# Florescence/UNet-Medical-Image-Contour-Segmentation

Hardware: AMD Instinct MI355X
Metric: images/sec (train step) UNet 1x512x512->1 (higher is better)
Workload: dtype bf16; 1 GPU; UNet(1,1,bilinear=True) train step (BCE+Dice+boundary, clip 1.0, RMSprop), 8 x 1x512x512 per GPU, global batch 8; parallelism=dp1, global_batch=8, per_gpu_batch=8, bn=per-rank batch statistics, dice=global-batch sums (all-reduced), streams=backward-weights on a side stream

## Files before the change

### include/unet_hip.h

```cpp
#ifndef UNET_HIP_H
#define UNET_HIP_H

#include <stddef.h>
#include <stdint.h>

#ifdef __cplusplus
extern "C" {
#endif

typedef void* uh_stream;

enum { UH_F32 = 0, UH_BF16 = 1,
       UH_F32X3 = 2,
       UH_WFRAG = 0x100, UH_WFRAG_D = 0x200 };
enum { UH_OK = 0, UH_EINVAL = -1, UH_ELAUNCH = -2, UH_EWORKSPACE = -3 };

const char* uh_last_error(void);
int uh_version(void);

int uh_pack_w3x3(const float* w, int64_t sO, int64_t sI, int64_t sH, int64_t sW, int Cout, int Cin,
                 void* w_fwd, void* w_dgrad, int dt, uh_stream stream);
int uh_pack_w3x3_batched(const int64_t* table, int nlayers, int64_t ntiles, void* w_fwd_flat,
                         void* w_dgrad_flat, int dt, uh_stream stream);
int uh_unpack_dw3x3(const float* dw_krsc, float* dw, int64_t sO, int64_t sI, int64_t sH, int64_t sW,
                    int Cout, int Cin, uh_stream stream);

int uh_conv3x3_stat_slabs(int B, int H, int W, int Cin, int Cout, int dt);
int uh_conv3x3_wfrag_ok(int B, int H, int W, int C0, int C1, int Cout, int ld0, int ld1, int ldy, int dt);
int uh_conv3x3_fwd_kernel(int B, int H, int W, int C0, int C1, int Cout, int dt);
int uh_conv3x3_wgrad_plan(int B, int H, int W, int C0, int C1, int Cout, int dt, int narrow, int64_t* out);
int uh_conv3x3_fwd_kernel_plan(int B, int plan_B, int H, int W, int C0, int C1, int Cout, int dt);
int uh_conv3x3_wfrag_ok_plan(int B, int plan_B, int H, int W, int C0, int C1, int Cout, int ld0, int ld1, int ldy, int dt);
int uh_conv3x3_fwd_sum_class(int kernel);
int uh_conv3x3_fwd(const void* x0, int C0, int ld0, const void* x1, int C1, int ld1,
                   const void* w, void* y, int ldy, int Cout, float* stat_partials,
                   int B, int H, int W, int dt, uh_stream stream);
int uh_conv3x3_dgrad_bnsum_rows(int B, int H, int W, int Cdy, int Cdx, int lddy, int lddx, int ldq, int dt);
int uh_conv3x3_dgrad_bnsum(const void* dy, int Cdy, int lddy, const void* w_dgrad, void* dx, int lddx, int Cdx,
                           const void* q, int ldq, const float* coef, float* partials,
                           int B, int H, int W, int dt, uh_stream stream);
int uh_stem_ok(int Cin, int Cout, int dt);
int uh_stem_nblk(int B, int H, int W);
int uh_stem_stats(const void* x, int Cin, int ldx, const void* w, float* stat_partials, int B, int H, int W, int dt,
                  uh_stream stream);
int uh_stem_bn_relu_fwd(const void* x, int Cin, int ldx, const void* w, const float* scale, const float* shift, void* z, int ldz,
                        int B, int H, int W, int dt, uh_stream stream);
int uh_stem_bn_relu_bwd_reduce(const void* dz, int lddz, const void* x, int Cin, int ldx, const void* w, const float* scale,
                               const float* shift, const float* mean, const float* rstd, float* partials, int B, int H, int W,
                               int dt, uh_stream stream);
size_t uh_stem_bwd_wgrad_ws_bytes(int B, int H, int W, int Cin);
int uh_stem_bn_relu_bwd_wgrad(const void* dz, int lddz, const void* x, int Cin, int ldx, const void* w, const float* scale,
                              const float* shift, const float* mean, const float* rstd, const float* dgamma, const float* dbeta,
                              int64_t n_total, float* dw_krsc, void* ws, size_t ws_bytes, int B, int H, int W, int dt,
                              uh_stream stream);
int uh_conv3x3_fwd_affine_relu(const void* x0, int C0, int ld0, const void* x1, int C1, int ld1,
                               const void* w, void* z, int ldz, int Cout, const float* scale,
                               const float* shift, int B, int H, int W, int dt, uh_stream stream);
int uh_conv3x3_fwd_affine_relu_plan(const void* x0, int C0, int ld0, const void* x1, int C1, int ld1,
                                    const void* w, void* z, int ldz, int Cout, const float* scale,
                                    const float* shift, int B, int plan_B, int H, int W, int dt, uh_stream stream);
size_t uh_conv3x3_wgrad_ws_bytes(int B, int H, int W, int Cin, int Cout, int dt);
int uh_conv3x3_wgrad(const void* dy, int lddy, const void* x0, int C0, int ld0,
                     const void* x1, int C1, int ld1, float* dw_krsc, int Cout,
                     void* ws, size_t ws_bytes, int B, int H, int W, int dt, uh_stream stream);
int uh_conv3x3_wgrad_partials(const void* dy, int lddy, const void* x0, int C0, int ld0, const void* x1, int C1, int ld1,
                              float* dw_krsc, int Cout, void* ws, size_t ws_bytes, int B, int H, int W, int dt,
// ... 249 lines not shown
```

### unet-medical-image-contour-segmentation_amd/_lib.py

```python
from __future__ import annotations

import ctypes
import os
import re
from typing import Dict, List, Tuple

PKG_DIR = os.path.dirname(os.path.abspath(__file__))
ROOT = os.path.dirname(PKG_DIR)
HEADER = os.path.join(ROOT, "include", "unet_hip.h")
LIB_PATH = os.environ.get("UH_LIB_PATH") or os.path.join(PKG_DIR, "libunet_hip.so")

UH_F32, UH_BF16, UH_F32X3 = 0, 1, 2
UH_WFRAG, UH_WFRAG_D = 0x100, 0x200

_CTYPES = {
    "int": ctypes.c_int, "int64_t": ctypes.c_int64, "float": ctypes.c_float, "double": ctypes.c_double,
    "size_t": ctypes.c_size_t, "uh_stream": ctypes.c_void_p,
}
_RET = {"int": ctypes.c_int, "size_t": ctypes.c_size_t, "const char*": ctypes.c_char_p}


def parse_header(path: str = HEADER) -> Dict[str, Tuple[str, List[str]]]:
    text = open(path).read()
    text = re.sub(r"/\*.*?\*/", " ", text, flags=re.S)
    protos = {}
    for m in re.finditer(r"(const char\*|int|size_t)\s+(uh_\w+)\s*\(([^;{]*?)\)\s*;", text, flags=re.S):
        ret, name, args = m.group(1), m.group(2), " ".join(m.group(3).split())
        types = []
        if args and args != "void":
            for a in args.split(","):
                a = a.strip()
                if "*" in a:
                    types.append("ptr")
                else:
                    types.append(a.rsplit(" ", 1)[0].strip())
        protos[name] = (ret, types)
    return protos


class _Lib:
    def __init__(self):
        self._dll = None
        self.protos = parse_header()

    def load(self):
        if self._dll is not None:
# ... 26 lines not shown
```

### unet-medical-image-contour-segmentation_amd/csrc/conv3x3.hip

```cpp
#include "uh_vec.h"

__host__ __device__ __forceinline__ int uh_wfrag_mode(int es, int rows) { return es == 2 ? ((rows % 128 == 0) ? 2 : 1) : 0; }
template <int ES>
__device__ __forceinline__ int64_t uh_wfrag_index(int o, int tap, int k, int K, int mode) {
    constexpr int CK = 64 / ES, VEC = 16 / ES;
    int g, m;
    if (mode == 2) {
        const int c32 = o & 31;
        g = ((o >> 5) << 1) | ((c32 >> 2) & 1);
        m = ((c32 >> 3) << 2) | (c32 & 3);
    } else if (mode == 1) {
        const int c16 = o & 15, q = c16 >> 2;
        g = o >> 4;
        m = ((((q & 1) << 1) | (q >> 1)) << 2) | (c16 & 3);
    } else {
        g = o >> 4;
        m = o & 15;
    }
    const int chunk = k / CK, e = k - chunk * CK, kp = e / VEC, v = e - kp * VEC;
    return ((((int64_t)g * 9 + tap) * (K / CK) + chunk) * 64 + (kp * 16 + m)) * VEC + v;
}

template <typename T>
__global__ void pack_w3x3_kernel(const float* __restrict__ w, int64_t sO, int64_t sI, int64_t sH, int64_t sW,
// ... 433 lines not shown
            stats[((int64_t)blockIdx.x * 2 + 0) * Cout + co_blk + tid] = red[2 * BN + tid];
            stats[((int64_t)blockIdx.x * 2 + 1) * Cout + co_blk + tid] = red[tid] + red[BN + tid];
        }
        if (blockIdx.y == 0 && tid == 0) stats[(int64_t)gridDim.x * 2 * Cout + blockIdx.x] = (float)(vy * vx);
    }
}

constexpr int HALO2_BYTES = HALO_PIX * 64;
constexpr int HALO2_STRIDE = 6 * 4096;
constexpr unsigned OOB_OFFSET = 0xF0000000u;

__device__ __forceinline__ void uh_dma16(u32x4 desc, unsigned lds_addr, unsigned voff, int soff) {
    asm volatile("s_mov_b32 m0, %0\n\ts_nop 0\n\tbuffer_load_dwordx4 %1, %2, %3 offen lds"
                 :: "s"(lds_addr), "v"(voff), "s"(desc), "s"(soff) : "memory", "m0");
}
__device__ __forceinline__ void uh_ld16_async(u32x4& dst, u32x4 desc, unsigned voff, int soff) {
    asm volatile("buffer_load_dwordx4 %0, %1, %2, %3 offen" : "+v"(dst) : "v"(voff), "s"(desc), "s"(soff) : "memory");
}
__device__ __forceinline__ void uh_ld8_async(u32x2& dst, u32x4 desc, unsigned voff, int soff) {
    asm volatile("buffer_load_dwordx2 %0, %1, %2, %3 offen" : "+v"(dst) : "v"(voff), "s"(desc), "s"(soff) : "memory");
}
__device__ __forceinline__ u32x4 uh_desc_words(const void* p, unsigned bytes) {
    const uint64_t a = (uint64_t)p;
    return u32x4{(unsigned)a, (unsigned)(a >> 32) & 0xffffu, bytes, 0x00020000u};
}
#define UH_WAIT_VM(n) do { asm volatile("s_waitcnt vmcnt(%0)" :: "n"(n) : "memory"); __builtin_amdgcn_sched_barrier(0); } while (0)

__device__ __forceinline__ int halo_swz(int hx) { return ((hx >> 2) & 1) << 1; }

#ifndef UH_BUILD_PRE
#define UH_BUILD_PRE 0
#endif
constexpr int PRE_MAX_C = 512;
template <typename T, int NBW, bool SPLIT = false, bool WRES = false, bool PRE = false, bool BSUM = false, int KS = 1>
__global__ __launch_bounds__(256 * KS, ((NBW == 1 && !WRES && !BSUM && KS == 1) ? 3 : 2)) void conv3x3_fwd_mfma_v2(
    const T* __restrict__ x0, int C0, int ld0, const T* __restrict__ x1, int C1, int ld1,
    const T* __restrict__ w, T* __restrict__ y, int ldy, int Cout, float* __restrict__ stats,
    int B, int H, int W, int tilesX, int tilesY, unsigned x0_bytes, unsigned x1_bytes, unsigned y_bytes,
    const float* __restrict__ ep_scale, const float* __restrict__ ep_shift, int C0v, int C1v, int Coutv, int wfrag,
    const float* __restrict__ pre_scale = nullptr, const float* __restrict__ pre_shift = nullptr,
    const T* __restrict__ bs_y = nullptr, int bs_ld = 0, unsigned bs_bytes = 0, const float* __restrict__ bs_coef = nullptr) {
    static_assert(!PRE || (sizeof(T) == 2 && !SPLIT), "PRE is the bf16 training path");
    static_assert(!BSUM || (sizeof(T) == 2 && !SPLIT && !PRE), "BSUM is the bf16 backward-data path");
    static_assert(KS == 1 || (KS == 2 && sizeof(T) == 2 && NBW == 1 && !SPLIT && !WRES && !PRE), "KS = 2 is a bf16 NBW = 1 form");
    if constexpr (BSUM) {
        x1 = nullptr; C1 = 0; ld1 = 0; x1_bytes = 0;
        C0v = C0; C1v = 0; Coutv = Cout;
        ep_scale = nullptr; ep_shift = nullptr;
        bs_ld = ldy; bs_bytes = y_bytes;
    }
    constexpr int ES = sizeof(T);
    constexpr int CK = 64 / ES;
    constexpr int VEC = 16 / ES;
    constexpr int BN = NBW * 64;
    constexpr int NPIECE = HALO_PIX * 4;
    constexpr int NLOAD = 6;
    constexpr int PF = WRES ? 1 : 2;

    constexpr bool TRI = WRES && !PRE;
    __shared__ __attribute__((aligned(16))) unsigned char lds_all[(TRI ? 3 : KS * 2) * HALO2_STRIDE];
    __shared__ float wg_sum[3][BN];
    __shared__ __attribute__((aligned(16))) float pre_tab[PRE ? 2 * PRE_MAX_C : 4];
    __shared__ __attribute__((aligned(16))) float bs_tab[BSUM ? 4 * BN : 4];
    float n_run = 0.f;

    const int tid = threadIdx.x & 255;
    const int lane = tid & 63;
    const int wave_all = __builtin_amdgcn_readfirstlane((int)(threadIdx.x >> 6));
    const int wave = wave_all & 3;
    const int grp = KS == 2 ? (wave_all >> 2) : 0;
    unsigned char* const lds = lds_all + grp * (2 * HALO2_STRIDE);
    const int lx = lane & 15, kg = lane >> 4;
    const int nslab = Cout / BN;
    const int nlanes = gridDim.x / nslab;
    int tile_lane, slab;
    if ((nlanes & 7) == 0) {
        const int xcd = blockIdx.x & 7, jj = blockIdx.x >> 3;
        slab = jj % nslab;
        tile_lane = (jj / nslab) * 8 + xcd;
    } else {
        slab = blockIdx.x / nlanes;
        tile_lane = blockIdx.x - slab * nlanes;
    }
    const int co_blk = slab * BN;
    const int Cin = C0 + C1;
    const int nch0 = (C0v + CK - 1) / CK, nch1 = (C1v + CK - 1) / CK;
    const int nchunk = nch0 + nch1;
    const int skip1 = C0 / CK - nch0;
    auto chunk_of = [&](int v) -> int { return v < nch0 ? v : v + skip1; };
    const int ntile = B * tilesX * tilesY;

    const u32x4 rs0 = uh_desc_words(x0, x0_bytes);
    const u32x4 rs1 = uh_desc_words(x1 ? x1 : x0, x1 ? x1_bytes : x0_bytes);
    __amdgpu_buffer_rsrc_t rsy = __builtin_amdgcn_make_buffer_rsrc((void*)y, 0, (int)y_bytes, 0x00020000);
    const unsigned lds_base = (unsigned)(uintptr_t)(__attribute__((address_space(3))) unsigned char*)lds;
    constexpr bool REL_LIVE = !(BSUM && NBW == 2);
    auto rel_of = [&](int t, int k) -> int {
        const int p = t + k * 256, q = p >> 2;
        const int hy = (q * 3641) >> 16, hx = q - hy * HALO_W;
        return (hy * W + hx) * ld0 * ES + (((p & 3) ^ halo_swz(hx)) << 4);
    };
    int rel0[NLOAD];
#pragma unroll
    for (int k = 0; k < NLOAD; ++k) rel0[k] = REL_LIVE ? rel_of(tid, k) : 0;
    int d_b = 0, d_y0 = 0, d_x0 = 0;
    bool d_in = false;
    auto dma_tile = [&](int tile) {
        int t = tile;
        const int txt = t % tilesX; t /= tilesX;
        const int tyt = t % tilesY;
        d_b = t / tilesY;
        d_y0 = tyt * TILE; d_x0 = txt * TILE;
        d_in = d_y0 >= 1 && d_y0 + TILE + 1 <= H && d_x0 >= 1 && d_x0 + TILE + 1 <= W;
    };
    auto dma_chunk = [&](int c, int bufi, bool live) {
// ... 107 lines not shown
                    const f32x4 t0 = t[0], t1 = t[1], t2 = t[2], t3 = t[3];
                    float r[8];
#pragma unroll
                    for (int e = 0; e < 4; ++e) {
                        r[2 * e] = __uint_as_float(v[e] << 16);
                        r[2 * e + 1] = __uint_as_float(v[e] & 0xffff0000u);
                    }
                    r[0] = uh_relu(fmaf(r[0], t0[0], t0[1])); r[1] = uh_relu(fmaf(r[1], t0[2], t0[3]));
                    r[2] = uh_relu(fmaf(r[2], t1[0], t1[1])); r[3] = uh_relu(fmaf(r[3], t1[2], t1[3]));
                    r[4] = uh_relu(fmaf(r[4], t2[0], t2[1])); r[5] = uh_relu(fmaf(r[5], t2[2], t2[3]));
                    r[6] = uh_relu(fmaf(r[6], t3[0], t3[1])); r[7] = uh_relu(fmaf(r[7], t3[2], t3[3]));
                    const bf16x8 o = {(bf16_t)r[0], (bf16_t)r[1], (bf16_t)r[2], (bf16_t)r[3],
                                      (bf16_t)r[4], (bf16_t)r[5], (bf16_t)r[6], (bf16_t)r[7]};
                    *slot = __builtin_bit_cast(u32x4, o);
                }
            }
        }
    };
    auto chunk_fence = [&](int c_next, int bufi_next, bool live_next) {
        if constexpr (TRI) {
            asm volatile("s_waitcnt vmcnt(%0) lgkmcnt(0)\n\ts_barrier" :: "n"(NLOAD) : "memory");
        } else if constexpr (PRE) {
            asm volatile("s_waitcnt vmcnt(0)" ::: "memory");
            __builtin_amdgcn_sched_barrier(0);
            if (live_next) pre_transform(c_next, bufi_next);
            asm volatile("s_waitcnt lgkmcnt(0)\n\ts_barrier" ::: "memory");
        } else {
            asm volatile("s_waitcnt vmcnt(0) lgkmcnt(0)\n\ts_barrier" ::: "memory");
        }
        __builtin_amdgcn_sched_barrier(0);
    };

    int tile = tile_lane;
    if (tile >= ntile) return;
    WFrag wA[3][NBW], wB[3][NBW], wC[3][NBW];
#pragma unroll
    for (int r = 0; r < 3; ++r)
#pragma unroll
        for (int n = 0; n < NBW; ++n) {
            wA[r][n].v = wB[r][n].v = wC[r][n].v = u32x4{0u, 0u, 0u, 0u};
            wA[r][n].hi = wB[r][n].hi = wC[r][n].hi = wA[r][n].lo = wB[r][n].lo = wC[r][n].lo = u32x2{0u, 0u};
        }
    auto load_w = [&](WFrag (&dst)[3][NBW], int chunk, int sft) {
        const int64_t wsrc = (int64_t)chunk * CK + (int64_t)sft * Cin;
#pragma unroll
        for (int r = 0; r < 3; ++r)
#pragma unroll
            for (int n = 0; n < NBW; ++n) wfrag_async(dst[r][n], wsrc + wn_off(n) + (int64_t)(r * 3) * Cin, n, r * 3 + sft, chunk);
    };
    int bufi = 0;
    f32x4 acc[16][NBW];
    auto mma_shift = [&](const unsigned char* buf, int sft, auto&& wget) {
        u32x4 xf[18];
        int lq = lane;
        if constexpr (!REL_LIVE) asm volatile("" : "+v"(lq));
        const unsigned char* xcol = buf + ((lq & 15) + sft) * 64 + (((lq >> 4) ^ halo_swz((lq & 15) + sft)) << 4);
        auto rd = [&](int k) { return *reinterpret_cast<const u32x4*>(xcol + k * (HALO_W * 64)); };
#pragma unroll
        for (int k = 0; k < 2 + PF; ++k) xf[k] = rd(k);
#pragma unroll
        for (int k = 2; k < 18; ++k) {
            if (k + PF < 18) xf[k + PF] = rd(k + PF);
            __builtin_amdgcn_sched_barrier(0);
            if constexpr (SPLIT) {
                if (k == 2) { split4(xf[0]); split4(xf[1]); }
                split4(xf[k]);
            }
// ... 97 lines not shown
            const int cur_c = chunk_of(v);
            const int next_c = chunk_of((v + 1 < v_end) ? v + 1 : v_first);
            const unsigned char* buf = lds + bufi * HALO2_STRIDE;
            load_w(wB, cur_c, 1);
            __builtin_amdgcn_sched_barrier(0);
            mma_shift(buf, 0, wsel(wA));
            load_w(wC, cur_c, 2);
            bool live_next = true;
            if (v + 1 < v_end) {
                dma_chunk(chunk_of(v + 1), bufi ^ 1, true);
            } else {
                live_next = next_tile < ntile;
                if (live_next) dma_tile(next_tile);
                dma_chunk(chunk_of(v_first), bufi ^ 1, live_next);
            }
            UH_WAIT_VM(NWLOAD + NLOAD);
            mma_shift(buf, 1, wsel(wB));
            load_w(wA, next_c, 0);
            UH_WAIT_VM(NLOAD + NWLOAD);
            mma_shift(buf, 2, wsel(wC));
            chunk_fence(next_c, bufi ^ 1, live_next);
        }
        }

        if constexpr (KS == 2) {
            f32x4* scratch = reinterpret_cast<f32x4*>(lds_all);
            if (grp == 1) {
#pragma unroll
                for (int i = 0; i < 16; ++i)
#pragma unroll
                    for (int n = 0; n < NBW; ++n) scratch[(i * NBW + n) * 256 + tid] = acc[i][n];
            }
            __syncthreads();
            if (grp == 1) return;
#pragma unroll
            for (int i = 0; i < 16; ++i)
#pragma unroll
                for (int n = 0; n < NBW; ++n) acc[i][n] += scratch[(i * NBW + n) * 256 + tid];
        }
        int t = tile;
        const int txt = t % tilesX; t /= tilesX;
        const int tyt = t % tilesY;
        const int b = t / tilesY;
        const int y0 = tyt * TILE, x0p = txt * TILE;
        const int gx = x0p + lx;
        const int vy = min(TILE, H - y0), vx = min(TILE, W - x0p);
        const bool full = (vy == TILE) && (vx == TILE);
        constexpr int BQB = 2 * NBW;
        u32x2 bqA[BSUM ? 8 : 1], bqB[BSUM ? 8 : 1];
        int lane_o = lane;
        if constexpr (BSUM) asm volatile("" : "+v"(lane_o));
        const int lx_o = lane_o & 15, kg_o = lane_o >> 4;
        auto bq_load = [&](u32x2 (&dst)[BSUM ? 8 : 1], int bi) {
            if constexpr (BSUM) {
                __amdgpu_buffer_rsrc_t rsq = __builtin_amdgcn_make_buffer_rsrc((void*)bs_y, 0, (int)bs_bytes, 0x00020000);
                const int n = bi >> 1, i0 = (bi & 1) * 8;
                const int gxc = min(x0p + (lane_o & 15), W - 1);
                const unsigned voff = (unsigned)((gxc * bs_ld + co_blk + ch(lane_o >> 4, n, 0)) * ES);
#pragma unroll
                for (int i = 0; i < 8; ++i) {
                    const int r = min(i0 + i, vy - 1);
                    dst[i] = __builtin_amdgcn_raw_buffer_load_b64(rsq, voff, ((b * H + y0 + r) * W) * bs_ld * ES, 0);
                }
            }
        };
        if (ep_scale) {
#pragma unroll
// ... 233 lines not shown
                for (int n = 0; n < NBW; ++n) {
                    const f32x4 q = *reinterpret_cast<const f32x4*>(&PV[ch(kg, n, 0)]);
#pragma unroll
                    for (int j = 0; j < 4; ++j) {
                        const float pv = q[j];
                        float s1 = 0.f, s2 = 0.f;
                        if (full) {
#pragma unroll
                            for (int i = 0; i < 16; ++i) {
                                const float d = acc[i][n][j] - pv;
                                s1 += d;
                                s2 = fmaf(d, d, s2);
                            }
                        } else {
#pragma unroll
                            for (int i = 0; i < 16; ++i) {
                                const float d = ((i < vy) && (gx < W)) ? acc[i][n][j] - pv : 0.f;
                                s1 += d;
                                s2 = fmaf(d, d, s2);
                            }
                        }
                        const float a1 = uh_row16_sum(s1), a2 = uh_row16_sum(s2);
                        if (lx == 0) {
                            const int cl = ch(kg, n, j);
                            S1[cl] += a1;
                            S2[cl] += a2;
                        }
                    }
                }
            }
            n_run += (float)(vy * vx);
        }
    }
    if constexpr (BSUM) {
        if (lx == 0) {
#pragma unroll
            for (int n = 0; n < NBW; ++n)
#pragma unroll
                for (int j = 0; j < 4; ++j) {
                    const int cl = ch(kg, n, j);
                    stats[((int64_t)tile_lane * 2 + 0) * Cout + co_blk + cl] = wg_sum[0][cl];
                    stats[((int64_t)tile_lane * 2 + 1) * Cout + co_blk + cl] = wg_sum[1][cl] * bs_tab[3 * BN + cl];
                }
        }
        return;
    }
    if (stats) {
        if (lx == 0) {
            const float inv_n = 1.f / n_run;
#pragma unroll
            for (int n = 0; n < NBW; ++n)
#pragma unroll
                for (int j = 0; j < 4; ++j) {
                    const int cl = ch(kg, n, j);
                    const float a1 = wg_sum[0][cl], a2 = wg_sum[1][cl];
                    stats[((int64_t)tile_lane * 2 + 0) * Cout + co_blk + cl] = wg_sum[2][cl] + a1 * inv_n;
                    stats[((int64_t)tile_lane * 2 + 1) * Cout + co_blk + cl] = fmaxf(a2 - a1 * a1 * inv_n, 0.f);
                }
        }
        float* counts = stats + (int64_t)ntile * 2 * Cout;
        if (slab == 0) {
            if (tid == 0) counts[tile_lane] = n_run;
            if (tile_lane == 0)
                for (int r = nlanes + tid; r < ntile; r += 256) counts[r] = 0.f;
        }
    }
}

template <typename T>
__global__ __launch_bounds__(256) void conv3x3_fwd_stem(const T* __restrict__ x, int Cin, int ldx,
                                                        const T* __restrict__ w, T* __restrict__ y, int ldy, int Cout,
                                                        float* __restrict__ stats, int B, int H, int W, int tilesX,
                                                        int tilesY) {
    __shared__ float xs[HALO_PIX * 4];
    __shared__ float red[4 * 64];
    const int tid = threadIdx.x, lane = tid & 63, wave = tid >> 6;
    int t = blockIdx.x;
    const int txt = t % tilesX; t /= tilesX;
    const int tyt = t % tilesY;
    const int b = t / tilesY;
    const int y0 = tyt * TILE, x0p = txt * TILE;
    for (int idx = tid; idx < HALO_PIX * 4; idx += 256) {
        int q = idx >> 2, ci = idx & 3;
        int hy = q / HALO_W, hx = q - hy * HALO_W;
        int gy = y0 - 1 + hy, gx = x0p - 1 + hx;
        float v = 0.f;
        if (ci < Cin && gy >= 0 && gy < H && gx >= 0 && gx < W)
            v = uh_to_f32(x[(int64_t)((b * H + gy) * W + gx) * ldx + ci]);
        xs[idx] = v;
    }
    __syncthreads();
    for (int cg = 0; cg < Cout; cg += 64) {
        const int co = cg + lane;
        const bool cok = co < Cout;
        float wr[36];
#pragma unroll
        for (int tap = 0; tap < 9; ++tap)
#pragma unroll
// ... 352 lines not shown
    if (threadIdx.x == 0) stats[(int64_t)gridDim.x * 2 * C + blockIdx.x] = (float)(vy * vx);
}

extern "C" int uh_conv3x3_stat_slabs(int B, int H, int W, int Cin, int Cout, int dt) {
    (void)Cin; (void)Cout; (void)dt;
    return B * ((H + TILE - 1) / TILE) * ((W + TILE - 1) / TILE);
}

static bool fwd_ksplit_ok(int64_t ntile, int Cin, int Cout) {
    static const bool off = getenv("UH_NO_KSPLIT") != nullptr && getenv("UH_NO_KSPLIT")[0] == '1';
    const int nchunk = Cin / 32;
    return !off && Cin % 32 == 0 && Cout % 64 == 0 && ntile * (Cout / 64) <= 256 && nchunk >= 8 && nchunk % 2 == 0;
}

enum FwdKernel {
    FWD_SIMT = 0,
    FWD_SLAB128 = 1,
    FWD_WRES = 2,
    FWD_KSPLIT = 3,
    FWD_STREAM = 4,
    FWD_LARGE = 5,
};

static int fwd_sum_class(int kernel) {
    return (kernel == FWD_SLAB128 || kernel == FWD_WRES || kernel == FWD_STREAM) ? FWD_SLAB128 : kernel;
}

struct FwdPlan {
    FwdKernel kernel;
    int stem;
    int slabs, lanes;
    int threads;
    bool split, pre, bsum;
};

static FwdPlan fwd_plan(int es, int B, int H, int W, int C0, int C1, int Cout, int ld0, int ld1, int ldy, bool ptrs16, bool y16,
                        bool split, bool narrow, bool pre, bool bsum, int plan_B = 0) {
    const int tiles1 = ((H + TILE - 1) / TILE) * ((W + TILE - 1) / TILE);
    const int ntile = B * tiles1;
    const int ck = 64 / es, Cin = C0 + C1;
    FwdPlan p = {FWD_SIMT, 0, 1, ntile, 256, split, pre, bsum};
    const bool mfma = C0 % ck == 0 && C1 % ck == 0 && Cout % 64 == 0 && ptrs16 && (ld0 * es) % 16 == 0 &&
                      (C1 == 0 || (ld1 * es) % 16 == 0) && (ldy * es) % 16 == 0;
    if (!mfma) {
        const bool y_ok = y16 && (ldy * es) % 16 == 0;
        if (Cin > 4 || C1 != 0) p.stem = 0;
        else if (es == 2 && Cout == 64 && y_ok) { p.stem = 3; p.lanes = ntile < 1024 ? ntile : 1024; }
        else p.stem = (Cout % (16 / es) == 0 && y_ok) ? 2 : 1;
        return p;
    }
    const int64_t px = (int64_t)B * H * W, lim = (1ll << 31) - 4096;
    if (px * ld0 * es >= lim || (C1 && px * ld1 * es >= lim) || px * ldy * es >= lim ||
        (int64_t)Cout * 9 * Cin * (split ? 4 : es) >= lim) {
        p.kernel = FWD_LARGE;
        p.slabs = Cout % 128 == 0 ? Cout / 128 : Cout / 64;
        return p;
    }
    auto lanes_for = [&](int per_cu, int slabs) {
        int gx = (per_cu * 256 + slabs - 1) / slabs;
        gx = (gx + 7) & ~7;
        return gx < ntile ? gx : ntile;
    };
    const bool bf16 = es == 2 && !split && !narrow;
    auto form = [&](int64_t nt) {
        if (Cout % 128 == 0 && nt * (Cout / 128) >= 512) return FWD_SLAB128;
        if (bf16 && Cin == 64) return FWD_WRES;
        if (bf16 && !pre && fwd_ksplit_ok(nt, Cin, Cout)) return FWD_KSPLIT;
        return FWD_STREAM;
    };
    p.kernel = form(ntile);
    if (plan_B > 0 && plan_B != B) {
        const FwdKernel pinned = form((int64_t)plan_B * tiles1);
        if (fwd_sum_class(pinned) != fwd_sum_class(p.kernel)) p.kernel = pinned;
    }
    switch (p.kernel) {
    case FWD_SLAB128: p.slabs = Cout / 128; p.lanes = lanes_for(2, p.slabs); break;
    case FWD_WRES: p.slabs = Cout / 64; p.lanes = lanes_for(2, p.slabs); break;
    case FWD_KSPLIT: p.slabs = Cout / 64; p.lanes = ntile; p.threads = 512; break;
    default: p.slabs = Cout / 64; p.lanes = lanes_for(bsum ? 2 : 3, p.slabs); break;
    }
    return p;
}

template <typename T, bool SPLIT, bool PRE, bool BSUM, typename... Args>
static void fwd_v2_form(const FwdPlan& p, hipStream_t st, Args... args) {
    constexpr bool BF16 = sizeof(T) == 2 && !SPLIT;
    const dim3 grid(p.lanes * p.slabs), block(p.threads);
    switch (p.kernel) {
    case FWD_SLAB128: hipLaunchKernelGGL((conv3x3_fwd_mfma_v2<T, 2, SPLIT, false, PRE, BSUM>), grid, block, 0, st, args...); break;
    case FWD_WRES:
        if constexpr (BF16) hipLaunchKernelGGL((conv3x3_fwd_mfma_v2<T, 1, false, true, PRE, BSUM>), grid, block, 0, st, args...);
        break;
    case FWD_KSPLIT:
        if constexpr (BF16 && !PRE) hipLaunchKernelGGL((conv3x3_fwd_mfma_v2<T, 1, false, false, false, BSUM, 2>), grid, block, 0, st, args...);
        break;
    case FWD_STREAM: hipLaunchKernelGGL((conv3x3_fwd_mfma_v2<T, 1, SPLIT, false, PRE, BSUM>), grid, block, 0, st, args...); break;
    default: break;
    }
}

template <typename T, typename... Args>
static void fwd_v2_launch(const FwdPlan& p, hipStream_t st, Args... args) {
    constexpr bool BF16 = sizeof(T) == 2;
    if (p.split) {
        if constexpr (!BF16) fwd_v2_form<T, true, false, false>(p, st, args...);
    } else if (p.bsum) {
        if constexpr (BF16) fwd_v2_form<T, false, false, true>(p, st, args...);
    } else if (p.pre) {
        if constexpr (BF16 && UH_BUILD_PRE) fwd_v2_form<T, false, true, false>(p, st, args...);
    } else {
        fwd_v2_form<T, false, false, false>(p, st, args...);
    }
}

struct ConvCall {
    const void *x0 = nullptr, *x1 = nullptr;
    int C0 = 0, ld0 = 0, C1 = 0, ld1 = 0, Cout = 0, B = 0, H = 0, W = 0;
    int dt = UH_F32;
    bool wfrag = false;
    int C0v = -1, C1v = -1, Coutv = -1;
    const float *pre_scale = nullptr, *pre_shift = nullptr;
    hipStream_t st = nullptr;
};
struct FwdCall : ConvCall {
    const void* w = nullptr;
    void* y = nullptr; int ldy = 0, plan_B = 0;
    float* stats = nullptr;
    const float *ep_scale = nullptr, *ep_shift = nullptr;
    bool ep_done = false;
    const void* bs_y = nullptr;
    int bs_ld = 0; const float* bs_coef = nullptr;
};

enum { CK_BF16_ONLY = 1, CK_NARROW = 2, CK_WFRAG = 4 };
static int conv_check(const char* fn, ConvCall& c, bool ptrs, int ldo, int dt, int flags = 0) {
    const bool narrow = (flags & CK_NARROW) != 0;
    UH_REQUIRE(c.x0 && ptrs, "%s: null pointer", fn);
    UH_REQUIRE(c.B > 0 && c.H > 0 && c.W > 0 && c.C0 > 0 && c.C1 >= 0 && c.Cout > 0, "%s: bad shape", fn);
    UH_REQUIRE(!narrow || (c.C0v > 0 && c.C0v <= c.C0 && c.C1v >= 0 && c.C1v <= c.C1 && c.Coutv > 0 && c.Coutv <= c.Cout),
               "%s: bad valid counts", fn);
    UH_REQUIRE(c.ld0 >= (narrow ? c.C0v : c.C0) && ldo >= (narrow ? c.Coutv : c.Cout) &&
               (c.C1 == 0 || (c.x1 && c.ld1 >= (narrow ? c.C1v : c.C1))), "%s: bad strides", fn);
    UH_REQUIRE((int64_t)c.B * c.H * c.W < (1ll << 31), "%s: pixel count overflows int32", fn);
    c.wfrag = (flags & CK_WFRAG) && (dt & UH_WFRAG);
    if (flags & CK_WFRAG) dt &= ~UH_WFRAG;
    UH_REQUIRE(!(flags & CK_BF16_ONLY) || dt == UH_BF16, "%s: bf16 only (dtype %d)", fn, dt);
    UH_REQUIRE(dt == UH_F32 || dt == UH_BF16 || dt == UH_F32X3, "%s: bad dtype %d", fn, dt);
    const int vec = dt == UH_BF16 ? 8 : 4;
    UH_REQUIRE(!narrow || (c.C0v % vec == 0 && c.C1v % vec == 0 && c.Coutv % vec == 0),
               "%s: valid counts must be multiples of a 16-byte piece", fn);
    c.dt = dt;
    return UH_OK;
}

template <typename T>
static int conv3x3_fwd_dispatch(FwdCall& c) {
    const T *x0 = (const T*)c.x0, *x1 = (const T*)c.x1, *w = (const T*)c.w, *bs_y = (const T*)c.bs_y;
    T* y = (T*)c.y;
    const float *ep_scale = c.ep_scale, *ep_shift = c.ep_shift;
    const bool split = c.dt == UH_F32X3, narrow = c.C0v >= 0, pre = c.pre_scale != nullptr, bsum = bs_y != nullptr;
    const int C0v = narrow ? c.C0v : c.C0, C1v = narrow ? c.C1v : c.C1, Coutv = narrow ? c.Coutv : c.Cout;
    c.ep_done = false;
    constexpr int ES = sizeof(T);
    const int tilesX = (c.W + TILE - 1) / TILE, tilesY = (c.H + TILE - 1) / TILE;
    const int Cin = c.C0 + c.C1;
    const bool ptrs16 = uh_aligned16(x0) && (c.C1 == 0 || uh_aligned16(x1)) && uh_aligned16(w) && uh_aligned16(y);
    const FwdPlan p = fwd_plan(ES, c.B, c.H, c.W, c.C0, c.C1, c.Cout, c.ld0, c.ld1, c.ldy, ptrs16, uh_aligned16(y), split, narrow, pre, bsum, c.plan_B);
    if (p.kernel != FWD_SIMT && p.kernel != FWD_LARGE) {
        if (ep_scale && !(uh_aligned16(ep_scale) && uh_aligned16(ep_shift))) ep_scale = ep_shift = nullptr;
        UH_REQUIRE(!split || ES == 4, "conv3x3_fwd: bf16x3 needs fp32 tensors");
        UH_REQUIRE(!(split && c.wfrag), "conv3x3_fwd: bf16x3 filters are KRSC packs");
        UH_REQUIRE(!(narrow && c.wfrag), "conv3x3_fwd: narrow-tensor calls take KRSC packs");
        if (pre) {
            UH_REQUIRE(UH_BUILD_PRE, "conv3x3_fwd: the consumer-side BatchNorm+ReLU instantiations are not in this build (UH_BUILD_PRE=1); uh_conv3x3_pre_ok says so");
            UH_REQUIRE(ES == 2, "conv3x3_fwd: the fused BatchNorm+ReLU input is a bf16 path; ask uh_conv3x3_pre_ok first");
            UH_REQUIRE(!(split || narrow || c.C0 > PRE_MAX_C), "conv3x3_fwd: the fused BatchNorm+ReLU input needs a plain bf16 call with at most %d channels in source 0; ask uh_conv3x3_pre_ok first", PRE_MAX_C);
        }
        const int64_t px = (int64_t)c.B * c.H * c.W, bq = bsum ? px * c.bs_ld * ES : 0;
        if (bsum) {
            UH_REQUIRE(ES == 2, "uh_conv3x3_dgrad_bnsum: bf16 only; ask uh_conv3x3_dgrad_bnsum_rows first");
            UH_REQUIRE(!(split || narrow || c.C1 != 0 || !c.stats || !c.bs_coef || c.bs_ld != c.ldy || !uh_aligned16(bs_y) || bq >= (1ll << 31) - 4096),
                       "uh_conv3x3_dgrad_bnsum: needs a plain single-source bf16 call and a 16-byte aligned BatchNorm input below 2 GiB; ask uh_conv3x3_dgrad_bnsum_rows first");
        }
        fwd_v2_launch<T>(p, c.st, x0, c.C0, c.ld0, x1, c.C1, c.ld1, w, y, c.ldy, c.Cout, c.stats, c.B, c.H, c.W, tilesX, tilesY, (unsigned)(px * c.ld0 * ES),
                         (unsigned)(c.C1 ? px * c.ld1 * ES : 0), (unsigned)(px * c.ldy * ES), ep_scale, ep_shift, C0v, C1v, Coutv,
                         c.wfrag ? 1 : 0, c.pre_scale, c.pre_shift, bs_y, c.bs_ld, (unsigned)bq, c.bs_coef);
        UH_CHECK_LAUNCH(pre ? "conv3x3_fwd_mfma_v2 (BatchNorm+ReLU input)"
                            : bsum ? "conv3x3_fwd_mfma_v2 (backward-data + BatchNorm sums)" : "conv3x3_fwd_mfma_v2");
        c.ep_done = ep_scale != nullptr;
        return UH_OK;
    }
    if (p.kernel == FWD_LARGE) {
        UH_REQUIRE(!pre, "conv3x3_fwd: the fused BatchNorm+ReLU input needs the LDS-DMA MFMA kernel (tensors below 2 GiB); ask uh_conv3x3_pre_ok first");
        UH_REQUIRE(!bsum, "uh_conv3x3_dgrad_bnsum: needs the LDS-DMA MFMA kernel (tensors below 2 GiB); ask uh_conv3x3_dgrad_bnsum_rows first");
        UH_REQUIRE(!c.wfrag, "conv3x3_fwd: the filter is packed fragment-major (UH_WFRAG) but this call cannot take the LDS-DMA MFMA kernel (a tensor of 2 GiB or more); ask uh_conv3x3_wfrag_ok first");
        UH_REQUIRE(!split, "conv3x3_fwd: bf16x3 is implemented for tensors below 2 GiB only");
        UH_REQUIRE(!narrow, "conv3x3_fwd: narrow tensors are implemented for tensors below 2 GiB only");
        if (c.Cout % 128 == 0)
            hipLaunchKernelGGL((conv3x3_fwd_mfma<T, 4>), dim3(p.lanes, p.slabs), dim3(p.threads), 0, c.st, x0, c.C0, c.ld0, x1, c.C1,
                               c.ld1, w, y, c.ldy, c.Cout, c.stats, c.B, c.H, c.W, tilesX, tilesY);
        else
            hipLaunchKernelGGL((conv3x3_fwd_mfma<T, 2>), dim3(p.lanes, p.slabs), dim3(p.threads), 0, c.st, x0, c.C0, c.ld0, x1, c.C1,
                               c.ld1, w, y, c.ldy, c.Cout, c.stats, c.B, c.H, c.W, tilesX, tilesY);
        UH_CHECK_LAUNCH("conv3x3_fwd_mfma");
        return UH_OK;
    }
    UH_REQUIRE(!pre, "conv3x3_fwd: the fused BatchNorm+ReLU input needs an MFMA-aligned shape; ask uh_conv3x3_pre_ok first");
    UH_REQUIRE(!bsum, "uh_conv3x3_dgrad_bnsum: needs an MFMA-aligned shape; ask uh_conv3x3_dgrad_bnsum_rows first");
    UH_REQUIRE(!c.wfrag, "conv3x3_fwd: the filter is packed fragment-major (UH_WFRAG) but the shape / alignment is outside the MFMA path; ask uh_conv3x3_wfrag_ok first");
    UH_REQUIRE(!split, "conv3x3_fwd: bf16x3 needs an MFMA-aligned shape (Cin %% 16 == 0, Cout %% 64 == 0, 16-byte strides)");
    UH_REQUIRE(!narrow, "conv3x3_fwd: narrow tensors need padded counts that are MFMA-aligned and 16-byte strides");
    if (p.stem == 3) {
        if constexpr (ES == 2) {
            switch (Cin) {
                case 1: hipLaunchKernelGGL((conv3x3_fwd_stem_v3<T, 1>), dim3(p.lanes), dim3(256), 0, c.st, x0, c.ld0, w, y, c.ldy, c.stats, c.B, c.H, c.W, tilesX, tilesY, ep_scale, ep_shift); break;
                case 2: hipLaunchKernelGGL((conv3x3_fwd_stem_v3<T, 2>), dim3(p.lanes), dim3(256), 0, c.st, x0, c.ld0, w, y, c.ldy, c.stats, c.B, c.H, c.W, tilesX, tilesY, ep_scale, ep_shift); break;
                case 3: hipLaunchKernelGGL((conv3x3_fwd_stem_v3<T, 3>), dim3(p.lanes), dim3(256), 0, c.st, x0, c.ld0, w, y, c.ldy, c.stats, c.B, c.H, c.W, tilesX, tilesY, ep_scale, ep_shift); break;
                default: hipLaunchKernelGGL((conv3x3_fwd_stem_v3<T, 4>), dim3(p.lanes), dim3(256), 0, c.st, x0, c.ld0, w, y, c.ldy, c.stats, c.B, c.H, c.W, tilesX, tilesY, ep_scale, ep_shift); break;
            }
// ... 38 lines not shown
                              int ldy, int Cout, float* stat_partials, int B, int H, int W, int dt, uh_stream stream) {
    FwdCall c;
    c.x0 = x0; c.C0 = C0; c.ld0 = ld0; c.x1 = x1; c.C1 = C1; c.ld1 = ld1; c.w = w; c.y = y; c.ldy = ldy; c.Cout = Cout;
    c.stats = stat_partials; c.B = B; c.H = H; c.W = W; c.st = (hipStream_t)stream;
    return conv3x3_fwd_call("uh_conv3x3_fwd", c, dt);
}

extern "C" int uh_conv3x3_wfrag_ok_plan(int B, int plan_B, int H, int W, int C0, int C1, int Cout, int ld0, int ld1, int ldy,
                                        int dt) {
    if (dt != UH_F32 && dt != UH_BF16) return 0;
    if (B <= 0 || plan_B < 0 || H <= 0 || W <= 0 || C0 <= 0 || C1 < 0 || Cout <= 0) return 0;
    const FwdKernel k = fwd_plan(dt == UH_BF16 ? 2 : 4, B, H, W, C0, C1, Cout, ld0, ld1, ldy, true, true, false, false, false,
                                 false, plan_B).kernel;
    return k != FWD_SIMT && k != FWD_LARGE;
}
extern "C" int uh_conv3x3_wfrag_ok(int B, int H, int W, int C0, int C1, int Cout, int ld0, int ld1, int ldy, int dt) {
    return uh_conv3x3_wfrag_ok_plan(B, 0, H, W, C0, C1, Cout, ld0, ld1, ldy, dt);
}

extern "C" int uh_conv3x3_fwd_kernel(int B, int H, int W, int C0, int C1, int Cout, int dt) {
    UH_REQUIRE(B > 0 && H > 0 && W > 0 && C0 > 0 && C1 >= 0 && Cout > 0, "uh_conv3x3_fwd_kernel: bad shape");
    UH_REQUIRE(dt == UH_F32 || dt == UH_BF16 || dt == UH_F32X3, "uh_conv3x3_fwd_kernel: bad dtype %d", dt);
    return fwd_plan(dt == UH_BF16 ? 2 : 4, B, H, W, C0, C1, Cout, C0, C1, Cout, true, true, dt == UH_F32X3, false, false,
                    false).kernel;
}

extern "C" int uh_conv3x3_fwd_kernel_plan(int B, int plan_B, int H, int W, int C0, int C1, int Cout, int dt) {
    UH_REQUIRE(B > 0 && plan_B >= 0 && H > 0 && W > 0 && C0 > 0 && C1 >= 0 && Cout > 0, "uh_conv3x3_fwd_kernel_plan: bad shape");
    UH_REQUIRE(dt == UH_F32 || dt == UH_BF16 || dt == UH_F32X3, "uh_conv3x3_fwd_kernel_plan: bad dtype %d", dt);
    return fwd_plan(dt == UH_BF16 ? 2 : 4, B, H, W, C0, C1, Cout, C0, C1, Cout, true, true, dt == UH_F32X3, false, false,
                    false, plan_B).kernel;
}

extern "C" int uh_conv3x3_fwd_sum_class(int kernel) {
    UH_REQUIRE(kernel >= FWD_SIMT && kernel <= FWD_LARGE, "uh_conv3x3_fwd_sum_class: bad kernel code %d", kernel);
    return fwd_sum_class(kernel);
}

extern "C" int uh_conv3x3_pre_ok(int B, int H, int W, int C0, int Cout, int ld0, int ldy, int dt) {
#if !UH_BUILD_PRE
    return 0;
#endif
    if (dt != UH_BF16 || C0 > PRE_MAX_C) return 0;
    if (C0 % 64 || Cout % 64) return 0;
    return uh_conv3x3_wfrag_ok(B, H, W, C0, 0, Cout, ld0, 0, ldy, dt);
}

extern "C" int uh_conv3x3_fwd_pre(const void* x0, int C0, int ld0, const float* pre_scale, const float* pre_shift, const void* w,
                                  void* y, int ldy, int Cout, float* stat_partials, int B, int H, int W, int dt,
                                  uh_stream stream) {
    UH_REQUIRE(pre_scale && pre_shift, "uh_conv3x3_fwd_pre: null pointer");
    FwdCall c;
    c.x0 = x0; c.C0 = C0; c.ld0 = ld0; c.w = w; c.y = y; c.ldy = ldy; c.Cout = Cout; c.stats = stat_partials;
    c.B = B; c.H = H; c.W = W; c.st = (hipStream_t)stream; c.pre_scale = pre_scale; c.pre_shift = pre_shift;
    if (const int rc = conv_check("uh_conv3x3_fwd_pre", c, c.w && c.y, c.ldy, dt, CK_BF16_ONLY | CK_WFRAG)) return rc;
    UH_REQUIRE(UH_BUILD_PRE, "uh_conv3x3_fwd_pre: the consumer-side BatchNorm+ReLU instantiations are not in this build (UH_BUILD_PRE=1); uh_conv3x3_pre_ok says so");
    UH_REQUIRE(uh_conv3x3_pre_ok(B, H, W, C0, Cout, ld0, ldy, c.dt), "uh_conv3x3_fwd_pre: shape outside the fused path (uh_conv3x3_pre_ok)");
    return conv3x3_fwd_dispatch<bf16_t>(c);
}

extern "C" int uh_conv3x3_dgrad_bnsum_rows(int B, int H, int W, int Cdy, int Cdx, int lddy, int lddx, int ldq, int dt) {
    if (dt != UH_BF16) return 0;
    if (!uh_conv3x3_wfrag_ok(B, H, W, Cdy, 0, Cdx, lddy, 0, lddx, dt)) return 0;
    if (ldq != lddx) return 0;
    return fwd_plan(2, B, H, W, Cdy, 0, Cdx, lddy, 0, lddx, true, true, false, false, false, true).lanes;
}
// ... 15 lines not shown
}

extern "C" int uh_conv3x3_fwd_affine_relu_plan(const void* x0, int C0, int ld0, const void* x1, int C1, int ld1, const void* w,
                                               void* z, int ldz, int Cout, const float* scale, const float* shift, int B,
                                               int plan_B, int H, int W, int dt, uh_stream stream) {
    UH_REQUIRE(plan_B >= 0, "uh_conv3x3_fwd_affine_relu: bad plan length %d", plan_B);
    UH_REQUIRE(scale && shift, "uh_conv3x3_fwd_affine_relu: null pointer");
    FwdCall c;
    c.x0 = x0; c.C0 = C0; c.ld0 = ld0; c.x1 = x1; c.C1 = C1; c.ld1 = ld1; c.w = w; c.y = z; c.ldy = ldz; c.Cout = Cout;
    c.B = B; c.H = H; c.W = W; c.st = (hipStream_t)stream; c.ep_scale = scale; c.ep_shift = shift; c.plan_B = plan_B;
    const int rc = conv3x3_fwd_call("uh_conv3x3_fwd_affine_relu", c, dt);
    if (rc != UH_OK || c.ep_done) return rc;
    return uh_bn_relu_apply(z, ldz, scale, shift, z, ldz, (int64_t)B * H * W, Cout, c.dt == UH_BF16 ? UH_BF16 : UH_F32, stream);
}

extern "C" int uh_conv3x3_fwd_affine_relu(const void* x0, int C0, int ld0, const void* x1, int C1, int ld1, const void* w,
                                          void* z, int ldz, int Cout, const float* scale, const float* shift, int B,
                                          int H, int W, int dt, uh_stream stream) {
    return uh_conv3x3_fwd_affine_relu_plan(x0, C0, ld0, x1, C1, ld1, w, z, ldz, Cout, scale, shift, B, 0, H, W, dt, stream);
}

extern "C" int uh_conv3x3_fwd_narrow_plan(const void* x0, int C0, int C0v, int ld0, const void* x1, int C1, int C1v, int ld1,
                                          const void* w, void* y, int ldy, int Cout, int Coutv, float* stat_partials,
                                          const float* scale, const float* shift, int B, int plan_B, int H, int W, int dt,
                                          uh_stream stream) {
    UH_REQUIRE(plan_B >= 0, "uh_conv3x3_fwd_narrow: bad plan length %d", plan_B);
    UH_REQUIRE((scale == nullptr) == (shift == nullptr), "uh_conv3x3_fwd_narrow: scale and shift come together");
    FwdCall c;
    c.x0 = x0; c.C0 = C0; c.ld0 = ld0; c.x1 = x1; c.C1 = C1; c.ld1 = ld1; c.w = w; c.y = y; c.ldy = ldy; c.Cout = Cout;
    c.stats = stat_partials; c.B = B; c.H = H; c.W = W; c.st = (hipStream_t)stream; c.ep_scale = scale; c.ep_shift = shift;
    c.C0v = C0v; c.C1v = C1v; c.Coutv = Coutv; c.plan_B = plan_B;
    const int rc = conv3x3_fwd_call("uh_conv3x3_fwd_narrow", c, dt, CK_NARROW);
    if (rc != UH_OK || !scale || c.ep_done) return rc;
    return uh_bn_relu_apply(y, ldy, scale, shift, y, ldy, (int64_t)B * H * W, Coutv, dt == UH_BF16 ? UH_BF16 : UH_F32, stream);
}

extern "C" int uh_conv3x3_fwd_narrow(const void* x0, int C0, int C0v, int ld0, const void* x1, int C1, int C1v, int ld1,
                                     const void* w, void* y, int ldy, int Cout, int Coutv, float* stat_partials,
                                     const float* scale, const float* shift, int B, int H, int W, int dt, uh_stream stream) {
    return uh_conv3x3_fwd_narrow_plan(x0, C0, C0v, ld0, x1, C1, C1v, ld1, w, y, ldy, Cout, Coutv, stat_partials, scale, shift, B, 0,
                                      H, W, dt, stream);
}

template <typename T> struct WgradCfg;
template <> struct WgradCfg<bf16_t> { static constexpr int TH = 8; };
template <> struct WgradCfg<float> { static constexpr int TH = 8; };

typedef __attribute__((ext_vector_type(16))) float f32x16;
typedef __attribute__((ext_vector_type(4))) short s16x4;

template <typename T, bool SPLIT = false>
__global__ __launch_bounds__(256, 2) void conv3x3_wgrad_mfma(
    const T* __restrict__ dy, int lddy, const T* __restrict__ x0, int C0, int ld0, const T* __restrict__ x1, int C1,
    int ld1, float* __restrict__ slabs, int Cout, int B, int H, int W, int tilesX, int tilesY, int nsplit,
    int C0v, int C1v, int Coutv) {
    constexpr int ES = sizeof(T);
    constexpr int TH = WgradCfg<T>::TH;
    constexpr int PB = 64 * ES;
    constexpr int XPIX = (TH + 2) * HALO_W;
    constexpr int DPIX = TH * TILE;
    constexpr int VEC = 16 / ES;
    constexpr int PPP = PB / 16;
    __shared__ __attribute__((aligned(16))) unsigned char lds[(XPIX + DPIX) * PB];
    unsigned char* xs = lds;
    unsigned char* ds = lds + XPIX * PB;

    const int tid = threadIdx.x, lane = tid & 63, wave = tid >> 6;
    const int wr = wave >> 1, wc = wave & 1;
    const int Cin = C0 + C1;
    const int nci = Cin / 64;
    const int cot = blockIdx.y / nci, cit = blockIdx.y - cot * nci;
    const int co0 = cot * 64, ci0 = cit * 64;
    const T* xsrc; int ldx;
    int xleft;
    if (ci0 < C0) { xsrc = x0 + ci0; ldx = ld0; xleft = C0v - ci0; } else { xsrc = x1 + (ci0 - C0); ldx = ld1; xleft = C1v - (ci0 - C0); }
    const T* dsrc = dy + co0;
    const int dleft = Coutv - co0;

    const int ntile = B * tilesX * tilesY;
    const int split = blockIdx.x;
    const int t_begin = (int)(((int64_t)ntile * split) / nsplit);
    const int t_end = (int)(((int64_t)ntile * (split + 1)) / nsplit);

    f32x16 acc[9];
#pragma unroll
    for (int k = 0; k < 9; ++k)
#pragma unroll
        for (int j = 0; j < 16; ++j) acc[k][j] = 0.f;

    auto lds_addr = [&](int q, int byte) -> int {
        if constexpr (ES == 2) return q * PB + (byte ^ (((q >> 1) & 1) << 6));
        else return q * PB + byte;
    };

    for (int tile = t_begin; tile < t_end; ++tile) {
        int t = tile;
        const int txt = t % tilesX; t /= tilesX;
        const int tyt = t % tilesY;
        const int b = t / tilesY;
        const int y0 = tyt * TH, x0p = txt * TILE;
        __syncthreads();
        constexpr int SB = 4;
        for (int base = 0; base < XPIX * PPP; base += SB * 256) {
            u32x4 v[SB];
            bool ok[SB];
#pragma unroll
            for (int k = 0; k < SB; ++k) {
                const int idx = min(base + tid + k * 256, XPIX * PPP - 1);
                const int q = idx / PPP, part = idx - q * PPP;
                const int hy = q / HALO_W, hx = q - hy * HALO_W;
                const int gy = y0 - 1 + hy, gx = x0p - 1 + hx;
                ok[k] = gy >= 0 && gy < H && gx >= 0 && gx < W && part * VEC < xleft;
                const int gyc = min(max(gy, 0), H - 1), gxc = min(max(gx, 0), W - 1), pc = part * VEC < xleft ? part : 0;
// ... 123 lines not shown
            }
        } else {
            const int l32 = lane & 31, kh = lane >> 5;
#pragma unroll 1
            for (int hy = 0; hy < TH + 2; ++hy) {
#pragma unroll
                for (int s = 0; s < 3; ++s) {
#pragma unroll
                    for (int r = 0; r < 3; ++r) {
                        const int ty = hy - r;
                        if (ty < 0 || ty >= TH) continue;
#pragma unroll
                        for (int kk = 0; kk < 8; ++kk) {
                            const int px = kk * 2 + kh;
                            float a = *reinterpret_cast<const float*>(ds + (ty * TILE + px) * PB + (wr * 32 + l32) * 4);
                            float bb = *reinterpret_cast<const float*>(xs + (hy * HALO_W + px + s) * PB + (wc * 32 + l32) * 4);
                            acc[r * 3 + s] = __builtin_amdgcn_mfma_f32_32x32x2f32(a, bb, acc[r * 3 + s], 0, 0, 0);
                        }
                    }
                }
            }
        }
    }

    float* slab = slabs + (int64_t)split * Cout * 9 * Cin;
    const int ci = ci0 + wc * 32 + (lane & 31);
#pragma unroll
    for (int tap = 0; tap < 9; ++tap)
#pragma unroll
        for (int reg = 0; reg < 16; ++reg) {
            int co = co0 + wr * 32 + (reg & 3) + 8 * (reg >> 2) + 4 * (lane >> 5);
            slab[((int64_t)co * 9 + tap) * Cin + ci] = acc[tap][reg];
        }
}

__device__ __forceinline__ void slab_reduce_block_f32(const float* __restrict__ slabs, float* __restrict__ out, int64_t n,
                                                      int nsplit, int64_t blk, f32x4 (*red)[64]) {
    const int cl = threadIdx.x & 63, sl = threadIdx.x >> 6;
    const int64_t i4 = blk * 64 + cl;
    const int64_t n4 = n >> 2;
    f32x4 a0 = {0.f, 0.f, 0.f, 0.f}, a1 = a0, a2 = a0, a3 = a0;
    if (i4 < n4) {
        const f32x4* base = reinterpret_cast<const f32x4*>(slabs) + i4;
        int k = sl;
        for (; k + 12 < nsplit; k += 16) {
            a0 += base[(int64_t)k * n4];
            a1 += base[(int64_t)(k + 4) * n4];
            a2 += base[(int64_t)(k + 8) * n4];
            a3 += base[(int64_t)(k + 12) * n4];
        }
        for (; k < nsplit; k += 4) a0 += base[(int64_t)k * n4];
    }
    red[sl][cl] = (a0 + a1) + (a2 + a3);
    __syncthreads();
    if (sl == 0 && i4 < n4) reinterpret_cast<f32x4*>(out)[i4] = (red[0][cl] + red[1][cl]) + (red[2][cl] + red[3][cl]);
}

__global__ __launch_bounds__(256) void slab_reduce_kernel(const float* __restrict__ slabs, float* __restrict__ out, int64_t n,
                                                          int nsplit) {
    __shared__ f32x4 red[8][64];
    slab_reduce_block_f32(slabs, out, n, nsplit, blockIdx.x, red);
}

__global__ __launch_bounds__(256) void slab_reduce_tall_kernel(const float* __restrict__ slabs, float* __restrict__ out, int64_t n,
                                                               int nsplit) {
    __shared__ f32x4 red[4][4];
// ... 103 lines not shown
        default: f(std::integral_constant<int, 4>{}); break;
    }
}

__global__ __launch_bounds__(256) void slab_reduce_f16pair_kernel(const unsigned* __restrict__ slabs, float* __restrict__ out,
                                                                  int64_t npair, int row, int nsplit, int coblk) {
    __shared__ f32x4 red[512];
    __shared__ float sc_tab[512];
    slab16_dispatch(nsplit, [&](auto sl) {
        slab_reduce_block_f16pair<decltype(sl)::value>(slabs, out, npair, row, nsplit, coblk, blockIdx.x, red, sc_tab);
    });
}

constexpr int SLAB_TAB = 8;
__global__ __launch_bounds__(256) void slab_reduce_batched_kernel(const int64_t* __restrict__ table, int nrows) {
    __shared__ f32x4 red[512];
    __shared__ float sc_tab[512];
    const int64_t b = blockIdx.x;
    int r = 0;
    for (int k = 1; k < nrows; ++k)
        if (table[k * SLAB_TAB + 6] <= b) r = k;
    const int64_t* t = table + r * SLAB_TAB;
    const int64_t blk = b - t[6];
    if (t[4] == 0)
        slab_reduce_block_f32(reinterpret_cast<const float*>(t[0]), reinterpret_cast<float*>(t[1]), t[2], (int)t[3], blk,
                              reinterpret_cast<f32x4(*)[64]>(red));
    else
        slab16_dispatch((int)t[3], [&](auto sl) {
            slab_reduce_block_f16pair<decltype(sl)::value>(reinterpret_cast<const unsigned*>(t[0]), reinterpret_cast<float*>(t[1]),
                                                           t[2] / 2, (int)t[5], (int)t[3], (int)t[7], blk, red, sc_tab);
        });
}

template <typename T, int NWR, bool PRE = false, bool SLAB16 = false>
__global__ __launch_bounds__(128 * NWR, 2) void conv3x3_wgrad_mfma_v2(
    const T* __restrict__ dy, int lddy, const T* __restrict__ x0, int C0, int ld0, const T* __restrict__ x1, int C1,
    int ld1, float* __restrict__ slabs, int Cout, int B, int H, int W, int tilesX, int tilesY, int nsplit,
    unsigned dy_bytes, unsigned x_bytes, int C0v, int C1v, int Coutv, const float* __restrict__ pre_scale = nullptr,
    const float* __restrict__ pre_shift = nullptr) {
    static_assert(sizeof(T) == 2, "v2 is the bf16 kernel");
    constexpr int TH = 8;
    constexpr int NT = 128 * NWR;
    constexpr int PB = 128;
    constexpr int DPB = 64 * NWR;
    constexpr int DU = DPB / 16;
    constexpr int XPIX = (TH + 2) * HALO_W;
    constexpr int DPIX = TH * TILE;
    constexpr int XUNITS = XPIX * 8;
    constexpr int XR = (XUNITS + NT - 1) / NT;
    constexpr int DR = DPIX * DU / NT;
    constexpr int RB = NT * 16;
    constexpr int XBYTES = XR * RB, STAGE = XBYTES + DR * RB;
    __shared__ __attribute__((aligned(16))) unsigned char lds[2 * STAGE];

    const int tid = threadIdx.x, lane = tid & 63;
    const int wave = __builtin_amdgcn_readfirstlane(tid >> 6);
    const int wr = wave >> 1, wc = wave & 1;
    const int Cin = C0 + C1;
    const int nci = Cin / 64;
    const int cot = blockIdx.y / nci, cit = blockIdx.y - cot * nci;
    const int co0 = cot * (32 * NWR), ci0 = cit * 64;
    const T* xsrc; int ldx;
    int xleft;
    if (ci0 < C0) { xsrc = x0 + ci0; ldx = ld0; xleft = C0v - ci0; } else { xsrc = x1 + (ci0 - C0); ldx = ld1; xleft = C1v - (ci0 - C0); }
    const int dleft = Coutv - co0;
    const u32x4 rsx = uh_desc_words(xsrc, x_bytes);
    const u32x4 rsd = uh_desc_words(dy + co0, dy_bytes);
    const unsigned lds_base = (unsigned)(uintptr_t)(__attribute__((address_space(3))) unsigned char*)lds;

    const int ntile = B * tilesX * tilesY;
    const int split = blockIdx.x;
    const int t_begin = (int)(((int64_t)ntile * split) / nsplit);
    const int t_end = (int)(((int64_t)ntile * (split + 1)) / nsplit);

    int xg[XR], xo[XR];
#pragma unroll
    for (int k = 0; k < XR; ++k) {
        const int p = tid + k * NT;
        const int q = p >> 3;
        const int hy = q / HALO_W, hx = q - hy * HALO_W;
        const int u = (p & 7) ^ (((hx >> 1) & 1) << 2);
        xg[k] = (p < XUNITS && u * 8 < xleft) ? ((hy << 8) | hx) : -1;
        xo[k] = (hy * W + hx) * ldx * 2 + u * 16;
    }
    auto dswz = [&](int col) -> int { return NWR == 2 ? (((col >> 1) & 1) << 2) : ((col & 3) << 2); };
    static_assert(NT / DU == 2 * TILE, "dy DMA rounds are two tile rows apart");
    int dg0, dof0;
    {
        const int q = tid / DU, u = (tid % DU) ^ dswz(q & 15);
        dg0 = (u * 8 < dleft) ? (((q >> 4) << 8) | (q & 15)) : -1;
        dof0 = ((q >> 4) * W + (q & 15)) * lddy * 2 + u * 16;
    }
    const int dof_round = 2 * W * lddy * 2;
    auto issue = [&](int tile, int bufi) {
        int t = tile;
        const int txt = t % tilesX; t /= tilesX;
        const int tyt = t % tilesY;
        const int b = t / tilesY;
        const int y0 = tyt * TH, x0p = txt * TILE;
        const int xbase = ((b * H + y0 - 1) * W + x0p - 1) * ldx * 2;
        const int dbase = ((b * H + y0) * W + x0p) * lddy * 2;
        const unsigned xb = lds_base + bufi * STAGE + wave * 1024;
        const unsigned db = xb + XBYTES;
        const bool inside = y0 >= 1 && y0 + TH + 1 <= H && x0p >= 1 && x0p + TILE + 1 <= W;
// ... 205 lines not shown
                            for (int hh = 0; hh < 2; ++hh)
                                acc[r * 3 + sft][h][hh] = __builtin_amdgcn_mfma_f32_16x16x32_bf16(dfr[pr][h], xfr[a][sft][hh],
                                                                                                 acc[r * 3 + sft][h][hh], 0, 0, 0);
                }
            }
        }
        tile_fence(tile + 1, bufi ^ 1, tile + 1 < t_end);
    }
    }

    if constexpr (SLAB16) {
        float m = 0.f;
#pragma unroll
        for (int tap = 0; tap < 9; ++tap)
#pragma unroll
            for (int h = 0; h < 2; ++h)
#pragma unroll
                for (int hh = 0; hh < 2; ++hh)
#pragma unroll
                    for (int j = 0; j < 4; ++j) m = fmaxf(m, fabsf(acc[tap][h][hh][j]));
#pragma unroll
        for (int o = 32; o > 0; o >>= 1) m = fmaxf(m, __shfl_xor(m, o, 64));
        float* wmax = reinterpret_cast<float*>(lds);
        if (lane == 0) wmax[wave] = m;
        __syncthreads();
#pragma unroll
        for (int k = 0; k < 2 * NWR; ++k) m = fmaxf(m, wmax[k]);
        unsigned eb = (__float_as_uint(m) >> 23) & 0xffu;
        eb = eb < 15u ? 15u : (eb > 254u ? 254u : eb);
        const float sc = __uint_as_float((268u - eb) << 23);
        unsigned* slab16 = reinterpret_cast<unsigned*>(slabs) + (int64_t)split * (Cout / 2) * 9 * Cin;
        if (tid == 0) {
            float* inv = reinterpret_cast<float*>(reinterpret_cast<unsigned*>(slabs) + (int64_t)nsplit * (Cout / 2) * 9 * Cin);
            inv[(int64_t)split * gridDim.y + blockIdx.y] = __uint_as_float((eb - 14u) << 23);
        }
#pragma unroll
        for (int tap = 0; tap < 9; ++tap)
#pragma unroll
            for (int h = 0; h < 2; ++h)
#pragma unroll
                for (int hh = 0; hh < 2; ++hh)
#pragma unroll
                    for (int jp = 0; jp < 4; jp += 2) {
                        const int co = co0 + wr * 32 + h * 16 + (lane >> 4) * 4 + jp;
                        const int ci = ci0 + wc * 32 + hh * 16 + (lane & 15);
                        const f16x2 pr = {(_Float16)(acc[tap][h][hh][jp] * sc), (_Float16)(acc[tap][h][hh][jp + 1] * sc)};
                        slab16[((int64_t)(co >> 1) * 9 + tap) * Cin + ci] = __builtin_bit_cast(unsigned, pr);
                    }
        return;
    }
    float* slab = slabs + (int64_t)split * Cout * 9 * Cin;
#pragma unroll
    for (int tap = 0; tap < 9; ++tap)
#pragma unroll
        for (int h = 0; h < 2; ++h)
#pragma unroll
            for (int hh = 0; hh < 2; ++hh)
#pragma unroll
                for (int j = 0; j < 4; ++j) {
                    const int co = co0 + wr * 32 + h * 16 + (lane >> 4) * 4 + j;
                    const int ci = ci0 + wc * 32 + hh * 16 + (lane & 15);
                    slab[((int64_t)co * 9 + tap) * Cin + ci] = acc[tap][h][hh][j];
                }
}

__global__ void slab_reduce_scalar_kernel(const float* __restrict__ slabs, float* __restrict__ out, int64_t n, int nsplit) {
    int64_t i = (int64_t)blockIdx.x * blockDim.x + threadIdx.x;
    if (i >= n) return;
    float s = 0.f;
    for (int k = 0; k < nsplit; ++k) s += slabs[(int64_t)k * n + i];
    out[i] = s;
}

template <typename T>
__global__ __launch_bounds__(256) void conv3x3_wgrad_stem(const T* __restrict__ dy, int lddy, const T* __restrict__ x,
                                                          int Cin, int ldx, float* __restrict__ slabs, int Cout, int B,
                                                          int H, int W, int tilesX, int tilesY, int nsplit) {
    __shared__ float xs[HALO_PIX * 4];
    __shared__ float red[4 * 64];
    const int tid = threadIdx.x, lane = tid & 63, wave = tid >> 6;
    const int ntile = B * tilesX * tilesY;
    const int split = blockIdx.x;
    const int t_begin = (int)(((int64_t)ntile * split) / nsplit);
    const int t_end = (int)(((int64_t)ntile * (split + 1)) / nsplit);
    const int cg = blockIdx.y * 64;
    const int co = cg + lane;
    const bool cok = co < Cout;
    float acc[36];
#pragma unroll
    for (int k = 0; k < 36; ++k) acc[k] = 0.f;
    for (int tile = t_begin; tile < t_end; ++tile) {
        int t = tile;
        const int txt = t % tilesX; t /= tilesX;
        const int tyt = t % tilesY;
        const int b = t / tilesY;
        const int y0 = tyt * TILE, x0p = txt * TILE;
// ... 240 lines not shown
};

enum SlabReduceKernel { SR_NONE = 0, SR_SCALAR = 1, SR_VEC = 2, SR_TALL = 3, SR_F16PAIR = 4 };
struct SlabReduce {
    SlabReduceKernel kernel;
    int64_t n, blocks;
    int nsplit, row, coblk;
};

static SlabReduce slab_reduce_plan(int64_t n, int nsplit, int row, int coblk, bool f16pair, bool vec16, bool tall) {
    SlabReduce r = {SR_SCALAR, n, (n + 255) / 256, nsplit, row, coblk};
    if (f16pair) { r.kernel = SR_F16PAIR; r.blocks = uh_slab16_blocks(n / 2, nsplit); }
    else if (n % 4 == 0 && vec16 && tall && n <= 4096 && nsplit >= 256) { r.kernel = SR_TALL; r.blocks = (n / 4 + 3) / 4; }
    else if (n % 4 == 0 && vec16) { r.kernel = SR_VEC; r.blocks = (n / 4 + 63) / 64; }
    return r;
}

static int slab_reduce_launch(const SlabReduce& r, const void* slabs, float* dw, hipStream_t st) {
    const dim3 grid((unsigned)r.blocks), block(256);
    if (r.kernel == SR_F16PAIR)
        hipLaunchKernelGGL(slab_reduce_f16pair_kernel, grid, block, 0, st, (const unsigned*)slabs, dw, r.n / 2, r.row, r.nsplit, r.coblk);
    else if (r.kernel != SR_NONE)
        hipLaunchKernelGGL(r.kernel == SR_SCALAR ? slab_reduce_scalar_kernel : r.kernel == SR_TALL ? slab_reduce_tall_kernel : slab_reduce_kernel,
                           grid, block, 0, st, (const float*)slabs, dw, r.n, r.nsplit);
    UH_CHECK_LAUNCH(r.kernel == SR_F16PAIR ? "slab_reduce_f16pair_kernel" : "slab_reduce_kernel");
    return UH_OK;
}

struct WgradPlan {
    WgradKernel kernel;
    int tilesX, tilesY;
    int nsplit;
    dim3 grid;
    int threads;
    bool slab16, pre;
    SlabReduce reduce;
};
struct WgradAlign { bool ptrs, dy, dw, ws; };
static const WgradAlign WG_ALIGNED = {true, true, true, true};
static size_t wgrad_slab_bytes(const WgradPlan& p) { return (size_t)p.nsplit * p.reduce.n * sizeof(float); }

static WgradPlan wgrad_plan(int es, int B, int H, int W, int C0, int C1, int Cout, int ld0, int ld1, int lddy, WgradAlign a16,
                            bool narrow, bool pre) {
    static const bool slab_f32 = getenv("UH_WGRAD_SLAB_F32") != nullptr && getenv("UH_WGRAD_SLAB_F32")[0] == '1';
    static_assert(WgradCfg<bf16_t>::TH == WgradCfg<float>::TH, "one pixel-tile height for both element types");
    const int Cin = C0 + C1;
    const int64_t n = (int64_t)Cout * 9 * Cin;
    WgradPlan p = {WG_GENERIC, 0, 0, 0, dim3(Cout * 9), 256, false, pre, {SR_NONE, n, 0, 0, 9 * Cin, 0}};
    const bool dy_ok = a16.dy && (lddy * es) % 16 == 0;
    int nwr = 2;
    if (a16.ptrs && dy_ok && (ld0 * es) % 16 == 0 && (C1 == 0 || (ld1 * es) % 16 == 0) && C0 % 64 == 0 && Cin % 64 == 0 && Cout % 64 == 0) {
        p.tilesX = (W + TILE - 1) / TILE; p.tilesY = (H + WgradCfg<float>::TH - 1) / WgradCfg<float>::TH;
        const int ntile = B * p.tilesX * p.tilesY;
        const int64_t px = (int64_t)B * H * W, lim = (1ll << 31) - 4096;
        const bool dma = es == 2 && px * (ld0 > ld1 ? ld0 : ld1) * 2 < lim && px * lddy * 2 < lim;
        if (dma && !narrow && Cout % 128 == 0) nwr = 4;
        p.kernel = !dma ? WG_MFMA : nwr == 4 ? WG_DMA128 : WG_DMA64;
        const int ctiles = (Cin / 64) * (Cout / (32 * nwr));
        const int want = ((nwr == 4 ? 256 : 512) + ctiles - 1) / ctiles;
        p.nsplit = want < 1 ? 1 : (want > ntile ? ntile : want);
        p.grid = dim3(p.nsplit, ctiles); p.threads = 128 * nwr;
        p.slab16 = dma && a16.dw && !slab_f32;
    } else if (Cin <= 4 && C1 == 0) {
        p.tilesX = (W + TILE - 1) / TILE; p.tilesY = (H + TILE - 1) / TILE;
        const int ntile = B * p.tilesX * p.tilesY;
        p.nsplit = 1024 > ntile ? ntile : 1024;
        if (es == 2 && Cout == 64 && dy_ok) { p.kernel = WG_STEM_V3; p.grid = dim3(p.nsplit, Cin); }
        else if (Cout % (16 / es) == 0 && dy_ok) { p.kernel = WG_STEM_V2; p.grid = dim3(p.nsplit, 1, Cin); }
        else { p.kernel = WG_STEM; p.grid = dim3(p.nsplit, (Cout + 63) / 64); }
    } else
        return p;
    p.reduce = slab_reduce_plan(n, p.nsplit, 9 * Cin, 32 * nwr, p.slab16, a16.dw && a16.ws, false);
    return p;
}

extern "C" size_t uh_conv3x3_wgrad_ws_bytes(int B, int H, int W, int Cin, int Cout, int dt) {
    const int es = dt == UH_BF16 ? 2 : 4;
    const size_t wide = wgrad_slab_bytes(wgrad_plan(es, B, H, W, Cin, 0, Cout, Cin, 0, Cout, WG_ALIGNED, false, false));
    const size_t narrow = wgrad_slab_bytes(wgrad_plan(es, B, H, W, Cin, 0, Cout, Cin, 0, Cout, WG_ALIGNED, true, false));
    return (wide > narrow ? wide : narrow) + 16;
}

extern "C" int uh_conv3x3_wgrad_plan(int B, int H, int W, int C0, int C1, int Cout, int dt, int narrow, int64_t* out) {
    UH_REQUIRE(out && B > 0 && H > 0 && W > 0 && C0 > 0 && C1 >= 0 && Cout > 0, "uh_conv3x3_wgrad_plan: null pointer or bad shape");
    UH_REQUIRE(dt == UH_F32 || dt == UH_BF16 || dt == UH_F32X3, "uh_conv3x3_wgrad_plan: bad dtype %d", dt);
    const WgradPlan p = wgrad_plan(dt == UH_BF16 ? 2 : 4, B, H, W, C0, C1, Cout, C0, C1, Cout, WG_ALIGNED, narrow != 0, false);
    out[0] = p.kernel; out[1] = p.nsplit; out[2] = p.grid.x; out[3] = p.grid.y; out[4] = p.threads; out[5] = p.slab16 ? 1 : 0;
    out[6] = p.reduce.kernel; out[7] = p.reduce.blocks;
    return UH_OK;
}

template <typename T, typename... Args>
static void wgrad_v2_launch(const WgradPlan& p, hipStream_t st, Args... args) {
    auto form = [&](auto pre) {
        constexpr bool PRE = decltype(pre)::value;
        const dim3 block(p.threads);
        switch ((p.kernel == WG_DMA128 ? 2 : 0) + (p.slab16 ? 1 : 0)) {
        case 3: hipLaunchKernelGGL((conv3x3_wgrad_mfma_v2<T, 4, PRE, true>), p.grid, block, 0, st, args...); break;
        case 2: hipLaunchKernelGGL((conv3x3_wgrad_mfma_v2<T, 4, PRE, false>), p.grid, block, 0, st, args...); break;
        case 1: hipLaunchKernelGGL((conv3x3_wgrad_mfma_v2<T, 2, PRE, true>), p.grid, block, 0, st, args...); break;
        default: hipLaunchKernelGGL((conv3x3_wgrad_mfma_v2<T, 2, PRE, false>), p.grid, block, 0, st, args...); break;
        }
    };
    if (p.pre) {
        if constexpr (UH_BUILD_PRE) form(std::true_type{});
    } else
        form(std::false_type{});
}

struct WgradCall : ConvCall {
    const void* dy = nullptr; int lddy = 0;
    float* dw = nullptr;
    void* ws = nullptr; size_t ws_bytes = 0;
    int64_t* defer = nullptr;
};

template <typename T>
static int conv3x3_wgrad_dispatch(const WgradCall& c) {
    const T *dy = (const T*)c.dy, *x0 = (const T*)c.x0, *x1 = (const T*)c.x1;
    float* slabs = (float*)c.ws;
    constexpr int ES = sizeof(T);
    const int Cin = c.C0 + c.C1;
    const bool split = c.dt == UH_F32X3, narrow = c.C0v >= 0, pre = c.pre_scale != nullptr;
    const int C0v = narrow ? c.C0v : c.C0, C1v = narrow ? c.C1v : c.C1, Coutv = narrow ? c.Coutv : c.Cout;
    const WgradAlign a16 = {uh_aligned16(dy) && uh_aligned16(x0) && (c.C1 == 0 || uh_aligned16(x1)), uh_aligned16(dy), uh_aligned16(c.dw),
                            uh_aligned16(slabs)};
    const WgradPlan p = wgrad_plan(ES, c.B, c.H, c.W, c.C0, c.C1, c.Cout, c.ld0, c.ld1, c.lddy, a16, narrow, pre);
    const bool mfma = p.kernel >= WG_MFMA, dma = p.kernel >= WG_DMA64;
    UH_REQUIRE(!narrow || mfma, "uh_conv3x3_wgrad_narrow: needs the MFMA path (padded channel counts multiples of 64, 16-byte strides)");
    UH_REQUIRE(!split || mfma, "uh_conv3x3_wgrad: bf16x3 needs an MFMA-aligned shape (channel counts multiples of 64, 16-byte strides)");
    UH_REQUIRE(!pre || UH_BUILD_PRE, "uh_conv3x3_wgrad_pre: the consumer-side BatchNorm+ReLU instantiations are not in this build (UH_BUILD_PRE=1); uh_conv3x3_pre_ok says so");
    UH_REQUIRE(!pre || (dma && !narrow && !split), "uh_conv3x3_wgrad_pre: needs the bf16 LDS-DMA kernel (64-aligned channels, tensors below 2 GiB); ask uh_conv3x3_pre_ok first");
    for (int k = 0; c.defer && k < 8; ++k) c.defer[k] = 0;
    if (p.kernel != WG_GENERIC && (c.ws_bytes < wgrad_slab_bytes(p) || !c.ws)) {
        uh_set_error("uh_conv3x3_wgrad: workspace %zu < %zu bytes", c.ws_bytes, wgrad_slab_bytes(p));
        return UH_EWORKSPACE;
    }
    const dim3 block(p.threads);
    const int64_t px = (int64_t)c.B * c.H * c.W;
    switch (p.kernel) {
    case WG_GENERIC:
        hipLaunchKernelGGL(conv3x3_wgrad_generic<T>, p.grid, block, 0, c.st, dy, c.lddy, x0, c.C0, c.ld0, x1, c.C1, c.ld1, c.dw, c.Cout, c.B, c.H, c.W);
        UH_CHECK_LAUNCH("conv3x3_wgrad_generic");
        return UH_OK;
    case WG_DMA64: case WG_DMA128:
        if constexpr (ES == 2)
            wgrad_v2_launch<T>(p, c.st, dy, c.lddy, x0, c.C0, c.ld0, x1, c.C1, c.ld1, slabs, c.Cout, c.B, c.H, c.W, p.tilesX, p.tilesY, p.nsplit,
                               (unsigned)(px * c.lddy * 2), (unsigned)(px * (c.ld0 > c.ld1 ? c.ld0 : c.ld1) * 2), C0v, C1v, Coutv, c.pre_scale,
                               c.pre_shift);
        UH_CHECK_LAUNCH("conv3x3_wgrad_mfma_v2");
        break;
    case WG_MFMA:
        if (split) {
            if constexpr (ES == 4)
                hipLaunchKernelGGL((conv3x3_wgrad_mfma<T, true>), p.grid, block, 0, c.st, dy, c.lddy, x0, c.C0, c.ld0, x1, c.C1, c.ld1, slabs, c.Cout,
                                   c.B, c.H, c.W, p.tilesX, p.tilesY, p.nsplit, C0v, C1v, Coutv);
        } else
            hipLaunchKernelGGL(conv3x3_wgrad_mfma<T>, p.grid, block, 0, c.st, dy, c.lddy, x0, c.C0, c.ld0, x1, c.C1, c.ld1, slabs, c.Cout, c.B, c.H, c.W,
                               p.tilesX, p.tilesY, p.nsplit, C0v, C1v, Coutv);
        UH_CHECK_LAUNCH("conv3x3_wgrad_mfma");
        break;
    case WG_STEM_V3:
        if constexpr (ES == 2)
            hipLaunchKernelGGL((conv3x3_wgrad_stem_v3<T, 1>), p.grid, block, 0, c.st, dy, c.lddy, x0, c.ld0, slabs, c.B, c.H, c.W, p.tilesX,
                               p.tilesY, Cin);
        UH_CHECK_LAUNCH("conv3x3_wgrad_stem_v3");
        break;
    case WG_STEM_V2:
        hipLaunchKernelGGL(conv3x3_wgrad_stem_v2<T>, p.grid, block, 0, c.st, dy, c.lddy, x0, Cin, c.ld0, slabs, c.Cout, c.B, c.H, c.W, p.nsplit);
        UH_CHECK_LAUNCH("conv3x3_wgrad_stem_v2");
        break;
    case WG_STEM:
        hipLaunchKernelGGL(conv3x3_wgrad_stem<T>, p.grid, block, 0, c.st, dy, c.lddy, x0, Cin, c.ld0, slabs, c.Cout, c.B, c.H, c.W, p.tilesX,
                           p.tilesY, p.nsplit);
        UH_CHECK_LAUNCH("conv3x3_wgrad_stem");
        break;
    }
    const SlabReduce& r = p.reduce;
    if (c.defer && (r.kernel == SR_VEC || r.kernel == SR_F16PAIR) && a16.ws) {
        const int64_t row[8] = {(int64_t)(uintptr_t)slabs, (int64_t)(uintptr_t)c.dw, r.n, r.nsplit, r.kernel == SR_F16PAIR, r.row, r.blocks, r.coblk};
        for (int k = 0; k < 8; ++k) c.defer[k] = row[k];
        return UH_OK;
    }
    return slab_reduce_launch(r, slabs, c.dw, c.st);
}

static int conv3x3_wgrad_call(const char* fn, WgradCall& c, int dt, int flags = 0) {
    if (const int rc = conv_check(fn, c, c.dy && c.dw, c.lddy, dt, flags)) return rc;
    return c.dt == UH_BF16 ? conv3x3_wgrad_dispatch<bf16_t>(c) : conv3x3_wgrad_dispatch<float>(c);
}

extern "C" int uh_conv3x3_wgrad(const void* dy, int lddy, const void* x0, int C0, int ld0, const void* x1, int C1, int ld1,
// ... 21 lines not shown
    UH_CHECK_LAUNCH("slab_reduce_batched_kernel");
    return UH_OK;
}

extern "C" int uh_conv3x3_wgrad_pre(const void* dy, int lddy, const void* x0, int C0, int ld0, const float* pre_scale,
                                    const float* pre_shift, float* dw_krsc, int Cout, void* ws, size_t ws_bytes, int B, int H,
                                    int W, int dt, uh_stream stream) {
    UH_REQUIRE(pre_scale && pre_shift, "uh_conv3x3_wgrad_pre: null pointer");
    WgradCall c;
    c.dy = dy; c.lddy = lddy; c.x0 = x0; c.C0 = C0; c.ld0 = ld0; c.dw = dw_krsc; c.Cout = Cout; c.ws = ws; c.ws_bytes = ws_bytes;
    c.B = B; c.H = H; c.W = W; c.st = (hipStream_t)stream; c.pre_scale = pre_scale; c.pre_shift = pre_shift;
    if (const int rc = conv_check("uh_conv3x3_wgrad_pre", c, c.dy && c.dw, c.lddy, dt, CK_BF16_ONLY)) return rc;
    UH_REQUIRE(C0 % 64 == 0 && Cout % 64 == 0, "uh_conv3x3_wgrad_pre: channel counts must be multiples of 64");
    return conv3x3_wgrad_dispatch<bf16_t>(c);
}

extern "C" int uh_stem_ok(int Cin, int Cout, int dt) { return (dt == UH_BF16 && Cin == 1 && Cout == 64) ? 1 : 0; }
extern "C" int uh_stem_nblk(int B, int H, int W) {
    const int64_t ntile = (int64_t)B * ((H + TILE - 1) / TILE) * ((W + TILE - 1) / TILE);
    return (int)(ntile < 1024 ? ntile : 1024);
}

#define UH_STEM_COMMON(fn)                                                                                                    \
    UH_REQUIRE(x && w, fn ": null pointer");                                                                                  \
    UH_REQUIRE(B > 0 && H > 0 && W > 0 && ldx >= Cin, fn ": bad shape");                                                      \
    UH_REQUIRE(uh_stem_ok(Cin, 64, dt), fn ": bf16, one input channel, 64 output channels (uh_stem_ok)");                   \
    UH_REQUIRE((int64_t)B * H * W < (1ll << 31), fn ": pixel count overflows int32")

extern "C" int uh_stem_stats(const void* x, int Cin, int ldx, const void* w, float* stat_partials, int B, int H, int W, int dt,
                             uh_stream stream) {
    UH_STEM_COMMON("uh_stem_stats");
    UH_REQUIRE(stat_partials, "uh_stem_stats: null statistics buffer");
    return uh_stem_mfma_launch(0, x, ldx, w, nullptr, nullptr, nullptr, nullptr, nullptr, nullptr, 0.f, nullptr, 0, nullptr, 0,
                               stat_partials, B, H, W, uh_stem_nblk(B, H, W), stream);
}

extern "C" int uh_stem_bn_relu_fwd(const void* x, int Cin, int ldx, const void* w, const float* scale, const float* shift, void* z,
                                   int ldz, int B, int H, int W, int dt, uh_stream stream) {
    UH_STEM_COMMON("uh_stem_bn_relu_fwd");
    UH_REQUIRE(scale && shift && z && ldz >= 64, "uh_stem_bn_relu_fwd: null pointer / bad stride");
    UH_REQUIRE(uh_aligned16(z) && (ldz * 2) % 16 == 0, "uh_stem_bn_relu_fwd: z must be 16-byte aligned with a 16-byte pixel pitch");
    return uh_stem_mfma_launch(1, x, ldx, w, scale, shift, nullptr, nullptr, nullptr, nullptr, 0.f, nullptr, 0, z, ldz, nullptr, B, H, W,
                               uh_stem_nblk(B, H, W), stream);
}

extern "C" int uh_stem_bn_relu_bwd_reduce(const void* dz, int lddz, const void* x, int Cin, int ldx, const void* w,
                                          const float* scale, const float* shift, const float* mean, const float* rstd,
                                          float* partials, int B, int H, int W, int dt, uh_stream stream) {
    UH_STEM_COMMON("uh_stem_bn_relu_bwd_reduce");
    UH_REQUIRE(dz && scale && shift && mean && rstd && partials && lddz >= 64, "uh_stem_bn_relu_bwd_reduce: null pointer / bad stride");
    UH_REQUIRE(uh_aligned16(dz) && (lddz * 2) % 16 == 0, "uh_stem_bn_relu_bwd_reduce: dz must be 16-byte aligned with a 16-byte pixel pitch");
    return uh_stem_mfma_launch(2, x, ldx, w, scale, shift, mean, rstd, nullptr, nullptr, 0.f, dz, lddz, nullptr, 0, partials, B, H, W,
                               uh_stem_nblk(B, H, W), stream);
}

extern "C" size_t uh_stem_bwd_wgrad_ws_bytes(int B, int H, int W, int Cin) {
    return (size_t)uh_stem_nblk(B, H, W) * 64 * 9 * (Cin > 0 ? Cin : 1) * sizeof(float) + 16;
}

extern "C" int uh_stem_bn_relu_bwd_wgrad(const void* dz, int lddz, const void* x, int Cin, int ldx, const void* w,
                                         const float* scale, const float* shift, const float* mean, const float* rstd,
                                         const float* dgamma, const float* dbeta, int64_t n_total, float* dw_krsc, void* ws,
                                         size_t ws_bytes, int B, int H, int W, int dt, uh_stream stream) {
    UH_STEM_COMMON("uh_stem_bn_relu_bwd_wgrad");
    UH_REQUIRE(dz && scale && shift && mean && rstd && dgamma && dbeta && dw_krsc && ws && lddz >= 64,
               "uh_stem_bn_relu_bwd_wgrad: null pointer / bad stride");
    UH_REQUIRE(uh_aligned16(dz) && (lddz * 2) % 16 == 0, "uh_stem_bn_relu_bwd_wgrad: dz must be 16-byte aligned with a 16-byte pixel pitch");
    UH_REQUIRE(ws_bytes >= uh_stem_bwd_wgrad_ws_bytes(B, H, W, Cin), "uh_stem_bn_relu_bwd_wgrad: workspace too small");
    const float inv_n = (float)(1.0 / (double)(n_total > 0 ? n_total : (int64_t)B * H * W));
    float* slabs = (float*)ws;
    const int rc = uh_stem_mfma_launch(3, x, ldx, w, scale, shift, mean, rstd, dgamma, dbeta, inv_n, dz, lddz, nullptr, 0, slabs, B, H, W,
                                       uh_stem_nblk(B, H, W), stream);
    if (rc != UH_OK) return rc;
    return slab_reduce_launch(slab_reduce_plan((int64_t)64 * 9 * Cin, uh_stem_nblk(B, H, W), 9 * Cin, 64, false,
                                               uh_aligned16(dw_krsc) && uh_aligned16(slabs), true), slabs, dw_krsc, (hipStream_t)stream);
}

extern "C" int uh_conv3x3_wgrad_narrow(const void* dy, int lddy, int Cout, int Coutv, const void* x0, int C0, int C0v, int ld0,
                                       const void* x1, int C1, int C1v, int ld1, float* dw_krsc, void* ws, size_t ws_bytes,
                                       int B, int H, int W, int dt, uh_stream stream) {
    WgradCall c;
    c.dy = dy; c.lddy = lddy; c.x0 = x0; c.C0 = C0; c.ld0 = ld0; c.x1 = x1; c.C1 = C1; c.ld1 = ld1; c.dw = dw_krsc; c.Cout = Cout;
    c.ws = ws; c.ws_bytes = ws_bytes; c.B = B; c.H = H; c.W = W; c.st = (hipStream_t)stream;
    c.C0v = C0v; c.C1v = C1v; c.Coutv = Coutv;
    return conv3x3_wgrad_call("uh_conv3x3_wgrad_narrow", c, dt, CK_NARROW);
}
```

### unet-medical-image-contour-segmentation_amd/csrc/stem_mfma.hip

```cpp
#include "uh_common.h"
#include <type_traits>

namespace {

constexpr int ST_TILE = 16, ST_HALO = 18, ST_PITCH = 20;
constexpr int ST_C = 64;

struct StemArgs {
    const bf16_t* x; int ldx;
    const bf16_t* w;
    const float* scale; const float* shift; const float* mean; const float* rstd;
    const float* dgamma; const float* dbeta; float inv_n;
    const bf16_t* dz; int lddz;
    bf16_t* z; int ldz;
    float* out;
    int B, H, W, tilesX, tilesY;
};

template <int MODE>
__global__ __launch_bounds__(256, 2) void stem_mfma_kernel(StemArgs a) {
    __shared__ unsigned short xs[ST_HALO * ST_PITCH + 4];
    __shared__ float red[4][MODE == 3 ? 9 : 2][ST_C];
    __shared__ float pivot[ST_C];
    __shared__ __attribute__((aligned(16))) float cf[4][ST_C];
    constexpr int DP = 68;
    __shared__ __attribute__((aligned(16))) unsigned short dyt[MODE == 3 ? 4 * 16 * DP : 4];
    const int tid = threadIdx.x, lane = tid & 63, wave = tid >> 6;
    const int lx = lane & 15, kg = lane >> 4;
    const int ntile = a.B * a.tilesX * a.tilesY;
    const int H = a.H, W = a.W;

    s16x4 wA[4];
#pragma unroll
    for (int n = 0; n < 4; ++n) {
        const int c = 16 * (lx >> 2) + 4 * n + (lx & 3);
        short v[4];
#pragma unroll
        for (int e = 0; e < 4; ++e) {
            const int k = 4 * kg + e;
            v[e] = k < 9 ? __builtin_bit_cast(short, a.w[c * 9 + k]) : (short)0;
        }
        wA[n] = s16x4{v[0], v[1], v[2], v[3]};
    }
    int toff[4];
#pragma unroll
    for (int e = 0; e < 4; ++e) {
        const int k = 4 * kg + e;
        toff[e] = k < 9 ? (k / 3) * ST_PITCH + (k % 3) : -1;
    }
    const int c0 = 16 * kg;
    const int woff = lx < 9 ? (lx / 3) * ST_PITCH + (lx % 3) + 4 * kg : -1;

    float r_a[16], r_s[16], r_b[16], r_k[16];
#pragma unroll
    for (int i = 0; i < 16; ++i) { r_a[i] = r_s[i] = r_b[i] = r_k[i] = 0.f; }
    if constexpr (MODE == 1 || MODE == 2) {
#pragma unroll
        for (int i = 0; i < 16; ++i) {
            r_a[i] = a.scale[c0 + i]; r_s[i] = a.shift[c0 + i];
            if (MODE == 2) { r_b[i] = a.mean[c0 + i]; r_k[i] = a.rstd[c0 + i]; }
        }
    }
    if constexpr (MODE == 3) {
        if (tid < ST_C) {
            const float sc = a.scale[tid];
            const float b_ = -sc * a.rstd[tid] * a.dgamma[tid] * a.inv_n;
            cf[0][tid] = sc;
            cf[1][tid] = a.shift[tid];
            cf[2][tid] = b_;
            cf[3][tid] = -sc * a.dbeta[tid] * a.inv_n - b_ * a.mean[tid];
        }
    }

    constexpr int NACC = MODE == 3 ? 1 : (MODE == 1 ? 1 : 2);
    float acc[NACC][16];
#pragma unroll
    for (int k = 0; k < NACC; ++k)
#pragma unroll
        for (int i = 0; i < 16; ++i) acc[k][i] = 0.f;
    float pv[16];
#pragma unroll
    for (int i = 0; i < 16; ++i) pv[i] = 0.f;
    bool have_pivot = false;
    float cnt = 0.f;

    unsigned short xr[2];
    auto fetch_halo = [&](int tile_) {
        int t = tile_;
        const int txt = t % a.tilesX; t /= a.tilesX;
        const int tyt = t % a.tilesY;
        const int b = t / a.tilesY;
        const int y0 = tyt * ST_TILE, x0p = txt * ST_TILE;
#pragma unroll
        for (int k = 0; k < 2; ++k) {
            const int q = tid + k * 256;
            const int hy = q / ST_HALO, hx = q - hy * ST_HALO;
            const int gy = y0 - 1 + hy, gx = x0p - 1 + hx;
            const bool in = q < ST_HALO * ST_HALO && gy >= 0 && gy < H && gx >= 0 && gx < W;
            const int gyc = min(max(gy, 0), H - 1), gxc = min(max(gx, 0), W - 1);
            const unsigned short v = __builtin_bit_cast(unsigned short, a.x[(int64_t)((b * H + gyc) * W + gxc) * a.ldx]);
            xr[k] = in ? v : (unsigned short)0;
        }
    };
    if ((int)blockIdx.x < ntile) fetch_halo(blockIdx.x);

    for (int tile = blockIdx.x; tile < ntile; tile += gridDim.x) {
        int t = tile;
        const int txt = t % a.tilesX; t /= a.tilesX;
        const int tyt = t % a.tilesY;
        const int b = t / a.tilesY;
        const int y0 = tyt * ST_TILE, x0p = txt * ST_TILE;
        const int vy = min(ST_TILE, H - y0), vx = min(ST_TILE, W - x0p);
        u32x4 draw[4][2];
        if constexpr (MODE >= 2) {
#pragma unroll
            for (int rr = 0; rr < 4; ++rr) {
                const int gp = (b * H + y0 + min(4 * wave + rr, vy - 1)) * W + x0p + min(lx, vx - 1);
                const bf16_t* dp = a.dz + (int64_t)gp * a.lddz + c0;
                draw[rr][0] = *reinterpret_cast<const u32x4*>(dp);
                draw[rr][1] = *reinterpret_cast<const u32x4*>(dp + 8);
            }
        }
        __syncthreads();
#pragma unroll
        for (int k = 0; k < 2; ++k) {
            const int q = tid + k * 256;
            if (q < ST_HALO * ST_HALO) xs[(q / ST_HALO) * ST_PITCH + (q % ST_HALO)] = xr[k];
        }
        __syncthreads();
        if (tile + (int)gridDim.x < ntile) fetch_halo(tile + gridDim.x);

        auto do_row = [&](auto rr_c) {
            constexpr int rr = decltype(rr_c)::value;
            const int ty = 4 * wave + rr;
            const bool in = ty < vy && lx < vx;
            const int gpix = (b * H + y0 + min(ty, vy - 1)) * W + x0p + min(lx, vx - 1);
            const int base = ty * ST_PITCH + lx;
            short bv[4];
#pragma unroll
            for (int e = 0; e < 4; ++e) bv[e] = toff[e] >= 0 ? (short)xs[base + toff[e]] : (short)0;
            const s16x4 bB = {bv[0], bv[1], bv[2], bv[3]};
            float y[16];
#pragma unroll
            for (int n = 0; n < 4; ++n) {
                const f32x4 d = __builtin_amdgcn_mfma_f32_16x16x16bf16_1k(wA[n], bB, f32x4{0.f, 0.f, 0.f, 0.f}, 0, 0, 0);
#pragma unroll
                for (int j = 0; j < 4; ++j) y[4 * n + j] = uh_round_as<bf16_t>(d[j]);
            }
            if constexpr (MODE == 0) {
                if (!have_pivot) {
                    const bool mid = vy > 8 && vx > 8;
                    const int prow = mid ? 8 : 0, pcol = mid ? 8 : 0;
                    if (ty == prow && lx == pcol) {
#pragma unroll
                        for (int i = 0; i < 16; ++i) pivot[c0 + i] = y[i];
                    }
                }
                if (have_pivot && in) {
#pragma unroll
                    for (int i = 0; i < 16; ++i) { const float d = y[i] - pv[i]; acc[0][i] += d; acc[1][i] = fmaf(d, d, acc[1][i]); }
                }
                if (!have_pivot) {
#pragma unroll
// ... 77 lines not shown
            }
        };
        do_row(std::integral_constant<int, 0>{});
        if constexpr (MODE >= 2) __builtin_amdgcn_sched_barrier(0);
        do_row(std::integral_constant<int, 1>{});
        if constexpr (MODE >= 2) __builtin_amdgcn_sched_barrier(0);
        do_row(std::integral_constant<int, 2>{});
        if constexpr (MODE >= 2) __builtin_amdgcn_sched_barrier(0);
        do_row(std::integral_constant<int, 3>{});
        if constexpr (MODE == 0) {
            if (!have_pivot) {
                __syncthreads();
#pragma unroll
                for (int i = 0; i < 16; ++i) pv[i] = pivot[c0 + i];
                have_pivot = true;
#pragma unroll
                for (int rr = 0; rr < 4; ++rr) {
                    const int ty = 4 * wave + rr;
                    if (ty < vy && lx < vx) {
#pragma unroll
                        for (int i = 0; i < 16; ++i) {
                            const float v = rr == 0 ? r_a[i] : (rr == 1 ? r_s[i] : (rr == 2 ? r_b[i] : r_k[i]));
                            const float d = v - pv[i];
                            acc[0][i] += d;
                            acc[1][i] = fmaf(d, d, acc[1][i]);
                        }
                    }
                }
            }
            cnt += (float)(vy * vx);
        }
    }

    if constexpr (MODE == 1) return;
    if constexpr (MODE == 3) {
        __syncthreads();
        if (lx < 9) {
#pragma unroll
            for (int gq = 0; gq < 4; ++gq)
#pragma unroll
                for (int j = 0; j < 4; ++j) red[wave][lx][16 * gq + 4 * kg + j] = acc[0][4 * gq + j];
        }
        __syncthreads();
        float* slab = a.out + (int64_t)blockIdx.x * ST_C * 9;
        for (int idx = tid; idx < 9 * ST_C; idx += 256) {
            const int k = idx / ST_C, c = idx - k * ST_C;
            slab[c * 9 + k] = (red[0][k][c] + red[1][k][c]) + (red[2][k][c] + red[3][k][c]);
        }
        return;
    }
    constexpr int NK = 2;
#pragma unroll
    for (int k = 0; k < NK; ++k)
#pragma unroll
        for (int i = 0; i < 16; ++i) acc[k][i] = uh_row16_sum(acc[k][i]);
    __syncthreads();
    if (lx == 0) {
#pragma unroll
        for (int k = 0; k < NK; ++k)
#pragma unroll
            for (int i = 0; i < 16; ++i) red[wave][k][c0 + i] = acc[k][i];
    }
    __syncthreads();
    if constexpr (MODE == 0) {
        if (tid < ST_C) {
            const float s1 = (red[0][0][tid] + red[1][0][tid]) + (red[2][0][tid] + red[3][0][tid]);
            const float s2 = (red[0][1][tid] + red[1][1][tid]) + (red[2][1][tid] + red[3][1][tid]);
            const float n = cnt > 0.f ? cnt : 1.f;
            const float kk = have_pivot ? pivot[tid] : 0.f;
            a.out[((int64_t)blockIdx.x * 2 + 0) * ST_C + tid] = kk + s1 / n;
            a.out[((int64_t)blockIdx.x * 2 + 1) * ST_C + tid] = fmaxf(s2 - s1 * s1 / n, 0.f);
        }
        float* counts = a.out + (int64_t)ntile * 2 * ST_C;
        if (tid == 0) counts[blockIdx.x] = cnt;
        for (int r = gridDim.x + blockIdx.x * 256 + tid; r < ntile; r += gridDim.x * 256) counts[r] = 0.f;
    } else if constexpr (MODE == 2) {
        for (int idx = tid; idx < 2 * ST_C; idx += 256) {
            const int k = idx / ST_C, c = idx - k * ST_C;
            a.out[((int64_t)blockIdx.x * 2 + k) * ST_C + c] = (red[0][k][c] + red[1][k][c]) + (red[2][k][c] + red[3][k][c]);
        }
    }
}

}

int uh_stem_mfma_launch(int mode, const void* x, int ldx, const void* w, const float* scale, const float* shift,
                                   const float* mean, const float* rstd, const float* dgamma, const float* dbeta, float inv_n,
                                   const void* dz, int lddz, void* z, int ldz, float* out, int B, int H, int W, int grid,
                                   uh_stream stream) {
    StemArgs a;
    a.x = (const bf16_t*)x; a.ldx = ldx; a.w = (const bf16_t*)w;
    a.scale = scale; a.shift = shift; a.mean = mean; a.rstd = rstd; a.dgamma = dgamma; a.dbeta = dbeta; a.inv_n = inv_n;
    a.dz = (const bf16_t*)dz; a.lddz = lddz; a.z = (bf16_t*)z; a.ldz = ldz; a.out = out;
    a.B = B; a.H = H; a.W = W; a.tilesX = (W + ST_TILE - 1) / ST_TILE; a.tilesY = (H + ST_TILE - 1) / ST_TILE;
    hipStream_t st = (hipStream_t)stream;
    switch (mode) {
        case 0: hipLaunchKernelGGL(stem_mfma_kernel<0>, dim3(grid), dim3(256), 0, st, a); break;
        case 1: hipLaunchKernelGGL(stem_mfma_kernel<1>, dim3(grid), dim3(256), 0, st, a); break;
        case 2: hipLaunchKernelGGL(stem_mfma_kernel<2>, dim3(grid), dim3(256), 0, st, a); break;
        case 3: hipLaunchKernelGGL(stem_mfma_kernel<3>, dim3(grid), dim3(256), 0, st, a); break;
        default: uh_set_error("uh_stem_mfma_launch: bad mode %d", mode); return UH_EINVAL;
    }
    UH_CHECK_LAUNCH("stem_mfma_kernel");
    return UH_OK;
}
```

### unet-medical-image-contour-segmentation_amd/csrc/uh_common.h

```cpp
#pragma once
#include <hip/hip_runtime.h>
#include <stdint.h>
#include <stdio.h>
#include <stdarg.h>
#include "unet_hip.h"

typedef __bf16 bf16_t;
typedef __attribute__((ext_vector_type(8))) __bf16 bf16x8;
typedef __attribute__((ext_vector_type(4))) __bf16 bf16x4;
typedef __attribute__((ext_vector_type(4))) float f32x4;
typedef __attribute__((ext_vector_type(4))) unsigned int u32x4;
typedef __attribute__((ext_vector_type(2))) unsigned int u32x2;
typedef __attribute__((ext_vector_type(4))) short s16x4;

#define UH_WAVE 64

void uh_set_error(const char* fmt, ...);
#define UH_REQUIRE(cond, ...)                                   \
    do {                                                        \
        if (!(cond)) {                                          \
            uh_set_error(__VA_ARGS__);                          \
            return UH_EINVAL;                                   \
        }                                                       \
    } while (0)
#define UH_CHECK_LAUNCH(name)                                                         \
    do {                                                                              \
        hipError_t e__ = hipGetLastError();                                           \
        if (e__ != hipSuccess) {                                                      \
            uh_set_error("%s: launch failed: %s", name, hipGetErrorString(e__));      \
            return UH_ELAUNCH;                                                        \
        }                                                                             \
    } while (0)

static inline bool uh_aligned16(const void* p) { return (((uintptr_t)p) & 15) == 0; }

int uh_stem_mfma_launch(int mode, const void* x, int ldx, const void* w, const float* scale, const float* shift, const float* mean,
                        const float* rstd, const float* dgamma, const float* dbeta, float inv_n, const void* dz, int lddz, void* z,
                        int ldz, float* out, int B, int H, int W, int grid, uh_stream stream);

template <typename T> struct uh_traits;
template <> struct uh_traits<float> {
    static constexpr int VEC = 4;
};
template <> struct uh_traits<bf16_t> {
    static constexpr int VEC = 8;
};

__device__ __forceinline__ float uh_bf16_bits_to_f32(unsigned short b) {
    return __uint_as_float(((unsigned int)b) << 16);
}
__device__ __forceinline__ float uh_to_f32(float v) { return v; }
__device__ __forceinline__ float uh_to_f32(bf16_t v) { return (float)v; }
template <typename T> __device__ __forceinline__ T uh_from_f32(float v);
template <> __device__ __forceinline__ float uh_from_f32<float>(float v) { return v; }
template <> __device__ __forceinline__ bf16_t uh_from_f32<bf16_t>(float v) { return (bf16_t)v; }
template <typename T> __device__ __forceinline__ float uh_round_as(float v) { return uh_to_f32(uh_from_f32<T>(v)); }

template <typename T> struct uh_vec16;
template <> struct uh_vec16<float> {
    f32x4 v;
    static constexpr int N = 4;
    __device__ __forceinline__ float get(int i) const { return v[i]; }
    __device__ __forceinline__ void set(int i, float f) { v[i] = f; }
};
template <> struct uh_vec16<bf16_t> {
    bf16x8 v;
    static constexpr int N = 8;
    __device__ __forceinline__ float get(int i) const { return (float)v[i]; }
    __device__ __forceinline__ void set(int i, float f) { v[i] = (bf16_t)f; }
};

// ... 25 lines not shown
```

### unet-medical-image-contour-segmentation_amd/ops.py

```python
from __future__ import annotations

import contextlib
import ctypes
import os
from typing import NamedTuple, Optional, Tuple

import torch
from torch.autograd import Function

from ._lib import LIB, UH_BF16, UH_F32, UH_F32X3, UH_WFRAG, UH_WFRAG_D

BN_EPS_DEFAULT = 1e-5

PROFILE_ON = False
PROFILE = []


def _variant(Cin_split, Cout, esize):
    ck = 64 // esize
    ok = all(c % ck == 0 for c in Cin_split if c) and Cout % 64 == 0
    if ok:
        return "mfma"
    return "stem" if sum(Cin_split) <= 4 else "generic"


class _Timed:
    def __init__(self, name, flops, tag=None):
        self.name, self.flops, self.tag = name, flops, tag

    def __enter__(self):
        if PROFILE_ON:
            self.e0 = torch.cuda.Event(enable_timing=True)
            self.e1 = torch.cuda.Event(enable_timing=True)
            self.e0.record()
        return self

    def __exit__(self, *a):
        if PROFILE_ON:
            self.e1.record()
            PROFILE.append((self.name, self.flops, self.e0, self.e1, self.tag))


def _require_gpu(t: torch.Tensor, what: str = "tensor"):
# ... 49 lines not shown
        return False
    if H > 1 and t.stride(1) != W * ld:
        return False
    if B > 1 and t.stride(0) != H * W * ld:
        return False
    return True


def dense_nhwc(t: torch.Tensor) -> torch.Tensor:
    return t if is_pixel_dense(t) else t.contiguous()


def grad_like(dz: torch.Tensor, ref: torch.Tensor) -> torch.Tensor:
    return dense_nhwc(dz if dz.dtype == ref.dtype else dz.to(ref.dtype))


def to_nhwc(x: torch.Tensor, dtype: Optional[torch.dtype] = None) -> torch.Tensor:
    _require_gpu(x, "input")
    v = x.permute(0, 2, 3, 1)
    if dtype is not None and v.dtype != dtype:
        v = v.to(dtype)
    return dense_nhwc(v)


def to_nchw(x: torch.Tensor) -> torch.Tensor:
    return x.permute(0, 3, 1, 2)


def _empty_like_param(p: torch.Tensor) -> torch.Tensor:
    return torch.empty_strided(p.shape, p.stride(), dtype=torch.float32, device=p.device)


WGRAD_STREAM = None


GRAD_DST = {}


def _grad_buffer(p: torch.Tensor, wanted: bool = True):
    ent = GRAD_DST.get(p.data_ptr()) if wanted else None
    if ent is not None and ent[0].shape == p.shape and ent[0].stride() == p.stride():
        return ent
    return _empty_like_param(p), None


def _is_krsc_dense(w: torch.Tensor) -> bool:
    O, I, kh, kw = w.shape
    return w.stride() == (kh * kw * I, 1, kw * I, I)


FP32_MODE = "exact"


def conv_dt(x: torch.Tensor, C0: int, C1: int, Cout: int, need_dx: bool) -> int:
    if x.dtype == torch.float32 and FP32_MODE == "bf16x3":
        Cin = C0 + C1
        if Cin > 4 and C0 % 16 == 0 and C1 % 16 == 0 and Cout % 64 == 0 and (not need_dx or Cin % 64 == 0):
            return UH_F32X3
    return _dt(x)


WFRAG = True


def conv_flags(cdt: int, frag: bool) -> int:
    return cdt | (UH_WFRAG if frag else 0)
# ... 111 lines not shown
        self.ntiles = toff
        self.table = torch.tensor(rows, dtype=torch.int64).to(dev)
        self.ptrs = [w.data_ptr() for w in self.weights]
        self.strides = [tuple(w.stride()) for w in self.weights]
        self.wf = torch.empty(self.total, dtype=self.dtype, device=dev)
        self.wd = torch.empty(self.total, dtype=self.dtype, device=dev)
        self.versions = [None] * len(self.weights)
        self.index = {p: i for i, p in enumerate(self.ptrs)}

    def refresh(self):
        if any(w.data_ptr() != p or tuple(w.stride()) != st for w, p, st in zip(self.weights, self.ptrs, self.strides)):
            self._build()
        LIB.call("uh_pack_w3x3_batched", self.table.data_ptr(), len(self.weights), self.ntiles, self.wf.data_ptr(),
                 self.wd.data_ptr(), UH_BF16 if self.dtype == torch.bfloat16 else UH_F32, _stream())
        self.versions = [w._version for w in self.weights]
        self.epoch = WEIGHT_EPOCH

    def lookup(self, weight: torch.Tensor, dtype: torch.dtype, frag_f: bool = False, frag_d: bool = False):
        if FP32_MODE != "exact" and dtype == torch.float32:
            return None
        i = self.index.get(weight.data_ptr())
        if i is None or dtype != self.dtype or self.epoch != WEIGHT_EPOCH or self.versions[i] != weight._version \
                or self.strides[i] != tuple(weight.stride()) or self.frags[i] != (bool(frag_f), bool(frag_d)):
            return None
        n = weight.shape[0] * 9 * weight.shape[1]
        o = self.offsets[i]
        return self.wf[o:o + n], self.wd[o:o + n]


WEIGHT_PACK: Optional[ConvWeightPack] = None


def conv3x3_fwd(x0: torch.Tensor, x1: Optional[torch.Tensor], w_packed: torch.Tensor, Cout: int,
                want_stats: bool, dt_code: Optional[int] = None, wfrag: bool = False):
    B, H, W, C0 = x0.shape
    C1 = 0 if x1 is None else x1.shape[3]
    dt = _dt(x0) if dt_code is None else dt_code
    y = torch.empty((B, H, W, Cout), dtype=x0.dtype, device=x0.device)
    stats, nslab = None, 0
    if want_stats:
        nslab = LIB.query("uh_conv3x3_stat_slabs", B, H, W, C0 + C1, Cout, dt)
        stats = torch.empty(nslab * (2 * Cout + 2), dtype=torch.float32, device=x0.device)
    name = "conv3x3_fwd_" + _variant((C0, C1), Cout, x0.element_size())
    with _Timed(name, 2.0 * B * H * W * Cout * 9 * (C0 + C1), ("fwd" if want_stats else "dgrad", B, H, W, C0 + C1, Cout)):
        LIB.call("uh_conv3x3_fwd", x0.data_ptr(), C0, pixel_ld(x0), _p(x1), C1, pixel_ld_or0(x1),
                 w_packed.data_ptr(), y.data_ptr(), Cout, Cout, _p(stats), B, H, W, conv_flags(dt, wfrag), _stream())
    return y, stats, nslab


class SlabBatch:

    def __init__(self, flush_bytes: Optional[int] = None):
        self.flush_bytes = flush_bytes
        self.arena = {}
        self.rows, self.callbacks = [], []
        self.pending_bytes = 0
        self._tables = {}

    def workspace(self, key, nbytes: int, device) -> torch.Tensor:
        ws = self.arena.get(key)
        if ws is None or ws.numel() < nbytes or ws.device != device:
            ws = self.arena[key] = torch.empty(nbytes, dtype=torch.uint8, device=device)
            self._tables.clear()
        return ws

    def add(self, desc, callback):
        self.rows.append(tuple(desc))
        self.callbacks.append(callback)
        self.pending_bytes += 4 * int(desc[2])
        if self.flush_bytes is not None and self.pending_bytes >= self.flush_bytes:
            self.flush()

    def reset(self):
        self.rows, self.callbacks, self.pending_bytes = [], [], 0

    def close(self):
        self.reset()
        self.arena.clear()
        self._tables.clear()
# ... 4 lines not shown
        key = tuple(self.rows)
        entry = self._tables.get(key)
        if entry is None:
            if torch.cuda.is_current_stream_capturing():
                raise RuntimeError("SlabBatch: the reduction table would be built (allocation + host-to-device copy) during graph "
                                   "capture; run one eager step first")
            tab, off = [], 0
            for r in self.rows:
                tab.append([r[0], r[1], r[2], r[3], r[4], r[5], off, r[7]])
                off += r[6]
            dev = next(iter(self.arena.values())).device
            host = torch.tensor(tab, dtype=torch.int64).pin_memory()
            entry = self._tables[key] = (host.to(dev, non_blocking=True), len(tab), off, host)
        table, nrows, blocks = entry[:3]
        with _Timed("slab_reduce_batched", 0.0):
            LIB.call("uh_slab_reduce_batched", table.data_ptr(), nrows, blocks, _stream())
        cbs = self.callbacks
        self.reset()
        for cb in cbs:
            if cb is not None:
                cb(None)


SLAB_BATCH: Optional[SlabBatch] = None
DEFER_SLABS = os.environ.get("UH_DEFER_SLABS", "0") == "1"


def flush_slabs():
    if SLAB_BATCH is not None:
        SLAB_BATCH.flush()


def conv3x3_wgrad(dy: torch.Tensor, x0: torch.Tensor, x1: Optional[torch.Tensor], out_krsc: torch.Tensor,
                  split: bool = False, defer_cb=None) -> bool:
    B, H, W, Cout = dy.shape
    C0 = x0.shape[3]
    C1 = 0 if x1 is None else x1.shape[3]
    dt = _dt(dy)
    nbytes = LIB.query("uh_conv3x3_wgrad_ws_bytes", B, H, W, C0 + C1, Cout, dt)
    if split and dt == UH_F32 and C0 % 64 == 0 and C1 % 64 == 0 and Cout % 64 == 0:
        dt = UH_F32X3
    name = "conv3x3_wgrad_" + ("mfma" if (C0 % 64 == 0 and C1 % 64 == 0 and Cout % 64 == 0) else
                                ("stem" if C0 + C1 <= 4 else "generic"))
    batch = SLAB_BATCH if (defer_cb is not None and DEFER_SLABS and name == "conv3x3_wgrad_mfma") else None
    timed = _Timed(name, 2.0 * B * H * W * Cout * 9 * (C0 + C1), ("wgrad", B, H, W, C0 + C1, Cout))
    if batch is not None:
        ws = batch.workspace(out_krsc.data_ptr(), nbytes, dy.device)
        desc = (ctypes.c_int64 * 8)()
        with timed:
            LIB.call("uh_conv3x3_wgrad_partials", dy.data_ptr(), pixel_ld(dy), x0.data_ptr(), C0, pixel_ld(x0), _p(x1), C1,
                     pixel_ld_or0(x1), out_krsc.data_ptr(), Cout, ws.data_ptr(), nbytes, B, H, W, dt,
                     ctypes.addressof(desc), _stream())
        if desc[3] == 0:
            return False
        batch.add(list(desc), defer_cb)
        return True
    ws = torch.empty(nbytes, dtype=torch.uint8, device=dy.device)
    with timed:
        LIB.call("uh_conv3x3_wgrad", dy.data_ptr(), pixel_ld(dy), x0.data_ptr(), C0, pixel_ld(x0), _p(x1), C1,
                 pixel_ld_or0(x1), out_krsc.data_ptr(), Cout, ws.data_ptr(), nbytes, B, H, W, dt, _stream())
    return False


def conv3x3_wgrad_pre(dy: torch.Tensor, x0_raw: torch.Tensor, pre_coef: torch.Tensor, out_krsc: torch.Tensor):
    B, H, W, Cout = dy.shape
    C0 = x0_raw.shape[3]
    dt = _dt(dy)
    nbytes = LIB.query("uh_conv3x3_wgrad_ws_bytes", B, H, W, C0, Cout, dt)
    ws = torch.empty(nbytes, dtype=torch.uint8, device=dy.device)
    with _Timed("conv3x3_wgrad_mfma", 2.0 * B * H * W * Cout * 9 * C0):
        LIB.call("uh_conv3x3_wgrad_pre", dy.data_ptr(), pixel_ld(dy), x0_raw.data_ptr(), C0, pixel_ld(x0_raw),
                 pre_coef.data_ptr(), pre_coef[C0:].data_ptr(), out_krsc.data_ptr(), Cout, ws.data_ptr(), nbytes, B, H, W, dt,
                 _stream())


def bench_double_conv(B: int, H: int, W: int, Cin: int, Cout: int, dtype: torch.dtype, iters: int = 20):
    dev = torch.device("cuda", torch.cuda.current_device())
# ... 362 lines not shown

            def apply(part_ptr, nb, dg_ptr, db_ptr, n_total):
                LIB.call("uh_bn_relu_pool_bwd_apply", *sk, *bn_args, part_ptr, nb, dg_ptr, db_ptr, dy.data_ptr(), Cout,
                         B, H, W, n_total, Cout, dt, _stream())
        else:
            dz = grads[0]
            if dz is None:
                return _grads_for(_CBR_INPUTS)
            dz = grad_like(dz, y)
            if tail == TAIL_UP:
                Ho, Wo, pt, pl = ctx.up
                du, dz = dz, torch.empty((B, H, W, Cout), dtype=y.dtype, device=dev)
                LIB.call("uh_upsample2x_bwd", du.data_ptr(), pixel_ld(du), dz.data_ptr(), Cout, B, H, W, Cout, Ho, Wo, pt, pl,
                         dt, _stream())
            link = ctx.bnsum_pub
            if link is not None:
                if link.partials is not None and link.dz is not None and dz.data_ptr() == link.dz.data_ptr() and \
                        dz.shape == link.dz.shape and dz.stride() == link.dz.stride() and dz._version == link.dz_version:
                    partials, nblk = link.partials, link.rows
                else:
                    link = None
                ctx.bnsum_pub.partials = ctx.bnsum_pub.dz = ctx.bnsum_pub.y = ctx.bnsum_pub.coef = None
            if link is None:
                LIB.call("uh_bn_relu_bwd_reduce", dz.data_ptr(), pixel_ld(dz), *bn_args, partials.data_ptr(), n, Cout, dt, _stream())

            def apply(part_ptr, nb, dg_ptr, db_ptr, n_total):
                LIB.call("uh_bn_relu_bwd_apply", dz.data_ptr(), pixel_ld(dz), *bn_args, part_ptr, nb, dg_ptr, db_ptr,
                         dy.data_ptr(), Cout, n, n_total, Cout, dt, _stream())
        bn_wanted = (need["gamma"], need["beta"])
        bn_bufs = [_grad_buffer(p, w) for p, w in zip(ctx.bn_params, bn_wanted)]
        dy = torch.empty_like(y)
        _bn_backward_finish(partials, nblk, Cout, bn_bufs[0][0], bn_bufs[1][0], ctx.sync_bn, ctx.n_total, apply)
        dx0 = dx1 = None
        if wd is not None and (need["x0"] or need["x1"]):
            use, rows = ctx.bnsum_use, 0
            if use is not None and use.y is not None and use.y.shape == (B, H, W, Cin) and use.y.is_contiguous() and \
                    (H, Cin) not in BNSUM_OFF:
                rows = LIB.query("uh_conv3x3_dgrad_bnsum_rows", B, H, W, Cout, Cin, Cout, Cin, Cin, ctx.cdt)
            if rows > 0:
                dx = torch.empty((B, H, W, Cin), dtype=dy.dtype, device=dev)
                bsum = torch.empty(rows * 2 * Cin, dtype=torch.float32, device=dev)
                with _Timed("conv3x3_dgrad_bnsum_mfma", 2.0 * B * H * W * Cin * 9 * Cout, ("dgrad", B, H, W, Cout, Cin)):
                    LIB.call("uh_conv3x3_dgrad_bnsum", dy.data_ptr(), Cout, Cout, wd.data_ptr(), dx.data_ptr(), Cin, Cin,
                             use.y.data_ptr(), Cin, use.coef.data_ptr(), bsum.data_ptr(), B, H, W,
                             conv_flags(ctx.cdt, ctx.frag_d), _stream())
                use.partials, use.rows, use.dz, use.dz_version = bsum, rows, dx, dx._version
            else:
                dx, _, _ = conv3x3_fwd(dy, None, wd, Cin, False, ctx.cdt, ctx.frag_d)
            dx0 = dx[..., :C0] if need["x0"] else None
            dx1 = dx[..., C0:] if (x1 is not None and need["x1"]) else None
        dweight = side_done = None

        def run_wgrad(out_, defer_cb=None):
            if pre_coef is None:
                return conv3x3_wgrad(dy, x0, x1, out_, ctx.cdt == UH_F32X3, defer_cb)
            conv3x3_wgrad_pre(dy, x0, pre_coef, out_)
            return False

        if need["weight"]:
            dweight, cb_w = _grad_buffer(weight)
            if cb_w is not None and WGRAD_STREAM is not None and _is_krsc_dense(weight):
                side = WGRAD_STREAM
                ev = torch.cuda.Event()
                ev.record()
                side.wait_event(ev)
                with torch.cuda.stream(side):
                    run_wgrad(dweight)
                    side_done = torch.cuda.Event()
                    side_done.record()
                for t_ in (dy, x0, x1, pre_coef):
                    if t_ is not None:
                        t_.record_stream(side)
            elif _is_krsc_dense(weight):
                if run_wgrad(dweight, cb_w):
                    cb_w = None
                    dweight = None
            else:
                dwk = torch.empty(Cout * 9 * Cin, dtype=torch.float32, device=dev)
                run_wgrad(dwk)
                _unpack_dw3x3(dwk, dweight)
            if cb_w is not None:
                cb_w(side_done)
                dweight = None
        dgamma, dbeta = _bn_param_grads(bn_bufs, bn_wanted)
        return _grads_for(_CBR_INPUTS, x0=dx0, x1=dx1, weight=dweight, gamma=dgamma, beta=dbeta, head_w=dhead[0], head_b=dhead[1])


STEM_RECOMPUTE = os.environ.get("UH_STEM_RECOMPUTE", "1") != "0"
STEM_RECOMPUTE_MAX_CIN = 1


def stem_recompute_ok(x0: torch.Tensor, Cin: int, Cout: int) -> bool:
    return bool(STEM_RECOMPUTE and x0.dtype == torch.bfloat16 and Cin <= STEM_RECOMPUTE_MAX_CIN and x0.shape[-1] == Cin and
                LIB.query("uh_stem_ok", Cin, Cout, UH_BF16) and x0.shape[0] * x0.shape[1] * x0.shape[2] < 2 ** 31)


class StemConvBnReluFn(Function):

    @staticmethod
    def forward(ctx, x0, weight, gamma, beta, running_mean, running_var, num_batches_tracked, momentum: float, eps: float):
# ... 883 lines not shown
```

### unet-medical-image-contour-segmentation_amd/train.py

```python
from __future__ import annotations

import contextlib
import dataclasses
import math
import os
import weakref
from typing import Dict, Iterable, Optional, Union

import torch
import torch.nn as nn

from . import dp as dpmod
from . import ops
from ._lib import LIB


def _add_surface(terms: Dict[str, torch.Tensor], lg: torch.Tensor, true_masks: torch.Tensor, n_classes: int, weight: float,
                 classes, reduce_sums, world) -> Dict[str, torch.Tensor]:
    from .utils.surface_loss import head_classes
    weighted, value = ops.SurfaceLossFn.apply(lg, true_masks, 2 if n_classes == 1 else 1, head_classes(n_classes, classes),
                                              float(weight), reduce_sums, world)
    terms["loss"] = terms["loss"] + weighted
    terms["surface"] = value
    terms.pop("nan_flag", None)
# ... 400 lines not shown
        if flag is None or cc_loss:
            flag = torch.isnan(loss.detach()).reshape(1).float()
        probe = None
        if reduce_sums is not None:
            probe = optimizer.pattern_probe() if isinstance(optimizer, FusedRMSprop) else None
            if probe is not None:
                flag = torch.cat([flag.reshape(1), probe])
            flag = reduce_sums(flag)
        nan_host = _pinned_flag(loss.device, flag.numel())
        nan_host.copy_(flag, non_blocking=True)
        nan_event = torch.cuda.Event()
        nan_event.record()
    optimizer.zero_grad(set_to_none=True)
    loss.backward(gradient=_one_like(loss))
    ops.flush_slabs()
    if nan_event is not None:
        nan_event.synchronize()
        host = nan_host.tolist()
        if len(host) == 3:
            optimizer.check_probe(host[1], host[2], optimizer.sync.world)
        if host[0] > 0:
            if isinstance(optimizer, FusedRMSprop):
                optimizer.abort_step()
            raise RuntimeError("Fatal: NaN loss detected!")
    if isinstance(optimizer, FusedRMSprop):
        terms["grad_norm"] = optimizer.step()
    else:
        terms["grad_norm"] = torch.nn.utils.clip_grad_norm_(model.parameters(), gradient_clipping)
        optimizer.step()
    terms["logits"] = masks_pred.detach()
    return terms


class TrainStepper:

    def __init__(self, model: nn.Module, lr: float = 1e-5, weight_decay: float = 1e-8, momentum: float = 0.999,
                 gradient_clipping: float = 1.0, amp: bool = True, process_group=None, check_nan: bool = True,
                 wgrad_stream: Optional[bool] = None, cc_loss: bool = False, sync_bn: bool = False, fp32_mode: str = "exact",
                 surface_weight: float = 0.0, surface_classes=None, ema: Union[None, str, EmaConfig] = None):
        self.model = model
        self.ema = EmaConfig.of(ema)
        self._averaged = False
        self.surface_weight = float(surface_weight)
        self.surface_classes = surface_classes
        self._side_auto = wgrad_stream is None
        env = os.environ.get("UH_SIDE_STREAM")
        if self._side_auto and env in ("0", "1"):
            wgrad_stream, self._side_auto = (env == "1"), False
        want = wgrad_stream is None or bool(wgrad_stream)
        self.wgrad_stream = torch.cuda.Stream(priority=-1) if (want and torch.cuda.is_available()) else None
        self.amp = amp
        self.check_nan = check_nan
        if fp32_mode not in ("exact", "bf16x3"):
            raise ValueError("fp32_mode must be 'exact' or 'bf16x3'")
        self.fp32_mode = fp32_mode
        self.cc_loss = cc_loss
        self.group = process_group
        self.world = dpmod.world_size(process_group)
        self.reduce_sums = dpmod.make_sum_reducer(process_group)
        self.sync_bn = None
        self.bn_group = None
        if sync_bn and dpmod.sync_enabled(process_group):
            import torch.distributed as dist
            group = process_group
            if os.environ.get("UH_SYNCBN_OWN_GROUP") == "1":
                ranks = dist.get_process_group_ranks(process_group) if process_group is not None else list(range(dist.get_world_size()))
                self.bn_group = group = dist.new_group(ranks=ranks)
            self.sync_bn = (group, self.world)
        self.optimizer = FusedRMSprop(model.parameters(), lr=lr, weight_decay=weight_decay, momentum=momentum,
                                      gradient_clipping=gradient_clipping, process_group=process_group,
                                      **({} if self.ema is None else {"ema_decay": self.ema.decay, "ema_warmup": self.ema.warmup}))
        self._pack = None
        sync = self.optimizer.sync
        self._slabs = ops.SlabBatch(flush_bytes=None if sync is None else 8 << 20)

    def close(self):
        opt = getattr(self, "optimizer", None)
        if opt is not None:
            opt.close()
        grp, self.bn_group = getattr(self, "bn_group", None), None
        if grp is not None:
            import torch.distributed as dist
            self.sync_bn = None
            if dist.is_initialized():
                dist.destroy_process_group(grp)

    def __del__(self):
        try:
            if getattr(self, "bn_group", None) is not None:
                self.close()
        except Exception:
            pass

    @contextlib.contextmanager
    def averaged(self):
        if self.ema is None:
            raise RuntimeError("TrainStepper.averaged() needs ema=...")
        if self._averaged:
            raise RuntimeError("TrainStepper.averaged() is already active (it does not nest)")
        self.optimizer.swap_ema()
        self._averaged = True
        try:
            yield self.model
        finally:
            self.optimizer.swap_ema()
            self._averaged = False

    def _refuse_averaged(self):
        if self._averaged:
            raise RuntimeError("TrainStepper.step() inside averaged(): the model holds the averaged weights")

    def ema_state_dict(self) -> Dict[str, torch.Tensor]:
        if self.ema is None:
            raise RuntimeError("TrainStepper.ema_state_dict() needs ema=...")
        opt = self.optimizer
        src = opt.flat_p if self._averaged else opt.flat_ema
        base, size = opt.flat_p.data_ptr(), opt.flat_p.numel() * 4
        out = {}
        for k, v in self.model.state_dict().items():
            off = v.data_ptr() - base
            if 0 <= off < size and v.dtype == torch.float32:
                v = torch.as_strided(src, v.shape, v.stride(), off // 4)
            out[k] = v.detach().to("cpu", copy=True)
        return out

    SIDE_MIN_PIXELS = 1 << 20

    def _side_for(self, images):
        if self.wgrad_stream is None or not self._side_auto:
            return self.wgrad_stream
        if self.sync_bn is not None and self.bn_group is None:
            return None
        big = images.is_cuda and images.shape[0] * images.shape[-2] * images.shape[-1] >= self.SIDE_MIN_PIXELS
        return self.wgrad_stream if (self.amp and big) else None

    def step(self, images, true_masks, global_batch: Optional[int] = None):
        self._refuse_averaged()
        self.model.train()
        side = self._side_for(images)
        ops.WGRAD_STREAM = side
        ops.SYNC_BN = self.sync_bn
        ops.SYNC_BN_BATCH = None
        world = self.world
        if self.sync_bn is not None:
            lb = int(images.shape[0])
            gb = int(global_batch) if global_batch is not None else dpmod.global_batch(lb, self.group, images.device)
            ops.SYNC_BN_BATCH = (gb, lb)
            world = gb / lb
        fp32_mode_before, ops.FP32_MODE = ops.FP32_MODE, self.fp32_mode
        dt = torch.bfloat16 if self.amp else getattr(self.model, "compute_dtype", torch.float32)
        if self._pack is None or self._pack.dtype != dt:
            ws = [m.weight for m in self.model.modules() if isinstance(m, nn.Conv2d) and m.kernel_size == (3, 3)]
            self._pack = ops.ConvWeightPack(ws, dt) if ws and all(w.is_cuda for w in ws) else None
        if self._pack is not None:
            ops.WEIGHT_PACK = self._pack
            self._pack.refresh()
        self._slabs.reset()
        ops.SLAB_BATCH = self._slabs if side is None else None
        try:
            return train_step(self.model, self.optimizer, images, true_masks, amp=self.amp,
                              reduce_sums=self.reduce_sums, world=world, check_nan=self.check_nan, cc_loss=self.cc_loss,
                              surface_weight=self.surface_weight, surface_classes=self.surface_classes)
        finally:
            ops.SLAB_BATCH = None
            ops.FP32_MODE = fp32_mode_before


class GraphedTrainStepper(TrainStepper):

    def __init__(self, model: nn.Module, *args, warmup: int = 2, **kw):
        kw.setdefault("wgrad_stream", False)
        super().__init__(model, *args, **kw)
        if self.world != 1:
            raise RuntimeError("GraphedTrainStepper is single-process; use TrainStepper with torch.distributed")
        if self.cc_loss:
            raise RuntimeError("connected_component_loss returns a Python float (a device read-back every step): not capturable")
        self._refuse_surface()
        self._warmup = max(1, warmup)
        self._graph = None
        self._key = None

    def _refuse_surface(self):
        if self.surface_weight:
            raise RuntimeError("GraphedTrainStepper does not capture the surface loss (surface_weight must be 0): use TrainStepper")

    def _eager_step(self, images, masks):
        self.model.train()
        side = self._side_for(images)
        ops.WGRAD_STREAM = side
        ops.SYNC_BN = None
        fp32_mode_before, ops.FP32_MODE = ops.FP32_MODE, self.fp32_mode
        dt = torch.bfloat16 if self.amp else getattr(self.model, "compute_dtype", torch.float32)
        if self._pack is None or self._pack.dtype != dt:
            ws = [m.weight for m in self.model.modules() if isinstance(m, nn.Conv2d) and m.kernel_size == (3, 3)]
            self._pack = ops.ConvWeightPack(ws, dt) if ws and all(w.is_cuda for w in ws) else None
        if self._pack is not None:
            ops.WEIGHT_PACK = self._pack
# ... 104 lines not shown
```

Measured before the change: 880.5 images/sec.

## Add CU-budget grid capping with persistent conv loop for side-stream wgrad overlap

Adds a grid-cap flag encoded in the dtype word so the forward/dgrad MFMA conv kernel can run as a persistent grid-stride loop over logical workgroups, reading its parameters from the kernarg segment each iteration. The Python side can now split compute units between the main-stream dgrad and the side-stream wgrad, using an env override or a per-size table. The default table entries give a zero budget, so by default the launch grid stays uncapped. What still runs is the restructured kernel: a loop wrapper and kernarg reloads whose per-iteration overhead could change register use or scheduling.

```diff
diff --git a/include/unet_hip.h b/include/unet_hip.h
--- a/include/unet_hip.h
+++ b/include/unet_hip.h
@@ -12,7 +12,9 @@
 
 enum { UH_F32 = 0, UH_BF16 = 1,
        UH_F32X3 = 2,
-       UH_WFRAG = 0x100, UH_WFRAG_D = 0x200 };
+       UH_WFRAG = 0x100, UH_WFRAG_D = 0x200,
+       UH_GRID_CAP_SHIFT = 16, UH_GRID_CAP_MASK = 0x0fff0000 };
+#define UH_GRID_CAP(cus) ((((cus) + 1) << UH_GRID_CAP_SHIFT) & UH_GRID_CAP_MASK)
 enum { UH_OK = 0, UH_EINVAL = -1, UH_ELAUNCH = -2, UH_EWORKSPACE = -3 };
 
 const char* uh_last_error(void);
@@ -32,6 +34,7 @@
 int uh_conv3x3_fwd_kernel_plan(int B, int plan_B, int H, int W, int C0, int C1, int Cout, int dt);
 int uh_conv3x3_wfrag_ok_plan(int B, int plan_B, int H, int W, int C0, int C1, int Cout, int ld0, int ld1, int ldy, int dt);
 int uh_conv3x3_fwd_sum_class(int kernel);
+int uh_conv3x3_fwd_grid(int B, int H, int W, int C0, int C1, int Cout, int dt, int bsum, int64_t* out);
 int uh_conv3x3_fwd(const void* x0, int C0, int ld0, const void* x1, int C1, int ld1,
                    const void* w, void* y, int ldy, int Cout, float* stat_partials,
                    int B, int H, int W, int dt, uh_stream stream);
diff --git a/scratch/cu_share_collect.py b/scratch/cu_share_collect.py
--- /dev/null
+++ b/scratch/cu_share_collect.py
@@ -0,0 +1,18 @@
+import glob, json, re, statistics, sys
+out = sys.argv[1]
+res = {}
+for f in sorted(glob.glob(out + "/b*_W*_r*.log")):
+    m = re.search(r"b(\d)_W(\d+)_r(\d)\.log", f)
+    line = [l for l in open(f) if l.startswith("{")]
+    if not line:
+        continue
+    j = json.loads(line[-1])
+    res.setdefault((int(m.group(1)), int(m.group(2))), []).append(float(j["value"]))
+table = {}
+for (b, w), v in sorted(res.items()):
+    table[f"b{b}_W{w}"] = {"values": v, "median": statistics.median(v), "spread": max(v) - min(v)}
+    print(f"batch {b} W {w:3d}: " + " ".join(f"{x:7.1f}" for x in v) + f"   median {statistics.median(v):7.1f} spread {max(v) - min(v):5.1f}")
+json.dump(table, open(out + "/sweep.json", "w"), indent=1)
+b8 = {w: statistics.median(v) for (b, w), v in res.items() if b == 8}
+best = max(b8, key=b8.get)
+print("best W at batch 8:", best)
diff --git a/unet-medical-image-contour-segmentation_amd/_lib.py b/unet-medical-image-contour-segmentation_amd/_lib.py
--- a/unet-medical-image-contour-segmentation_amd/_lib.py
+++ b/unet-medical-image-contour-segmentation_amd/_lib.py
@@ -12,6 +12,13 @@
 
 UH_F32, UH_BF16, UH_F32X3 = 0, 1, 2
 UH_WFRAG, UH_WFRAG_D = 0x100, 0x200
+UH_GRID_CAP_SHIFT, UH_GRID_CAP_MASK = 16, 0x0fff0000
+
+
+def grid_cap_flag(cus: int) -> int:
+    if not 0 <= cus <= 4094:
+        raise ValueError(f"CU budget {cus} outside 0..4094")
+    return ((cus + 1) << UH_GRID_CAP_SHIFT) if cus else 0
 
 _CTYPES = {
     "int": ctypes.c_int, "int64_t": ctypes.c_int64, "float": ctypes.c_float, "double": ctypes.c_double,
diff --git a/unet-medical-image-contour-segmentation_amd/csrc/conv3x3.hip b/unet-medical-image-contour-segmentation_amd/csrc/conv3x3.hip
--- a/unet-medical-image-contour-segmentation_amd/csrc/conv3x3.hip
+++ b/unet-medical-image-contour-segmentation_amd/csrc/conv3x3.hip
@@ -489,23 +489,26 @@
 #define UH_BUILD_PRE 0
 #endif
 constexpr int PRE_MAX_C = 512;
+struct FwdV2Params {
+    const void* x0; int C0, ld0; const void* x1; int C1, ld1; const void* w; void* y; int ldy, Cout; float* stats;
+    int B, H, W, tilesX, tilesY; unsigned x0_bytes, x1_bytes, y_bytes; const float *ep_scale, *ep_shift; int C0v, C1v, Coutv, wfrag;
+    const float *pre_scale, *pre_shift; const void* bs_y; int bs_ld; unsigned bs_bytes; const float* bs_coef; int nwg;
+};
 template <typename T, int NBW, bool SPLIT = false, bool WRES = false, bool PRE = false, bool BSUM = false, int KS = 1>
 __global__ __launch_bounds__(256 * KS, ((NBW == 1 && !WRES && !BSUM && KS == 1) ? 3 : 2)) void conv3x3_fwd_mfma_v2(
-    const T* __restrict__ x0, int C0, int ld0, const T* __restrict__ x1, int C1, int ld1,
-    const T* __restrict__ w, T* __restrict__ y, int ldy, int Cout, float* __restrict__ stats,
-    int B, int H, int W, int tilesX, int tilesY, unsigned x0_bytes, unsigned x1_bytes, unsigned y_bytes,
-    const float* __restrict__ ep_scale, const float* __restrict__ ep_shift, int C0v, int C1v, int Coutv, int wfrag,
-    const float* __restrict__ pre_scale = nullptr, const float* __restrict__ pre_shift = nullptr,
-    const T* __restrict__ bs_y = nullptr, int bs_ld = 0, unsigned bs_bytes = 0, const float* __restrict__ bs_coef = nullptr) {
+    const T* x0_, int C0_, int ld0_, const T* x1_, int C1_, int ld1_,
+    const T* w_, T* y_, int ldy_, int Cout_, float* stats_,
+    int B_, int H_, int W_, int tilesX_, int tilesY_, unsigned x0_bytes_, unsigned x1_bytes_, unsigned y_bytes_,
+    const float* ep_scale_, const float* ep_shift_, int C0v_, int C1v_, int Coutv_, int wfrag_,
+    const float* pre_scale_ = nullptr, const float* pre_shift_ = nullptr,
+    const T* bs_y_ = nullptr, int bs_ld_ = 0, unsigned bs_bytes_ = 0, const float* bs_coef_ = nullptr,
+    int nwg_ = 0) {
+    (void)x0_; (void)C0_; (void)ld0_; (void)x1_; (void)C1_; (void)ld1_; (void)w_; (void)y_; (void)ldy_; (void)Cout_; (void)stats_; (void)B_; (void)H_;
+    (void)W_; (void)tilesX_; (void)tilesY_; (void)x0_bytes_; (void)x1_bytes_; (void)y_bytes_; (void)ep_scale_; (void)ep_shift_; (void)C0v_;
+    (void)C1v_; (void)Coutv_; (void)wfrag_; (void)pre_scale_; (void)pre_shift_; (void)bs_y_; (void)bs_ld_; (void)bs_bytes_; (void)bs_coef_; (void)nwg_;
     static_assert(!PRE || (sizeof(T) == 2 && !SPLIT), "PRE is the bf16 training path");
     static_assert(!BSUM || (sizeof(T) == 2 && !SPLIT && !PRE), "BSUM is the bf16 backward-data path");
     static_assert(KS == 1 || (KS == 2 && sizeof(T) == 2 && NBW == 1 && !SPLIT && !WRES && !PRE), "KS = 2 is a bf16 NBW = 1 form");
-    if constexpr (BSUM) {
-        x1 = nullptr; C1 = 0; ld1 = 0; x1_bytes = 0;
-        C0v = C0; C1v = 0; Coutv = Cout;
-        ep_scale = nullptr; ep_shift = nullptr;
-        bs_ld = ldy; bs_bytes = y_bytes;
-    }
     constexpr int ES = sizeof(T);
     constexpr int CK = 64 / ES;
     constexpr int VEC = 16 / ES;
@@ -519,25 +522,49 @@
     __shared__ float wg_sum[3][BN];
     __shared__ __attribute__((aligned(16))) float pre_tab[PRE ? 2 * PRE_MAX_C : 4];
     __shared__ __attribute__((aligned(16))) float bs_tab[BSUM ? 4 * BN : 4];
-    float n_run = 0.f;
-
-    const int tid = threadIdx.x & 255;
+
+    typedef const __attribute__((address_space(4))) FwdV2Params* KP;
+    for (int wg = blockIdx.x;;) {
+    KP kp = (KP)__builtin_amdgcn_kernarg_segment_ptr();
+    asm volatile("" : "+s"(kp));
+    const T* __restrict__ x0 = (const T*)kp->x0; int C0 = kp->C0, ld0 = kp->ld0;
+    const T* __restrict__ x1 = (const T*)kp->x1; int C1 = kp->C1, ld1 = kp->ld1;
+    const T* __restrict__ w = (const T*)kp->w; T* __restrict__ y = (T*)kp->y; int ldy = kp->ldy, Cout = kp->Cout;
+    float* __restrict__ stats = kp->stats;
+    const int B = kp->B, H = kp->H, W = kp->W, tilesX = kp->tilesX, tilesY = kp->tilesY;
+    unsigned x0_bytes = kp->x0_bytes, x1_bytes = kp->x1_bytes, y_bytes = kp->y_bytes;
+    const float* __restrict__ ep_scale = kp->ep_scale; const float* __restrict__ ep_shift = kp->ep_shift;
+    int C0v = kp->C0v, C1v = kp->C1v, Coutv = kp->Coutv; const int wfrag = kp->wfrag;
+    const float* __restrict__ pre_scale = kp->pre_scale; const float* __restrict__ pre_shift = kp->pre_shift;
+    const T* __restrict__ bs_y = (const T*)kp->bs_y; int bs_ld = kp->bs_ld; unsigned bs_bytes = kp->bs_bytes;
+    const float* __restrict__ bs_coef = kp->bs_coef; const int nwg = kp->nwg;
+    do {
+    if constexpr (BSUM) {
+        x1 = nullptr; C1 = 0; ld1 = 0; x1_bytes = 0;
+        C0v = C0; C1v = 0; Coutv = Cout;
+        ep_scale = nullptr; ep_shift = nullptr;
+        bs_ld = ldy; bs_bytes = y_bytes;
+    }
+    int tix = threadIdx.x;
+    asm volatile("" : "+v"(tix));
+    const int tid = tix & 255;
     const int lane = tid & 63;
-    const int wave_all = __builtin_amdgcn_readfirstlane((int)(threadIdx.x >> 6));
+    const int wave_all = __builtin_amdgcn_readfirstlane(tix >> 6);
     const int wave = wave_all & 3;
     const int grp = KS == 2 ? (wave_all >> 2) : 0;
     unsigned char* const lds = lds_all + grp * (2 * HALO2_STRIDE);
     const int lx = lane & 15, kg = lane >> 4;
+    float n_run = 0.f;
     const int nslab = Cout / BN;
-    const int nlanes = gridDim.x / nslab;
+    const int nlanes = nwg / nslab;
     int tile_lane, slab;
     if ((nlanes & 7) == 0) {
-        const int xcd = blockIdx.x & 7, jj = blockIdx.x >> 3;
+        const int xcd = wg & 7, jj = wg >> 3;
         slab = jj % nslab;
         tile_lane = (jj / nslab) * 8 + xcd;
     } else {
-        slab = blockIdx.x / nlanes;
-        tile_lane = blockIdx.x - slab * nlanes;
+        slab = wg / nlanes;
+        tile_lane = wg - slab * nlanes;
     }
     const int co_blk = slab * BN;
     const int Cin = C0 + C1;
@@ -711,7 +738,7 @@
     };
 
     int tile = tile_lane;
-    if (tile >= ntile) return;
+    if (tile >= ntile) continue;
     WFrag wA[3][NBW], wB[3][NBW], wC[3][NBW];
 #pragma unroll
     for (int r = 0; r < 3; ++r)
@@ -875,7 +902,7 @@
                     for (int n = 0; n < NBW; ++n) scratch[(i * NBW + n) * 256 + tid] = acc[i][n];
             }
             __syncthreads();
-            if (grp == 1) return;
+            if (grp == 1) break;
 #pragma unroll
             for (int i = 0; i < 16; ++i)
 #pragma unroll
@@ -1175,6 +1202,7 @@
             n_run += (float)(vy * vx);
         }
     }
+    if (KS == 2 && grp == 1) continue;
     if constexpr (BSUM) {
         if (lx == 0) {
 #pragma unroll
@@ -1186,7 +1214,7 @@
                     stats[((int64_t)tile_lane * 2 + 1) * Cout + co_blk + cl] = wg_sum[1][cl] * bs_tab[3 * BN + cl];
                 }
         }
-        return;
+        continue;
     }
     if (stats) {
         if (lx == 0) {
@@ -1207,6 +1235,13 @@
             if (tile_lane == 0)
                 for (int r = nlanes + tid; r < ntile; r += 256) counts[r] = 0.f;
         }
+    }
+    } while (0);
+    KP kq = (KP)__builtin_amdgcn_kernarg_segment_ptr();
+    asm volatile("" : "+s"(kq));
+    wg += gridDim.x;
+    if (wg >= kq->nwg) break;
+    __syncthreads();
     }
 }
 
@@ -1625,10 +1660,22 @@
     int slabs, lanes;
     int threads;
     bool split, pre, bsum;
+    int per_cu = 0;
+    int grid = 0;
 };
 
+static int grid_cap_of(int& dt) {
+    const int cap = (dt & UH_GRID_CAP_MASK) >> UH_GRID_CAP_SHIFT;
+    dt &= ~UH_GRID_CAP_MASK;
+    return cap;
+}
+static int capped_grid(int64_t logical, int cap, int per_cu) {
+    const int64_t g = cap > 0 ? (int64_t)(cap - 1) * per_cu : logical;
+    return (int)(g < logical ? g : logical);
+}
+
 static FwdPlan fwd_plan(int es, int B, int H, int W, int C0, int C1, int Cout, int ld0, int ld1, int ldy, bool ptrs16, bool y16,
-                        bool split, bool narrow, bool pre, bool bsum, int plan_B = 0) {
+                        bool split, bool narrow, bool pre, bool bsum, int plan_B = 0, int grid_cap = 0) {
     const int tiles1 = ((H + TILE - 1) / TILE) * ((W + TILE - 1) / TILE);
     const int ntile = B * tiles1;
     const int ck = 64 / es, Cin = C0 + C1;
@@ -1667,18 +1714,20 @@
         if (fwd_sum_class(pinned) != fwd_sum_class(p.kernel)) p.kernel = pinned;
     }
     switch (p.kernel) {
-    case FWD_SLAB128: p.slabs = Cout / 128; p.lanes = lanes_for(2, p.slabs); break;
-    case FWD_WRES: p.slabs = Cout / 64; p.lanes = lanes_for(2, p.slabs); break;
-    case FWD_KSPLIT: p.slabs = Cout / 64; p.lanes = ntile; p.threads = 512; break;
-    default: p.slabs = Cout / 64; p.lanes = lanes_for(bsum ? 2 : 3, p.slabs); break;
-    }
+    case FWD_SLAB128: p.slabs = Cout / 128; p.per_cu = 2; break;
+    case FWD_WRES: p.slabs = Cout / 64; p.per_cu = 2; break;
+    case FWD_KSPLIT: p.slabs = Cout / 64; p.per_cu = 1; p.threads = 512; break;
+    default: p.slabs = Cout / 64; p.per_cu = bsum ? 2 : 3; break;
+    }
+    p.lanes = p.kernel == FWD_KSPLIT ? ntile : lanes_for(p.per_cu, p.slabs);
+    p.grid = capped_grid((int64_t)p.lanes * p.slabs, grid_cap, p.per_cu);
     return p;
 }
 
 template <typename T, bool SPLIT, bool PRE, bool BSUM, typename... Args>
 static void fwd_v2_form(const FwdPlan& p, hipStream_t st, Args... args) {
     constexpr bool BF16 = sizeof(T) == 2 && !SPLIT;
-    const dim3 grid(p.lanes * p.slabs), block(p.threads);
+    const dim3 grid(p.grid), block(p.threads);
     switch (p.kernel) {
     case FWD_SLAB128: hipLaunchKernelGGL((conv3x3_fwd_mfma_v2<T, 2, SPLIT, false, PRE, BSUM>), grid, block, 0, st, args...); break;
     case FWD_WRES:
@@ -1711,6 +1760,7 @@
     int C0 = 0, ld0 = 0, C1 = 0, ld1 = 0, Cout = 0, B = 0, H = 0, W = 0;
     int dt = UH_F32;
     bool wfrag = false;
+    int grid_cap = 0;
     int C0v = -1, C1v = -1, Coutv = -1;
     const float *pre_scale = nullptr, *pre_shift = nullptr;
     hipStream_t st = nullptr;
@@ -1735,6 +1785,7 @@
     UH_REQUIRE(c.ld0 >= (narrow ? c.C0v : c.C0) && ldo >= (narrow ? c.Coutv : c.Cout) &&
                (c.C1 == 0 || (c.x1 && c.ld1 >= (narrow ? c.C1v : c.C1))), "%s: bad strides", fn);
     UH_REQUIRE((int64_t)c.B * c.H * c.W < (1ll << 31), "%s: pixel count overflows int32", fn);
+    c.grid_cap = grid_cap_of(dt);
     c.wfrag = (flags & CK_WFRAG) && (dt & UH_WFRAG);
     if (flags & CK_WFRAG) dt &= ~UH_WFRAG;
     UH_REQUIRE(!(flags & CK_BF16_ONLY) || dt == UH_BF16, "%s: bf16 only (dtype %d)", fn, dt);
@@ -1758,7 +1809,10 @@
     const int tilesX = (c.W + TILE - 1) / TILE, tilesY = (c.H + TILE - 1) / TILE;
     const int Cin = c.C0 + c.C1;
     const bool ptrs16 = uh_aligned16(x0) && (c.C1 == 0 || uh_aligned16(x1)) && uh_aligned16(w) && uh_aligned16(y);
-    const FwdPlan p = fwd_plan(ES, c.B, c.H, c.W, c.C0, c.C1, c.Cout, c.ld0, c.ld1, c.ldy, ptrs16, uh_aligned16(y), split, narrow, pre, bsum, c.plan_B);
+    const FwdPlan p = fwd_plan(ES, c.B, c.H, c.W, c.C0, c.C1, c.Cout, c.ld0, c.ld1, c.ldy, ptrs16, uh_aligned16(y), split, narrow, pre, bsum, c.plan_B, c.grid_cap);
+    UH_REQUIRE(c.grid_cap == 0 || (p.kernel != FWD_SIMT && p.kernel != FWD_LARGE),
+               "conv3x3_fwd: a CU budget (UH_GRID_CAP) needs the LDS-DMA MFMA kernel; this call takes another one");
+    UH_REQUIRE(c.grid_cap == 0 || p.grid > 0, "conv3x3_fwd: the CU budget (UH_GRID_CAP) leaves this launch no workgroup");
     if (p.kernel != FWD_SIMT && p.kernel != FWD_LARGE) {
         if (ep_scale && !(uh_aligned16(ep_scale) && uh_aligned16(ep_shift))) ep_scale = ep_shift = nullptr;
         UH_REQUIRE(!split || ES == 4, "conv3x3_fwd: bf16x3 needs fp32 tensors");
@@ -1777,7 +1831,7 @@
         }
         fwd_v2_launch<T>(p, c.st, x0, c.C0, c.ld0, x1, c.C1, c.ld1, w, y, c.ldy, c.Cout, c.stats, c.B, c.H, c.W, tilesX, tilesY, (unsigned)(px * c.ld0 * ES),
                          (unsigned)(c.C1 ? px * c.ld1 * ES : 0), (unsigned)(px * c.ldy * ES), ep_scale, ep_shift, C0v, C1v, Coutv,
-                         c.wfrag ? 1 : 0, c.pre_scale, c.pre_shift, bs_y, c.bs_ld, (unsigned)bq, c.bs_coef);
+                         c.wfrag ? 1 : 0, c.pre_scale, c.pre_shift, bs_y, c.bs_ld, (unsigned)bq, c.bs_coef, p.lanes * p.slabs);
         UH_CHECK_LAUNCH(pre ? "conv3x3_fwd_mfma_v2 (BatchNorm+ReLU input)"
                             : bsum ? "conv3x3_fwd_mfma_v2 (backward-data + BatchNorm sums)" : "conv3x3_fwd_mfma_v2");
         c.ep_done = ep_scale != nullptr;
@@ -1882,6 +1936,19 @@
                     false, plan_B).kernel;
 }
 
+extern "C" int uh_conv3x3_fwd_grid(int B, int H, int W, int C0, int C1, int Cout, int dt, int bsum, int64_t* out) {
+    const int cap = grid_cap_of(dt);
+    UH_REQUIRE(out && B > 0 && H > 0 && W > 0 && C0 > 0 && C1 >= 0 && Cout > 0, "uh_conv3x3_fwd_grid: null pointer or bad shape");
+    UH_REQUIRE(dt == UH_F32 || dt == UH_BF16 || dt == UH_F32X3, "uh_conv3x3_fwd_grid: bad dtype %d", dt);
+    const FwdPlan p = fwd_plan(dt == UH_BF16 ? 2 : 4, B, H, W, C0, C1, Cout, C0, C1, Cout, true, true, dt == UH_F32X3, false, false,
+                               bsum != 0, 0, cap);
+    const bool v2 = p.kernel != FWD_SIMT && p.kernel != FWD_LARGE;
+    UH_REQUIRE(cap == 0 || v2, "uh_conv3x3_fwd_grid: a CU budget (UH_GRID_CAP) needs the LDS-DMA MFMA kernel; this shape takes kernel %d", (int)p.kernel);
+    UH_REQUIRE(!v2 || p.grid > 0, "uh_conv3x3_fwd_grid: the CU budget (UH_GRID_CAP) leaves this launch no workgroup");
+    out[0] = p.kernel; out[1] = (int64_t)p.lanes * p.slabs; out[2] = v2 ? p.grid : out[1]; out[3] = p.per_cu;
+    return UH_OK;
+}
+
 extern "C" int uh_conv3x3_fwd_sum_class(int kernel) {
     UH_REQUIRE(kernel >= FWD_SIMT && kernel <= FWD_LARGE, "uh_conv3x3_fwd_sum_class: bad kernel code %d", kernel);
     return fwd_sum_class(kernel);
@@ -1963,7 +2030,7 @@
     c.C0v = C0v; c.C1v = C1v; c.Coutv = Coutv; c.plan_B = plan_B;
     const int rc = conv3x3_fwd_call("uh_conv3x3_fwd_narrow", c, dt, CK_NARROW);
     if (rc != UH_OK || !scale || c.ep_done) return rc;
-    return uh_bn_relu_apply(y, ldy, scale, shift, y, ldy, (int64_t)B * H * W, Coutv, dt == UH_BF16 ? UH_BF16 : UH_F32, stream);
+    return uh_bn_relu_apply(y, ldy, scale, shift, y, ldy, (int64_t)B * H * W, Coutv, c.dt == UH_BF16 ? UH_BF16 : UH_F32, stream);
 }
 
 extern "C" int uh_conv3x3_fwd_narrow(const void* x0, int C0, int C0v, int ld0, const void* x1, int C1, int C1v, int ld1,
@@ -1984,7 +2051,8 @@
 __global__ __launch_bounds__(256, 2) void conv3x3_wgrad_mfma(
     const T* __restrict__ dy, int lddy, const T* __restrict__ x0, int C0, int ld0, const T* __restrict__ x1, int C1,
     int ld1, float* __restrict__ slabs, int Cout, int B, int H, int W, int tilesX, int tilesY, int nsplit,
-    int C0v, int C1v, int Coutv) {
+    int C0v, int C1v, int Coutv,
+    int nlanes) {
     constexpr int ES = sizeof(T);
     constexpr int TH = WgradCfg<T>::TH;
     constexpr int PB = 64 * ES;
@@ -2000,7 +2068,10 @@
     const int wr = wave >> 1, wc = wave & 1;
     const int Cin = C0 + C1;
     const int nci = Cin / 64;
-    const int cot = blockIdx.y / nci, cit = blockIdx.y - cot * nci;
+    const int lane0 = blockIdx.y * gridDim.x + blockIdx.x, lane_step = gridDim.x * gridDim.y;
+    for (int wlane = lane0; wlane < nlanes; wlane += lane_step) {
+    const int ytile = wlane / nsplit;
+    const int cot = ytile / nci, cit = ytile - cot * nci;
     const int co0 = cot * 64, ci0 = cit * 64;
     const T* xsrc; int ldx;
     int xleft;
@@ -2009,7 +2080,7 @@
     const int dleft = Coutv - co0;
 
     const int ntile = B * tilesX * tilesY;
-    const int split = blockIdx.x;
+    const int split = wlane - ytile * nsplit;
     const int t_begin = (int)(((int64_t)ntile * split) / nsplit);
     const int t_end = (int)(((int64_t)ntile * (split + 1)) / nsplit);
 
@@ -2199,6 +2270,7 @@
             int co = co0 + wr * 32 + (reg & 3) + 8 * (reg >> 2) + 4 * (lane >> 5);
             slab[((int64_t)co * 9 + tap) * Cin + ci] = acc[tap][reg];
         }
+    }
 }
 
 __device__ __forceinline__ void slab_reduce_block_f32(const float* __restrict__ slabs, float* __restrict__ out, int64_t n,
@@ -2368,13 +2440,33 @@
         });
 }
 
+struct WgradV2Params {
+    const void* dy; int lddy; const void* x0; int C0, ld0; const void* x1; int C1, ld1; float* slabs;
+    int Cout, B, H, W, tilesX, tilesY, nsplit; unsigned dy_bytes, x_bytes; int C0v, C1v, Coutv, nlanes;
+    const float *pre_scale, *pre_shift;
+};
 template <typename T, int NWR, bool PRE = false, bool SLAB16 = false>
 __global__ __launch_bounds__(128 * NWR, 2) void conv3x3_wgrad_mfma_v2(
-    const T* __restrict__ dy, int lddy, const T* __restrict__ x0, int C0, int ld0, const T* __restrict__ x1, int C1,
-    int ld1, float* __restrict__ slabs, int Cout, int B, int H, int W, int tilesX, int tilesY, int nsplit,
-    unsigned dy_bytes, unsigned x_bytes, int C0v, int C1v, int Coutv, const float* __restrict__ pre_scale = nullptr,
-    const float* __restrict__ pre_shift = nullptr) {
+    const T* dy_, int lddy_, const T* x0_, int C0_, int ld0_, const T* x1_, int C1_,
+    int ld1_, float* slabs_, int Cout_, int B_, int H_, int W_, int tilesX_, int tilesY_, int nsplit_,
+    unsigned dy_bytes_, unsigned x_bytes_, int C0v_, int C1v_, int Coutv_, int nlanes_, const float* pre_scale_ = nullptr,
+    const float* pre_shift_ = nullptr) {
     static_assert(sizeof(T) == 2, "v2 is the bf16 kernel");
+    (void)dy_; (void)lddy_; (void)x0_; (void)C0_; (void)ld0_; (void)x1_; (void)C1_; (void)ld1_; (void)slabs_; (void)Cout_; (void)B_; (void)H_;
+    (void)W_; (void)tilesX_; (void)tilesY_; (void)nsplit_; (void)dy_bytes_; (void)x_bytes_; (void)C0v_; (void)C1v_; (void)Coutv_; (void)nlanes_;
+    (void)pre_scale_; (void)pre_shift_;
+    typedef const __attribute__((address_space(4))) WgradV2Params* KP;
+    for (int wlane = blockIdx.y * gridDim.x + blockIdx.x;;) {
+    KP kp = (KP)__builtin_amdgcn_kernarg_segment_ptr();
+    asm volatile("" : "+s"(kp));
+    const T* __restrict__ dy = (const T*)kp->dy; const int lddy = kp->lddy;
+    const T* __restrict__ x0 = (const T*)kp->x0; const int C0 = kp->C0, ld0 = kp->ld0;
+    const T* __restrict__ x1 = (const T*)kp->x1; const int C1 = kp->C1, ld1 = kp->ld1;
+    float* __restrict__ slabs = kp->slabs;
+    const int Cout = kp->Cout, B = kp->B, H = kp->H, W = kp->W, tilesX = kp->tilesX, tilesY = kp->tilesY, nsplit = kp->nsplit;
+    const unsigned dy_bytes = kp->dy_bytes, x_bytes = kp->x_bytes;
+    const int C0v = kp->C0v, C1v = kp->C1v, Coutv = kp->Coutv, nlanes = kp->nlanes;
+    const float* __restrict__ pre_scale = kp->pre_scale; const float* __restrict__ pre_shift = kp->pre_shift;
     constexpr int TH = 8;
     constexpr int NT = 128 * NWR;
     constexpr int PB = 128;
@@ -2389,12 +2481,15 @@
     constexpr int XBYTES = XR * RB, STAGE = XBYTES + DR * RB;
     __shared__ __attribute__((aligned(16))) unsigned char lds[2 * STAGE];
 
-    const int tid = threadIdx.x, lane = tid & 63;
+    int tid = threadIdx.x;
+    asm volatile("" : "+v"(tid));
+    const int lane = tid & 63;
     const int wave = __builtin_amdgcn_readfirstlane(tid >> 6);
     const int wr = wave >> 1, wc = wave & 1;
     const int Cin = C0 + C1;
     const int nci = Cin / 64;
-    const int cot = blockIdx.y / nci, cit = blockIdx.y - cot * nci;
+    const int ytile = wlane / nsplit, nytile = nlanes / nsplit;
+    const int cot = ytile / nci, cit = ytile - cot * nci;
     const int co0 = cot * (32 * NWR), ci0 = cit * 64;
     const T* xsrc; int ldx;
     int xleft;
@@ -2405,7 +2500,7 @@
     const unsigned lds_base = (unsigned)(uintptr_t)(__attribute__((address_space(3))) unsigned char*)lds;
 
     const int ntile = B * tilesX * tilesY;
-    const int split = blockIdx.x;
+    const int split = wlane - ytile * nsplit;
     const int t_begin = (int)(((int64_t)ntile * split) / nsplit);
     const int t_end = (int)(((int64_t)ntile * (split + 1)) / nsplit);
 
@@ -2677,7 +2772,7 @@
         unsigned* slab16 = reinterpret_cast<unsigned*>(slabs) + (int64_t)split * (Cout / 2) * 9 * Cin;
         if (tid == 0) {
             float* inv = reinterpret_cast<float*>(reinterpret_cast<unsigned*>(slabs) + (int64_t)nsplit * (Cout / 2) * 9 * Cin);
-            inv[(int64_t)split * gridDim.y + blockIdx.y] = __uint_as_float((eb - 14u) << 23);
+            inv[(int64_t)split * nytile + ytile] = __uint_as_float((eb - 14u) << 23);
         }
 #pragma unroll
         for (int tap = 0; tap < 9; ++tap)
@@ -2692,8 +2787,7 @@
                         const f16x2 pr = {(_Float16)(acc[tap][h][hh][jp] * sc), (_Float16)(acc[tap][h][hh][jp + 1] * sc)};
                         slab16[((int64_t)(co >> 1) * 9 + tap) * Cin + ci] = __builtin_bit_cast(unsigned, pr);
                     }
-        return;
-    }
+    } else {
     float* slab = slabs + (int64_t)split * Cout * 9 * Cin;
 #pragma unroll
     for (int tap = 0; tap < 9; ++tap)
@@ -2707,6 +2801,13 @@
                     const int ci = ci0 + wc * 32 + hh * 16 + (lane & 15);
                     slab[((int64_t)co * 9 + tap) * Cin + ci] = acc[tap][h][hh][j];
                 }
+    }
+    KP kq = (KP)__builtin_amdgcn_kernarg_segment_ptr();
+    asm volatile("" : "+s"(kq));
+    wlane += gridDim.x * gridDim.y;
+    if (wlane >= kq->nlanes) break;
+    __syncthreads();
+    }
 }
 
 __global__ void slab_reduce_scalar_kernel(const float* __restrict__ slabs, float* __restrict__ out, int64_t n, int nsplit) {
@@ -3013,6 +3114,7 @@
     int tilesX, tilesY;
     int nsplit;
     dim3 grid;
+    dim3 launch;
     int threads;
     bool slab16, pre;
     SlabReduce reduce;
@@ -3022,12 +3124,12 @@
 static size_t wgrad_slab_bytes(const WgradPlan& p) { return (size_t)p.nsplit * p.reduce.n * sizeof(float); }
 
 static WgradPlan wgrad_plan(int es, int B, int H, int W, int C0, int C1, int Cout, int ld0, int ld1, int lddy, WgradAlign a16,
-                            bool narrow, bool pre) {
+                            bool narrow, bool pre, int grid_cap = 0) {
     static const bool slab_f32 = getenv("UH_WGRAD_SLAB_F32") != nullptr && getenv("UH_WGRAD_SLAB_F32")[0] == '1';
     static_assert(WgradCfg<bf16_t>::TH == WgradCfg<float>::TH, "one pixel-tile height for both element types");
     const int Cin = C0 + C1;
     const int64_t n = (int64_t)Cout * 9 * Cin;
-    WgradPlan p = {WG_GENERIC, 0, 0, 0, dim3(Cout * 9), 256, false, pre, {SR_NONE, n, 0, 0, 9 * Cin, 0}};
+    WgradPlan p = {WG_GENERIC, 0, 0, 0, dim3(Cout * 9), dim3(Cout * 9), 256, false, pre, {SR_NONE, n, 0, 0, 9 * Cin, 0}};
     const bool dy_ok = a16.dy && (lddy * es) % 16 == 0;
     int nwr = 2;
     if (a16.ptrs && dy_ok && (ld0 * es) % 16 == 0 && (C1 == 0 || (ld1 * es) % 16 == 0) && C0 % 64 == 0 && Cin % 64 == 0 && Cout % 64 == 0) {
@@ -3041,6 +3143,7 @@
         const int want = ((nwr == 4 ? 256 : 512) + ctiles - 1) / ctiles;
         p.nsplit = want < 1 ? 1 : (want > ntile ? ntile : want);
         p.grid = dim3(p.nsplit, ctiles); p.threads = 128 * nwr;
+        p.launch = grid_cap > 0 ? dim3(capped_grid((int64_t)p.nsplit * ctiles, grid_cap, nwr == 4 ? 1 : 2)) : p.grid;
         p.slab16 = dma && a16.dw && !slab_f32;
     } else if (Cin <= 4 && C1 == 0) {
         p.tilesX = (W + TILE - 1) / TILE; p.tilesY = (H + TILE - 1) / TILE;
@@ -3049,6 +3152,7 @@
         if (es == 2 && Cout == 64 && dy_ok) { p.kernel = WG_STEM_V3; p.grid = dim3(p.nsplit, Cin); }
         else if (Cout % (16 / es) == 0 && dy_ok) { p.kernel = WG_STEM_V2; p.grid = dim3(p.nsplit, 1, Cin); }
         else { p.kernel = WG_STEM; p.grid = dim3(p.nsplit, (Cout + 63) / 64); }
+        p.launch = p.grid;
     } else
         return p;
     p.reduce = slab_reduce_plan(n, p.nsplit, 9 * Cin, 32 * nwr, p.slab16, a16.dw && a16.ws, false);
@@ -3064,9 +3168,12 @@
 
 extern "C" int uh_conv3x3_wgrad_plan(int B, int H, int W, int C0, int C1, int Cout, int dt, int narrow, int64_t* out) {
     UH_REQUIRE(out && B > 0 && H > 0 && W > 0 && C0 > 0 && C1 >= 0 && Cout > 0, "uh_conv3x3_wgrad_plan: null pointer or bad shape");
+    const int cap = grid_cap_of(dt);
     UH_REQUIRE(dt == UH_F32 || dt == UH_BF16 || dt == UH_F32X3, "uh_conv3x3_wgrad_plan: bad dtype %d", dt);
-    const WgradPlan p = wgrad_plan(dt == UH_BF16 ? 2 : 4, B, H, W, C0, C1, Cout, C0, C1, Cout, WG_ALIGNED, narrow != 0, false);
-    out[0] = p.kernel; out[1] = p.nsplit; out[2] = p.grid.x; out[3] = p.grid.y; out[4] = p.threads; out[5] = p.slab16 ? 1 : 0;
+    const WgradPlan p = wgrad_plan(dt == UH_BF16 ? 2 : 4, B, H, W, C0, C1, Cout, C0, C1, Cout, WG_ALIGNED, narrow != 0, false, cap);
+    UH_REQUIRE(cap == 0 || p.kernel >= WG_MFMA, "uh_conv3x3_wgrad_plan: a CU budget (UH_GRID_CAP) needs an MFMA kernel; this shape takes kernel %d", (int)p.kernel);
+    UH_REQUIRE(p.launch.x > 0, "uh_conv3x3_wgrad_plan: the CU budget (UH_GRID_CAP) leaves this launch no workgroup");
+    out[0] = p.kernel; out[1] = p.nsplit; out[2] = p.launch.x; out[3] = p.launch.y; out[4] = p.threads; out[5] = p.slab16 ? 1 : 0;
     out[6] = p.reduce.kernel; out[7] = p.reduce.blocks;
     return UH_OK;
 }
@@ -3077,10 +3184,10 @@
         constexpr bool PRE = decltype(pre)::value;
         const dim3 block(p.threads);
         switch ((p.kernel == WG_DMA128 ? 2 : 0) + (p.slab16 ? 1 : 0)) {
-        case 3: hipLaunchKernelGGL((conv3x3_wgrad_mfma_v2<T, 4, PRE, true>), p.grid, block, 0, st, args...); break;
-        case 2: hipLaunchKernelGGL((conv3x3_wgrad_mfma_v2<T, 4, PRE, false>), p.grid, block, 0, st, args...); break;
-        case 1: hipLaunchKernelGGL((conv3x3_wgrad_mfma_v2<T, 2, PRE, true>), p.grid, block, 0, st, args...); break;
-        default: hipLaunchKernelGGL((conv3x3_wgrad_mfma_v2<T, 2, PRE, false>), p.grid, block, 0, st, args...); break;
+        case 3: hipLaunchKernelGGL((conv3x3_wgrad_mfma_v2<T, 4, PRE, true>), p.launch, block, 0, st, args...); break;
+        case 2: hipLaunchKernelGGL((conv3x3_wgrad_mfma_v2<T, 4, PRE, false>), p.launch, block, 0, st, args...); break;
+        case 1: hipLaunchKernelGGL((conv3x3_wgrad_mfma_v2<T, 2, PRE, true>), p.launch, block, 0, st, args...); break;
+        default: hipLaunchKernelGGL((conv3x3_wgrad_mfma_v2<T, 2, PRE, false>), p.launch, block, 0, st, args...); break;
         }
     };
     if (p.pre) {
@@ -3106,8 +3213,11 @@
     const int C0v = narrow ? c.C0v : c.C0, C1v = narrow ? c.C1v : c.C1, Coutv = narrow ? c.Coutv : c.Cout;
     const WgradAlign a16 = {uh_aligned16(dy) && uh_aligned16(x0) && (c.C1 == 0 || uh_aligned16(x1)), uh_aligned16(dy), uh_aligned16(c.dw),
                             uh_aligned16(slabs)};
-    const WgradPlan p = wgrad_plan(ES, c.B, c.H, c.W, c.C0, c.C1, c.Cout, c.ld0, c.ld1, c.lddy, a16, narrow, pre);
+    const WgradPlan p = wgrad_plan(ES, c.B, c.H, c.W, c.C0, c.C1, c.Cout, c.ld0, c.ld1, c.lddy, a16, narrow, pre, c.grid_cap);
     const bool mfma = p.kernel >= WG_MFMA, dma = p.kernel >= WG_DMA64;
+    const int nlanes = (int)(p.grid.x * p.grid.y);
+    UH_REQUIRE(c.grid_cap == 0 || mfma, "uh_conv3x3_wgrad: a CU budget (UH_GRID_CAP) needs an MFMA kernel; this call takes another one");
+    UH_REQUIRE(p.launch.x > 0, "uh_conv3x3_wgrad: the CU budget (UH_GRID_CAP) leaves this launch no workgroup");
     UH_REQUIRE(!narrow || mfma, "uh_conv3x3_wgrad_narrow: needs the MFMA path (padded channel counts multiples of 64, 16-byte strides)");
     UH_REQUIRE(!split || mfma, "uh_conv3x3_wgrad: bf16x3 needs an MFMA-aligned shape (channel counts multiples of 64, 16-byte strides)");
     UH_REQUIRE(!pre || UH_BUILD_PRE, "uh_conv3x3_wgrad_pre: the consumer-side BatchNorm+ReLU instantiations are not in this build (UH_BUILD_PRE=1); uh_conv3x3_pre_ok says so");
@@ -3127,18 +3237,18 @@
     case WG_DMA64: case WG_DMA128:
         if constexpr (ES == 2)
             wgrad_v2_launch<T>(p, c.st, dy, c.lddy, x0, c.C0, c.ld0, x1, c.C1, c.ld1, slabs, c.Cout, c.B, c.H, c.W, p.tilesX, p.tilesY, p.nsplit,
-                               (unsigned)(px * c.lddy * 2), (unsigned)(px * (c.ld0 > c.ld1 ? c.ld0 : c.ld1) * 2), C0v, C1v, Coutv, c.pre_scale,
+                               (unsigned)(px * c.lddy * 2), (unsigned)(px * (c.ld0 > c.ld1 ? c.ld0 : c.ld1) * 2), C0v, C1v, Coutv, nlanes, c.pre_scale,
                                c.pre_shift);
         UH_CHECK_LAUNCH("conv3x3_wgrad_mfma_v2");
         break;
     case WG_MFMA:
         if (split) {
             if constexpr (ES == 4)
-                hipLaunchKernelGGL((conv3x3_wgrad_mfma<T, true>), p.grid, block, 0, c.st, dy, c.lddy, x0, c.C0, c.ld0, x1, c.C1, c.ld1, slabs, c.Cout,
-                                   c.B, c.H, c.W, p.tilesX, p.tilesY, p.nsplit, C0v, C1v, Coutv);
+                hipLaunchKernelGGL((conv3x3_wgrad_mfma<T, true>), p.launch, block, 0, c.st, dy, c.lddy, x0, c.C0, c.ld0, x1, c.C1, c.ld1, slabs, c.Cout,
+                                   c.B, c.H, c.W, p.tilesX, p.tilesY, p.nsplit, C0v, C1v, Coutv, nlanes);
         } else
-            hipLaunchKernelGGL(conv3x3_wgrad_mfma<T>, p.grid, block, 0, c.st, dy, c.lddy, x0, c.C0, c.ld0, x1, c.C1, c.ld1, slabs, c.Cout, c.B, c.H, c.W,
-                               p.tilesX, p.tilesY, p.nsplit, C0v, C1v, Coutv);
+            hipLaunchKernelGGL(conv3x3_wgrad_mfma<T>, p.launch, block, 0, c.st, dy, c.lddy, x0, c.C0, c.ld0, x1, c.C1, c.ld1, slabs, c.Cout, c.B, c.H, c.W,
+                               p.tilesX, p.tilesY, p.nsplit, C0v, C1v, Coutv, nlanes);
         UH_CHECK_LAUNCH("conv3x3_wgrad_mfma");
         break;
     case WG_STEM_V3:
@@ -3226,7 +3336,7 @@
     UH_STEM_COMMON("uh_stem_stats");
     UH_REQUIRE(stat_partials, "uh_stem_stats: null statistics buffer");
     return uh_stem_mfma_launch(0, x, ldx, w, nullptr, nullptr, nullptr, nullptr, nullptr, nullptr, 0.f, nullptr, 0, nullptr, 0,
-                               stat_partials, B, H, W, uh_stem_nblk(B, H, W), stream);
+                               stat_partials, B, H, W, uh_stem_nblk(B, H, W), uh_stem_nblk(B, H, W), stream);
 }
 
 extern "C" int uh_stem_bn_relu_fwd(const void* x, int Cin, int ldx, const void* w, const float* scale, const float* shift, void* z,
@@ -3235,7 +3345,7 @@
     UH_REQUIRE(scale && shift && z && ldz >= 64, "uh_stem_bn_relu_fwd: null pointer / bad stride");
     UH_REQUIRE(uh_aligned16(z) && (ldz * 2) % 16 == 0, "uh_stem_bn_relu_fwd: z must be 16-byte aligned with a 16-byte pixel pitch");
     return uh_stem_mfma_launch(1, x, ldx, w, scale, shift, nullptr, nullptr, nullptr, nullptr, 0.f, nullptr, 0, z, ldz, nullptr, B, H, W,
-                               uh_stem_nblk(B, H, W), stream);
+                               uh_stem_nblk(B, H, W), uh_stem_nblk(B, H, W), stream);
 }
 
 extern "C" int uh_stem_bn_relu_bwd_reduce(const void* dz, int lddz, const void* x, int Cin, int ldx, const void* w,
@@ -3245,7 +3355,7 @@
     UH_REQUIRE(dz && scale && shift && mean && rstd && partials && lddz >= 64, "uh_stem_bn_relu_bwd_reduce: null pointer / bad stride");
     UH_REQUIRE(uh_aligned16(dz) && (lddz * 2) % 16 == 0, "uh_stem_bn_relu_bwd_reduce: dz must be 16-byte aligned with a 16-byte pixel pitch");
     return uh_stem_mfma_launch(2, x, ldx, w, scale, shift, mean, rstd, nullptr, nullptr, 0.f, dz, lddz, nullptr, 0, partials, B, H, W,
-                               uh_stem_nblk(B, H, W), stream);
+                               uh_stem_nblk(B, H, W), uh_stem_nblk(B, H, W), stream);
 }
 
 extern "C" size_t uh_stem_bwd_wgrad_ws_bytes(int B, int H, int W, int Cin) {
@@ -3256,6 +3366,8 @@
                                          const float* scale, const float* shift, const float* mean, const float* rstd,
                                          const float* dgamma, const float* dbeta, int64_t n_total, float* dw_krsc, void* ws,
                                          size_t ws_bytes, int B, int H, int W, int dt, uh_stream stream) {
+    const int cap = grid_cap_of(dt), nblk = uh_stem_nblk(B, H, W), grid = capped_grid(nblk, cap, 4);
+    UH_REQUIRE(grid > 0, "uh_stem_bn_relu_bwd_wgrad: the CU budget (UH_GRID_CAP) leaves this launch no workgroup");
     UH_STEM_COMMON("uh_stem_bn_relu_bwd_wgrad");
     UH_REQUIRE(dz && scale && shift && mean && rstd && dgamma && dbeta && dw_krsc && ws && lddz >= 64,
                "uh_stem_bn_relu_bwd_wgrad: null pointer / bad stride");
@@ -3264,7 +3376,7 @@
     const float inv_n = (float)(1.0 / (double)(n_total > 0 ? n_total : (int64_t)B * H * W));
     float* slabs = (float*)ws;
     const int rc = uh_stem_mfma_launch(3, x, ldx, w, scale, shift, mean, rstd, dgamma, dbeta, inv_n, dz, lddz, nullptr, 0, slabs, B, H, W,
-                                       uh_stem_nblk(B, H, W), stream);
+                                       nblk, grid, stream);
     if (rc != UH_OK) return rc;
     return slab_reduce_launch(slab_reduce_plan((int64_t)64 * 9 * Cin, uh_stem_nblk(B, H, W), 9 * Cin, 64, false,
                                                uh_aligned16(dw_krsc) && uh_aligned16(slabs), true), slabs, dw_krsc, (hipStream_t)stream);
diff --git a/unet-medical-image-contour-segmentation_amd/csrc/stem_mfma.hip b/unet-medical-image-contour-segmentation_amd/csrc/stem_mfma.hip
--- a/unet-medical-image-contour-segmentation_amd/csrc/stem_mfma.hip
+++ b/unet-medical-image-contour-segmentation_amd/csrc/stem_mfma.hip
@@ -15,6 +15,7 @@
     bf16_t* z; int ldz;
     float* out;
     int B, H, W, tilesX, tilesY;
+    int nlanes;
 };
 
 template <int MODE>
@@ -72,6 +73,8 @@
         }
     }
 
+    const int nlanes = a.nlanes;
+    for (int wlane = blockIdx.x; wlane < nlanes; wlane += gridDim.x) {
     constexpr int NACC = MODE == 3 ? 1 : (MODE == 1 ? 1 : 2);
     float acc[NACC][16];
 #pragma unroll
@@ -102,9 +105,9 @@
             xr[k] = in ? v : (unsigned short)0;
         }
     };
-    if ((int)blockIdx.x < ntile) fetch_halo(blockIdx.x);
-
-    for (int tile = blockIdx.x; tile < ntile; tile += gridDim.x) {
+    if (wlane < ntile) fetch_halo(wlane);
+
+    for (int tile = wlane; tile < ntile; tile += nlanes) {
         int t = tile;
         const int txt = t % a.tilesX; t /= a.tilesX;
         const int tyt = t % a.tilesY;
@@ -128,7 +131,7 @@
             if (q < ST_HALO * ST_HALO) xs[(q / ST_HALO) * ST_PITCH + (q % ST_HALO)] = xr[k];
         }
         __syncthreads();
-        if (tile + (int)gridDim.x < ntile) fetch_halo(tile + gridDim.x);
+        if (tile + nlanes < ntile) fetch_halo(tile + nlanes);
 
         auto do_row = [&](auto rr_c) {
             constexpr int rr = decltype(rr_c)::value;
@@ -272,7 +275,7 @@
         }
     }
 
-    if constexpr (MODE == 1) return;
+    if constexpr (MODE == 1) continue;
     if constexpr (MODE == 3) {
         __syncthreads();
         if (lx < 9) {
@@ -282,12 +285,12 @@
                 for (int j = 0; j < 4; ++j) red[wave][lx][16 * gq + 4 * kg + j] = acc[0][4 * gq + j];
         }
         __syncthreads();
-        float* slab = a.out + (int64_t)blockIdx.x * ST_C * 9;
+        float* slab = a.out + (int64_t)wlane * ST_C * 9;
         for (int idx = tid; idx < 9 * ST_C; idx += 256) {
             const int k = idx / ST_C, c = idx - k * ST_C;
             slab[c * 9 + k] = (red[0][k][c] + red[1][k][c]) + (red[2][k][c] + red[3][k][c]);
         }
-        return;
+        continue;
     }
     constexpr int NK = 2;
 #pragma unroll
@@ -308,17 +311,18 @@
             const float s2 = (red[0][1][tid] + red[1][1][tid]) + (red[2][1][tid] + red[3][1][tid]);
             const float n = cnt > 0.f ? cnt : 1.f;
             const float kk = have_pivot ? pivot[tid] : 0.f;
-            a.out[((int64_t)blockIdx.x * 2 + 0) * ST_C + tid] = kk + s1 / n;
-            a.out[((int64_t)blockIdx.x * 2 + 1) * ST_C + tid] = fmaxf(s2 - s1 * s1 / n, 0.f);
+            a.out[((int64_t)wlane * 2 + 0) * ST_C + tid] = kk + s1 / n;
+            a.out[((int64_t)wlane * 2 + 1) * ST_C + tid] = fmaxf(s2 - s1 * s1 / n, 0.f);
         }
         float* counts = a.out + (int64_t)ntile * 2 * ST_C;
-        if (tid == 0) counts[blockIdx.x] = cnt;
-        for (int r = gridDim.x + blockIdx.x * 256 + tid; r < ntile; r += gridDim.x * 256) counts[r] = 0.f;
+        if (tid == 0) counts[wlane] = cnt;
+        for (int r = nlanes + wlane * 256 + tid; r < ntile; r += nlanes * 256) counts[r] = 0.f;
     } else if constexpr (MODE == 2) {
         for (int idx = tid; idx < 2 * ST_C; idx += 256) {
             const int k = idx / ST_C, c = idx - k * ST_C;
-            a.out[((int64_t)blockIdx.x * 2 + k) * ST_C + c] = (red[0][k][c] + red[1][k][c]) + (red[2][k][c] + red[3][k][c]);
-        }
+            a.out[((int64_t)wlane * 2 + k) * ST_C + c] = (red[0][k][c] + red[1][k][c]) + (red[2][k][c] + red[3][k][c]);
+        }
+    }
     }
 }
 
@@ -326,12 +330,14 @@
 
 int uh_stem_mfma_launch(int mode, const void* x, int ldx, const void* w, const float* scale, const float* shift,
                                    const float* mean, const float* rstd, const float* dgamma, const float* dbeta, float inv_n,
-                                   const void* dz, int lddz, void* z, int ldz, float* out, int B, int H, int W, int grid,
-                                   uh_stream stream) {
+                                   const void* dz, int lddz, void* z, int ldz, float* out, int B, int H, int W, int nlanes,
+                                   int grid, uh_stream stream) {
     StemArgs a;
     a.x = (const bf16_t*)x; a.ldx = ldx; a.w = (const bf16_t*)w;
     a.scale = scale; a.shift = shift; a.mean = mean; a.rstd = rstd; a.dgamma = dgamma; a.dbeta = dbeta; a.inv_n = inv_n;
     a.dz = (const bf16_t*)dz; a.lddz = lddz; a.z = (bf16_t*)z; a.ldz = ldz; a.out = out;
+    UH_REQUIRE(grid > 0 && grid <= nlanes, "uh_stem_mfma_launch: bad grid %d for %d lanes", grid, nlanes);
+    a.nlanes = nlanes;
     a.B = B; a.H = H; a.W = W; a.tilesX = (W + ST_TILE - 1) / ST_TILE; a.tilesY = (H + ST_TILE - 1) / ST_TILE;
     hipStream_t st = (hipStream_t)stream;
     switch (mode) {
diff --git a/unet-medical-image-contour-segmentation_amd/csrc/uh_common.h b/unet-medical-image-contour-segmentation_amd/csrc/uh_common.h
--- a/unet-medical-image-contour-segmentation_amd/csrc/uh_common.h
+++ b/unet-medical-image-contour-segmentation_amd/csrc/uh_common.h
@@ -36,7 +36,7 @@
 
 int uh_stem_mfma_launch(int mode, const void* x, int ldx, const void* w, const float* scale, const float* shift, const float* mean,
                         const float* rstd, const float* dgamma, const float* dbeta, float inv_n, const void* dz, int lddz, void* z,
-                        int ldz, float* out, int B, int H, int W, int grid, uh_stream stream);
+                        int ldz, float* out, int B, int H, int W, int nlanes, int grid, uh_stream stream);
 
 template <typename T> struct uh_traits;
 template <> struct uh_traits<float> {
diff --git a/unet-medical-image-contour-segmentation_amd/ops.py b/unet-medical-image-contour-segmentation_amd/ops.py
--- a/unet-medical-image-contour-segmentation_amd/ops.py
+++ b/unet-medical-image-contour-segmentation_amd/ops.py
@@ -8,7 +8,7 @@
 import torch
 from torch.autograd import Function
 
-from ._lib import LIB, UH_BF16, UH_F32, UH_F32X3, UH_WFRAG, UH_WFRAG_D
+from ._lib import LIB, UH_BF16, UH_F32, UH_F32X3, UH_WFRAG, UH_WFRAG_D, grid_cap_flag
 
 BN_EPS_DEFAULT = 1e-5
 
@@ -124,6 +124,7 @@
 
 
 WGRAD_STREAM = None
+WGRAD_CUS = (0, 0)
 
 
 GRAD_DST = {}
@@ -301,7 +302,7 @@
 
 
 def conv3x3_fwd(x0: torch.Tensor, x1: Optional[torch.Tensor], w_packed: torch.Tensor, Cout: int,
-                want_stats: bool, dt_code: Optional[int] = None, wfrag: bool = False):
+                want_stats: bool, dt_code: Optional[int] = None, wfrag: bool = False, grid_cap: int = 0):
     B, H, W, C0 = x0.shape
     C1 = 0 if x1 is None else x1.shape[3]
     dt = _dt(x0) if dt_code is None else dt_code
@@ -311,9 +312,13 @@
         nslab = LIB.query("uh_conv3x3_stat_slabs", B, H, W, C0 + C1, Cout, dt)
         stats = torch.empty(nslab * (2 * Cout + 2), dtype=torch.float32, device=x0.device)
     name = "conv3x3_fwd_" + _variant((C0, C1), Cout, x0.element_size())
+    cap = 0
+    if grid_cap and dt in (UH_F32, UH_BF16) and LIB.query("uh_conv3x3_wfrag_ok", B, H, W, C0, C1, Cout, pixel_ld(x0), pixel_ld_or0(x1),
+                                                          Cout, dt):
+        cap = grid_cap_flag(grid_cap)
     with _Timed(name, 2.0 * B * H * W * Cout * 9 * (C0 + C1), ("fwd" if want_stats else "dgrad", B, H, W, C0 + C1, Cout)):
         LIB.call("uh_conv3x3_fwd", x0.data_ptr(), C0, pixel_ld(x0), _p(x1), C1, pixel_ld_or0(x1),
-                 w_packed.data_ptr(), y.data_ptr(), Cout, Cout, _p(stats), B, H, W, conv_flags(dt, wfrag), _stream())
+                 w_packed.data_ptr(), y.data_ptr(), Cout, Cout, _p(stats), B, H, W, conv_flags(dt, wfrag) | cap, _stream())
     return y, stats, nslab
 
 
@@ -384,7 +389,7 @@
 
 
 def conv3x3_wgrad(dy: torch.Tensor, x0: torch.Tensor, x1: Optional[torch.Tensor], out_krsc: torch.Tensor,
-                  split: bool = False, defer_cb=None) -> bool:
+                  split: bool = False, defer_cb=None, grid_cap: int = 0) -> bool:
     B, H, W, Cout = dy.shape
     C0 = x0.shape[3]
     C1 = 0 if x1 is None else x1.shape[3]
@@ -395,6 +400,8 @@
     name = "conv3x3_wgrad_" + ("mfma" if (C0 % 64 == 0 and C1 % 64 == 0 and Cout % 64 == 0) else
                                 ("stem" if C0 + C1 <= 4 else "generic"))
     batch = SLAB_BATCH if (defer_cb is not None and DEFER_SLABS and name == "conv3x3_wgrad_mfma") else None
+    if grid_cap and name == "conv3x3_wgrad_mfma":
+        dt |= grid_cap_flag(grid_cap)
     timed = _Timed(name, 2.0 * B * H * W * Cout * 9 * (C0 + C1), ("wgrad", B, H, W, C0 + C1, Cout))
     if batch is not None:
         ws = batch.workspace(out_krsc.data_ptr(), nbytes, dy.device)
@@ -823,6 +830,11 @@
         dy = torch.empty_like(y)
         _bn_backward_finish(partials, nblk, Cout, bn_bufs[0][0], bn_bufs[1][0], ctx.sync_bn, ctx.n_total, apply)
         dx0 = dx1 = None
+        dweight = cb_w = side_done = None
+        if need["weight"]:
+            dweight, cb_w = _grad_buffer(weight)
+        to_side = cb_w is not None and WGRAD_STREAM is not None and _is_krsc_dense(weight)
+        side_cus, main_cus = WGRAD_CUS if to_side else (0, 0)
         if wd is not None and (need["x0"] or need["x1"]):
             use, rows = ctx.bnsum_use, 0
             if use is not None and use.y is not None and use.y.shape == (B, H, W, Cin) and use.y.is_contiguous() and \
@@ -834,29 +846,26 @@
                 with _Timed("conv3x3_dgrad_bnsum_mfma", 2.0 * B * H * W * Cin * 9 * Cout, ("dgrad", B, H, W, Cout, Cin)):
                     LIB.call("uh_conv3x3_dgrad_bnsum", dy.data_ptr(), Cout, Cout, wd.data_ptr(), dx.data_ptr(), Cin, Cin,
                              use.y.data_ptr(), Cin, use.coef.data_ptr(), bsum.data_ptr(), B, H, W,
-                             conv_flags(ctx.cdt, ctx.frag_d), _stream())
+                             conv_flags(ctx.cdt, ctx.frag_d) | grid_cap_flag(main_cus), _stream())
                 use.partials, use.rows, use.dz, use.dz_version = bsum, rows, dx, dx._version
             else:
-                dx, _, _ = conv3x3_fwd(dy, None, wd, Cin, False, ctx.cdt, ctx.frag_d)
+                dx, _, _ = conv3x3_fwd(dy, None, wd, Cin, False, ctx.cdt, ctx.frag_d, grid_cap=main_cus)
             dx0 = dx[..., :C0] if need["x0"] else None
             dx1 = dx[..., C0:] if (x1 is not None and need["x1"]) else None
-        dweight = side_done = None
-
-        def run_wgrad(out_, defer_cb=None):
+        def run_wgrad(out_, defer_cb=None, cus=0):
             if pre_coef is None:
-                return conv3x3_wgrad(dy, x0, x1, out_, ctx.cdt == UH_F32X3, defer_cb)
+                return conv3x3_wgrad(dy, x0, x1, out_, ctx.cdt == UH_F32X3, defer_cb, grid_cap=cus)
             conv3x3_wgrad_pre(dy, x0, pre_coef, out_)
             return False
 
         if need["weight"]:
-            dweight, cb_w = _grad_buffer(weight)
-            if cb_w is not None and WGRAD_STREAM is not None and _is_krsc_dense(weight):
+            if to_side:
                 side = WGRAD_STREAM
                 ev = torch.cuda.Event()
                 ev.record()
                 side.wait_event(ev)
                 with torch.cuda.stream(side):
-                    run_wgrad(dweight)
+                    run_wgrad(dweight, cus=side_cus)
                     side_done = torch.cuda.Event()
                     side_done.record()
                 for t_ in (dy, x0, x1, pre_coef):
diff --git a/unet-medical-image-contour-segmentation_amd/train.py b/unet-medical-image-contour-segmentation_amd/train.py
--- a/unet-medical-image-contour-segmentation_amd/train.py
+++ b/unet-medical-image-contour-segmentation_amd/train.py
@@ -456,6 +456,30 @@
     return terms
 
 
+WGRAD_CUS_TABLE = (
+    ("bf16", 1 << 21, 0),
+    ("bf16", 1 << 20, 0),
+)
+
+
+def wgrad_cus_for(pixels: int, dtype: str, cus: int) -> int:
+    if cus <= 1 or pixels <= 0:
+        return 0
+    for dt, floor, w256 in WGRAD_CUS_TABLE:
+        if dt == dtype and pixels >= floor:
+            return max(0, min(cus - 1, (w256 * cus + 128) // 256))
+    return 0
+
+
+def parse_wgrad_cus(text: Optional[str]) -> Optional[int]:
+    if text is None or text.strip() == "":
+        return None
+    t = text.strip()
+    if not t.isdigit() or int(t) > 4094:
+        raise ValueError(f"UH_WGRAD_CUS={text!r}: expected a compute-unit count (0 = off)")
+    return int(t)
+
+
 class TrainStepper:
 
     def __init__(self, model: nn.Module, lr: float = 1e-5, weight_decay: float = 1e-8, momentum: float = 0.999,
@@ -497,11 +521,31 @@
         self._pack = None
         sync = self.optimizer.sync
         self._slabs = ops.SlabBatch(flush_bytes=None if sync is None else 8 << 20)
+        self._wgrad_cus_env = parse_wgrad_cus(os.environ.get("UH_WGRAD_CUS"))
+        self._cu_count = None
+
+    def _cu_budgets(self, images, side):
+        if side is None or not images.is_cuda:
+            return (0, 0)
+        if self._cu_count is None:
+            self._cu_count = int(torch.cuda.get_device_properties(images.device).multi_processor_count)
+        cus = self._cu_count
+        w = self._wgrad_cus_env
+        if w is None:
+            w = wgrad_cus_for(images.shape[0] * images.shape[-2] * images.shape[-1], "bf16" if self.amp else "fp32", cus)
+        if w == 0:
+            return (0, 0)
+        if w >= cus:
+            raise ValueError(f"UH_WGRAD_CUS={w}: the device has {cus} compute units, the backward chain needs some")
+        return (w, cus - w)
 
     def close(self):
         opt = getattr(self, "optimizer", None)
         if opt is not None:
             opt.close()
+        slabs = getattr(self, "_slabs", None)
+        if slabs is not None:
+            slabs.close()
         grp, self.bn_group = getattr(self, "bn_group", None), None
         if grp is not None:
             import torch.distributed as dist
@@ -563,6 +607,7 @@
         self.model.train()
         side = self._side_for(images)
         ops.WGRAD_STREAM = side
+        ops.WGRAD_CUS = self._cu_budgets(images, side)
         ops.SYNC_BN = self.sync_bn
         ops.SYNC_BN_BATCH = None
         world = self.world
@@ -587,6 +632,7 @@
                               surface_weight=self.surface_weight, surface_classes=self.surface_classes)
         finally:
             ops.SLAB_BATCH = None
+            ops.WGRAD_CUS = (0, 0)
             ops.FP32_MODE = fp32_mode_before
 
 
```

New measurement: 877.4 images/sec. No clear change (-0.4%).
